# topel/audioset-convnext-inf

Hardware: NVIDIA B200
Metric: clips/sec (10s@32kHz, bf16) (higher is better)
Workload: dtype bf16

## Files before the change

### audioset-convnext-inf_b200/_native.py

```python
import ctypes
import os
import threading

_HERE = os.path.dirname(os.path.abspath(__file__))
_LIB_PATH = os.environ.get("ACX_LIBACX") or os.path.join(_HERE, "libacx.so")
_lock = threading.Lock()
_lib = None

ACX_BF16, ACX_F32 = 0, 1
EPI_BIAS, EPI_BIAS_GELU, EPI_BIAS_SCALE_RESID = 0, 1, 2

_vp, _i, _ll = ctypes.c_void_p, ctypes.c_int, ctypes.c_longlong

SIGNATURES = {
    "acx_version": [],
    "acx_last_error": [],
    "acx_device_ok": [],
    "acx_wave_prep": [_vp, _vp, _vp, _i, _i, _i, _i, _i, _vp],
    "acx_wave_prep_pcm16": [_vp, _vp, _vp, _i, _i, _i, _i, _i, _vp],
    "acx_power_mel_log": [_vp, _i, _i, _vp, _vp, _vp, _vp, _vp, _vp, _i, _i, _vp],
    "acx_frontend_fused": [_vp, _vp, _i, _vp, _vp, _vp, _vp, _i, _vp, _vp, _vp, _i, _i, _i, _i, _i, _vp],
    "acx_frame_fold": [_vp, _vp, _vp, _i, _i, _i, _i, _i, _vp],
    "acx_frame_fold_pcm16": [_vp, _vp, _vp, _i, _i, _i, _i, _i, _vp],
    "acx_frontend_folded": [_vp, _vp, _vp, _vp, _vp, _vp, _i, _vp, _vp, _vp, _i, _i, _i, _i, _vp],
    "acx_stem": [_vp, _vp, _vp, _vp, _vp, _vp, _i, _i, _i, _i, _vp],
    "acx_stem_gp": [_vp, _vp, _vp, _vp, _vp, _vp, _i, _i, _i, _vp],
    "acx_dwconv_ln": [_vp, _vp, _vp, _vp, _vp, _vp, _i, _i, _i, _i, _i, _vp],
    "acx_dwconv_tc": [_vp, _vp, _vp, _vp, _i, _i, _i, _i, _vp],
    "acx_layernorm_rows": [_vp, _vp, _vp, _vp, _ll, _i, _vp],
    "acx_dwconv_tc_gp": [_vp, _vp, _vp, _vp, _i, _i, _i, _i, _vp],
    "acx_gp_transpose": [_vp, _vp, _ll, _i, _i, _vp],
    "acx_gp_row_stats": [_vp, _vp, _ll, _i, _vp],
    "acx_ln_patchify_gp": [_vp, _vp, _vp, _vp, _i, _i, _i, _i, _vp],
    "acx_ln_patchify": [_vp, _vp, _vp, _vp, _i, _i, _i, _i, _i, _vp],
    "acx_downsample_fused_gp": [_vp, _vp, _vp, _vp, _vp, _vp, _i, _i, _i, _i, _i, _vp],
    "acx_gemm_bf16": [_vp, _vp, _vp, _i, _i, _i, _i, _vp, _vp, _vp, _vp],
    "acx_gemm_bf16_gp_out": [_vp, _vp, _vp, _i, _i, _i, _vp, _vp],
    "acx_gemm_bf16_pw1_gp": [_vp, _vp, _vp, _i, _i, _i, _vp, _vp, _vp, _vp],
    "acx_gemm_bf16_pw2_gp": [_vp, _vp, _vp, _i, _i, _i, _vp, _vp, _vp],
    "acx_gemm_f32": [_vp, _ll, _i, _i, _vp, _vp, _i, _i, _i, _i, _i, _vp, _vp, _vp, _vp],
    "acx_mlp_fused": [_vp, _vp, _vp, _vp, _vp, _vp, _vp, _i, _i, _vp],
    "acx_mlp_fused_ln": [_vp, _vp, _vp, _vp, _vp, _vp, _vp, _vp, _vp, _i, _i, _vp],
    "acx_mlp_fused_gp": [_vp, _vp, _vp, _vp, _vp, _vp, _vp, _vp, _vp, _vp, _i, _i, _vp],
    "acx_head": [_vp, _vp, _vp, _vp, _vp, _vp, _vp, _vp, _vp, _i, _i, _i, _i, _i, _i, _vp],
    "acx_nhwc_to_nchw_f32": [_vp, _vp, _i, _i, _i, _i, _i, _vp],
    "acx_resample_fit": [_vp, _i, _vp, _vp, _i, _i, _i, _i, _i, _i, _i, _vp],
    "acx_wave_prep_ragged": [_vp, _vp, _vp, _i, _i, _i, _i, _i, _i, _vp, _vp],
    "acx_frame_fold_ragged": [_vp, _vp, _vp, _i, _i, _i, _i, _i, _i, _vp, _vp],
    "acx_stem_ragged": [_vp, _vp, _vp, _vp, _vp, _vp, _i, _i, _i, _i, _vp, _vp],
    "acx_stem_gp_ragged": [_vp, _vp, _vp, _vp, _vp, _vp, _i, _i, _i, _vp, _vp],
    "acx_dwconv_tc_ragged": [_vp, _vp, _vp, _vp, _i, _i, _i, _i, _vp, _vp],
    "acx_dwconv_tc_gp_ragged": [_vp, _vp, _vp, _vp, _i, _i, _i, _i, _vp, _vp],
    "acx_dwconv_ln_ragged": [_vp, _vp, _vp, _vp, _vp, _vp, _i, _i, _i, _i, _i, _vp, _vp],
    "acx_head_ragged": [_vp, _vp, _vp, _vp, _vp, _vp, _vp, _vp, _vp, _i, _i, _i, _i, _i, _i, _vp, _vp],
    "acx_nhwc_to_nchw_f32_ragged": [_vp, _vp, _i, _i, _i, _i, _i, _vp, _vp],
    "acx_wave_prep_windows": [_vp, _ll, _vp, _vp, _vp, _vp, _i, _i, _i, _i, _i, _vp],
    "acx_wave_prep_pcm16_windows": [_vp, _ll, _vp, _vp, _vp, _vp, _i, _i, _i, _i, _i, _vp],
    "acx_frame_fold_windows": [_vp, _ll, _vp, _vp, _vp, _vp, _i, _i, _i, _i, _i, _vp],
    "acx_frame_fold_pcm16_windows": [_vp, _ll, _vp, _vp, _vp, _vp, _i, _i, _i, _i, _i, _vp],
}


class NativeError(RuntimeError):
    pass


def lib_path():
    return _LIB_PATH


def load():
    global _lib
    if _lib is not None:
        return _lib
    with _lock:
        if _lib is not None:
            return _lib
        if not os.path.isfile(_LIB_PATH):
            try:
                from . import build as _build
                _build.build()
            except Exception as e:
                raise NativeError(
                    f"libacx.so is missing at {_LIB_PATH} and could not be built ({e}). "
                    "The B200 path has no CPU or PyTorch fallback.") from e
        try:
            lib = ctypes.CDLL(_LIB_PATH)
        except OSError as e:
            raise NativeError(f"cannot load {_LIB_PATH}: {e}") from e
        for name, argtypes in SIGNATURES.items():
            try:
                fn = getattr(lib, name)
            except AttributeError as e:
                raise NativeError(f"{_LIB_PATH} does not export {name}; rebuild it") from e
            fn.argtypes = argtypes
            fn.restype = ctypes.c_char_p if name == "acx_last_error" else ctypes.c_int
        _lib = lib
    return _lib


def last_error():
    msg = load().acx_last_error()
    return msg.decode("utf-8", "replace") if msg else ""


def check(rc, what):
    if rc != 0:
        raise NativeError(f"{what} failed (code {rc}): {last_error()}")


def call(name, *args):
    check(getattr(load(), name)(*args), name)
```

### audioset-convnext-inf_b200/csrc/common.cuh

```cuda
#pragma once
#include <cuda.h>
#include <cuda_bf16.h>
#include <cuda_fp16.h>
#include <cuda_runtime.h>
#include <stdint.h>
#include <stdio.h>
#include <stdlib.h>

#include <atomic>

#include "../../include/acx.h"

namespace acx {

void set_error(const char* fmt, ...);
const char* last_error();

#define ACX_CHECK(cond, code, ...)                  \
  do {                                              \
    if (!(cond)) {                                  \
      ::acx::set_error(__VA_ARGS__);                \
      return (code);                                \
    }                                               \
  } while (0)

#define ACX_CUDA(expr)                                                              \
  do {                                                                              \
    cudaError_t _e = (expr);                                                        \
    if (_e != cudaSuccess) {                                                        \
      ::acx::set_error("%s failed: %s (%s:%d)", #expr, cudaGetErrorString(_e),      \
                       __FILE__, __LINE__);                                         \
      return ACX_ERR_CUDA;                                                          \
    }                                                                               \
  } while (0)

#define ACX_SET_MAX_SMEM(kern, bytes)                                                               \
  do {                                                                                              \
    static std::atomic<unsigned long long> acx_done_{0};       \
    int acx_dev_ = 0;                                                                               \
    ACX_CUDA(cudaGetDevice(&acx_dev_));                                                             \
    if (acx_dev_ >= 64 || !((acx_done_.load(std::memory_order_acquire) >> acx_dev_) & 1ull)) {      \
      ACX_CUDA(cudaFuncSetAttribute(kern, cudaFuncAttributeMaxDynamicSharedMemorySize, (bytes)));   \
      if (acx_dev_ < 64) acx_done_.fetch_or(1ull << acx_dev_, std::memory_order_release);           \
    }                                                                                               \
  } while (0)

static inline int sm_count() {
  static std::atomic<int> cached[64];
  int dev = 0;
  if (cudaGetDevice(&dev) != cudaSuccess) return 148;
  if (dev < 64) {
    const int c = cached[dev].load(std::memory_order_relaxed);
    if (c > 0) return c;
  }
  int sms = 0;
  if (cudaDeviceGetAttribute(&sms, cudaDevAttrMultiProcessorCount, dev) != cudaSuccess || sms <= 0) return 148;
  if (dev < 64) cached[dev].store(sms, std::memory_order_relaxed);
  return sms;
}

#ifndef ACX_PDL_DEFAULT
#define ACX_PDL_DEFAULT 7
#endif
__device__ __forceinline__ void pdl_trigger() { asm volatile("griddepcontrol.launch_dependents;" ::: "memory"); }
__device__ __forceinline__ void pdl_wait() { asm volatile("griddepcontrol.wait;" ::: "memory"); }

enum PdlKind { PDL_GEMM = 1, PDL_MLP = 2, PDL_DWTC = 4, PDL_STATS = 8, PDL_SMALL = 16 };
static inline bool pdl_enabled(int kind) {
  const char* e = getenv("ACX_PDL");
  return ((e ? atoi(e) : ACX_PDL_DEFAULT) & kind) != 0;
}

template <typename... KArgs, typename... Args>
static inline cudaError_t launch_pdl(void (*kern)(KArgs...), dim3 grid, dim3 block, size_t smem, cudaStream_t st, int cluster_x,
                                     int kind, Args&&... args) {
  cudaLaunchConfig_t cfg = {};
  cfg.gridDim = grid;
  cfg.blockDim = block;
  cfg.dynamicSmemBytes = smem;
  cfg.stream = st;
  cudaLaunchAttribute attr[2];
  unsigned na = 0;
  if (cluster_x > 1) {
    attr[na].id = cudaLaunchAttributeClusterDimension;
    attr[na].val.clusterDim.x = cluster_x;
    attr[na].val.clusterDim.y = 1;
    attr[na].val.clusterDim.z = 1;
    ++na;
  }
  if (pdl_enabled(kind)) {
    attr[na].id = cudaLaunchAttributeProgrammaticStreamSerialization;
    attr[na].val.programmaticStreamSerializationAllowed = 1;
    ++na;
  }
  cfg.attrs = attr;
  cfg.numAttrs = na;
  return cudaLaunchKernelEx(&cfg, kern, static_cast<KArgs>(args)...);
}

static inline int ceil_div(int a, int b) { return (a + b - 1) / b; }
static inline size_t align_up(size_t x, size_t a) { return (x + a - 1) / a * a; }

using bf16 = __nv_bfloat16;

template <typename T> struct Pair;
template <> struct Pair<float> {
  using type = float2;
  __device__ static __forceinline__ float2 unpack(float2 v) { return v; }
  __device__ static __forceinline__ float2 pack(float a, float b) { return make_float2(a, b); }
};
template <> struct Pair<bf16> {
  using type = uint32_t;
  __device__ static __forceinline__ float2 unpack(uint32_t v) {
    return make_float2(__uint_as_float(v << 16), __uint_as_float(v & 0xffff0000u));
  }
  __device__ static __forceinline__ uint32_t pack(float a, float b) {
    __nv_bfloat162 h = __floats2bfloat162_rn(a, b);
    return *reinterpret_cast<uint32_t*>(&h);
  }
};

__device__ __forceinline__ float to_float(float v) { return v; }
__device__ __forceinline__ float to_float(bf16 v) { return __bfloat162float(v); }
template <typename T> __device__ __forceinline__ T from_float(float v);
template <> __device__ __forceinline__ float from_float<float>(float v) { return v; }
template <> __device__ __forceinline__ bf16 from_float<bf16>(float v) { return __float2bfloat16_rn(v); }

__device__ __forceinline__ float warp_sum(float v) {
#pragma unroll
  for (int o = 16; o > 0; o >>= 1) v += __shfl_xor_sync(0xffffffffu, v, o);
  return v;
}

__device__ __forceinline__ float gelu_erf(float x) {
  return 0.5f * x * (1.0f + erff(x * 0.70710678118654752440f));
}

struct GeluPair {
  unsigned long long x, u;
};
__device__ __forceinline__ unsigned long long f2_pack(float lo, float hi) {
  unsigned long long r;
  asm("mov.b64 %0, {%1, %2};" : "=l"(r) : "f"(lo), "f"(hi));
  return r;
}
__device__ __forceinline__ void gelu_op_tanh(GeluPair& g) {
  asm volatile(
      "{\n\t.reg .f32 lo, hi;\n\tmov.b64 {lo, hi}, %0;\n\ttanh.approx.f32 lo, lo;\n\ttanh.approx.f32 hi, hi;\n\t"
      "mov.b64 %0, {lo, hi};\n\t}"
      : "+l"(g.u));
}
struct LnFold {
  unsigned long long rstd2, nmr2;
  uint32_t sb1_base, sbs_base;
};
template <bool kT, bool kA, bool kFold = false>
__device__ __forceinline__ void gelu_stage_ta4(GeluPair* t, GeluPair* a, const uint32_t* acc, uint32_t sbias_addr,
                                               const LnFold fold = LnFold{}) {
  const unsigned long long k50 = f2_pack(50.0f, 50.0f);
  const unsigned long long kc = f2_pack(-3.51516788e-04f, -3.51516788e-04f);
  const unsigned long long kb = f2_pack(3.70056460e-02f, 3.70056460e-02f);
  const unsigned long long ka = f2_pack(7.97507884e-01f, 7.97507884e-01f);
  unsigned long long q[4], p[4];
  if (kT) gelu_op_tanh(t[0]);
  if (kA) {
#pragma unroll
    for (int i = 0; i < 4; ++i) {
      float2 b;
#ifdef ACX_AB_NO_FOLD_EPI
      if (false) {
#else
      if (kFold) {
#endif
        float2 sj;
        asm("ld.shared.v4.f32 {%0, %1, %2, %3}, [%4];"
            : "=f"(b.x), "=f"(b.y), "=f"(sj.x), "=f"(sj.y)
            : "r"(fold.sbs_base + 2 * (sbias_addr - fold.sb1_base) + 16 * i));
        unsigned long long tt;
        asm volatile("fma.rn.f32x2 %0, %1, %2, %3;" : "=l"(tt) : "l"(fold.nmr2), "l"(f2_pack(sj.x, sj.y)), "l"(f2_pack(b.x, b.y)));
        asm volatile("fma.rn.f32x2 %0, %1, %2, %3;"
                     : "=l"(a[i].x)
                     : "l"(fold.rstd2), "l"(f2_pack(__uint_as_float(acc[2 * i]), __uint_as_float(acc[2 * i + 1]))), "l"(tt));
      } else {
        asm("ld.shared.v2.f32 {%0, %1}, [%2];" : "=f"(b.x), "=f"(b.y) : "r"(sbias_addr + 8 * i));
        asm volatile("add.rn.f32x2 %0, %1, %2;"
                     : "=l"(a[i].x)
                     : "l"(f2_pack(__uint_as_float(acc[2 * i]), __uint_as_float(acc[2 * i + 1]))), "l"(f2_pack(b.x, b.y)));
      }
    }
  }
  if (kT) gelu_op_tanh(t[1]);
  if (kA) {
#pragma unroll
    for (int i = 0; i < 4; ++i) asm volatile("mul.rn.f32x2 %0, %1, %1;" : "=l"(q[i]) : "l"(a[i].x));
#pragma unroll
    for (int i = 0; i < 4; ++i)
      asm volatile(
          "{\n\t.reg .f32 lo, hi, c;\n\tmov.b64 {lo, hi}, %0;\n\tmov.b64 {c, _}, %1;\n\t"
          "min.f32 lo, lo, c;\n\tmin.f32 hi, hi, c;\n\tmov.b64 %0, {lo, hi};\n\t}"
          : "+l"(q[i])
          : "l"(k50));
  }
  if (kT) gelu_op_tanh(t[2]);
  if (kA) {
#pragma unroll
    for (int i = 0; i < 4; ++i) asm volatile("fma.rn.f32x2 %0, %1, %2, %3;" : "=l"(p[i]) : "l"(q[i]), "l"(kc), "l"(kb));
  }
  if (kT) gelu_op_tanh(t[3]);
  if (kA) {
#pragma unroll
    for (int i = 0; i < 4; ++i) asm volatile("fma.rn.f32x2 %0, %1, %2, %3;" : "=l"(q[i]) : "l"(q[i]), "l"(p[i]), "l"(ka));
#pragma unroll
    for (int i = 0; i < 4; ++i) asm volatile("mul.rn.f32x2 %0, %1, %2;" : "=l"(a[i].u) : "l"(a[i].x), "l"(q[i]));
  }
}
__device__ __forceinline__ void gelu_stage_c8_twice_bf16(const GeluPair* g, uint32_t* pk) {
  unsigned long long o[8];
#pragma unroll
  for (int i = 0; i < 8; ++i) asm volatile("fma.rn.f32x2 %0, %1, %2, %1;" : "=l"(o[i]) : "l"(g[i].x), "l"(g[i].u));
#pragma unroll
  for (int i = 0; i < 8; ++i)
    asm volatile("{\n\t.reg .f32 lo, hi;\n\tmov.b64 {lo, hi}, %1;\n\tcvt.rn.bf16x2.f32 %0, hi, lo;\n\t}"
                 : "=r"(pk[i])
                 : "l"(o[i]));
}

template <bool kTwice, bool kFold = false>
__device__ __forceinline__ void bias_gelu_tile16_sp(const uint32_t* __restrict__ acc ,
                                                    const float* __restrict__ sbias , float2 (&out)[16],
                                                    const LnFold fold = LnFold{}) {
  GeluPair g[16];
  const uint32_t sb = static_cast<uint32_t>(__cvta_generic_to_shared(sbias));
  gelu_stage_ta4<false, true, kFold>(nullptr, g, acc, sb, fold);
  gelu_stage_ta4<true, true, kFold>(g, g + 4, acc + 8, sb + 32, fold);
  gelu_stage_ta4<true, true, kFold>(g + 4, g + 8, acc + 16, sb + 64, fold);
  gelu_stage_ta4<true, true, kFold>(g + 8, g + 12, acc + 24, sb + 96, fold);
  gelu_stage_ta4<true, false>(g + 12, nullptr, nullptr, 0);
  const unsigned long long khalf = f2_pack(0.5f, 0.5f);
#pragma unroll
  for (int i = 0; i < 16; ++i) {
    unsigned long long o, x = g[i].x;
    if (!kTwice) asm volatile("mul.rn.f32x2 %0, %1, %2;" : "=l"(x) : "l"(g[i].x), "l"(khalf));
    asm volatile("fma.rn.f32x2 %0, %1, %2, %1;" : "=l"(o) : "l"(x), "l"(g[i].u));
    asm("mov.b64 {%0, %1}, %2;" : "=f"(out[i].x), "=f"(out[i].y) : "l"(o));
  }
}

}
```

### audioset-convnext-inf_b200/csrc/dwconv_tc.cu

```cuda
#include <stdlib.h>

#include "common.cuh"
#include "ptx.cuh"

namespace acx {
namespace dwtc {

constexpr int TR = 63;
constexpr int AR = TR + 6;
constexpr int A_STRIDE = 73 * 128;
constexpr int CG = 8;
constexpr int BAND_TILE = 32 * 64;
constexpr int BAND = 7 * BAND_TILE;
constexpr int NSLOT = 2;
constexpr int THREADS = 256;
constexpr int OFF_A = 0;
constexpr int OFF_BAND = CG * A_STRIDE;
constexpr int OFF_TAPS = OFF_BAND + NSLOT * BAND;
constexpr int OFF_DUMMY = OFF_TAPS + 1024;
constexpr int OFF_BAR = OFF_DUMMY + 512;
constexpr int SMEM_BYTES = OFF_BAR + 128 + 1024;
static_assert(OFF_BAND % 1024 == 0 && BAND % 1024 == 0, "swizzle atoms");
static_assert(2 * (SMEM_BYTES + 1024) <= 227 * 1024, "two CTAs per SM");
static_assert(TR * 28 * 16 <= NSLOT * BAND, "the write-out staging of the planar layout lives in the band slots");
// ... 595 lines not shown
    float sum = 0.f;
#pragma unroll
    for (int j = 0; j < CH; ++j) sum += val[q][j];
#pragma unroll
    for (int o = LPP / 2; o > 0; o >>= 1) sum += __shfl_xor_sync(0xffffffffu, sum, o);
    const float mean = sum * (1.0f / C);
    float sq = 0.f;
#pragma unroll
    for (int j = 0; j < CH; ++j) {
      val[q][j] -= mean;
      sq = fmaf(val[q][j], val[q][j], sq);
    }
#pragma unroll
    for (int o = LPP / 2; o > 0; o >>= 1) sq += __shfl_xor_sync(0xffffffffu, sq, o);
    const float rstd = rsqrtf(sq * (1.0f / C) + 1e-6f);
    if (ok[q]) {
      bf16* dst = out + (grp * NPIX + q) * C + lig * CH;
#pragma unroll
      for (int j = 0; j < 3; ++j) {
        const int k = 8 * j;
        const float4 g0 = __ldg(reinterpret_cast<const float4*>(gp + k)), g1 = __ldg(reinterpret_cast<const float4*>(gp + k + 4));
        const float4 b0 = __ldg(reinterpret_cast<const float4*>(bp + k)), b1 = __ldg(reinterpret_cast<const float4*>(bp + k + 4));
        uint4 o4;
        o4.x = Pair<bf16>::pack(val[q][k + 0] * rstd * g0.x + b0.x, val[q][k + 1] * rstd * g0.y + b0.y);
        o4.y = Pair<bf16>::pack(val[q][k + 2] * rstd * g0.z + b0.z, val[q][k + 3] * rstd * g0.w + b0.w);
        o4.z = Pair<bf16>::pack(val[q][k + 4] * rstd * g1.x + b1.x, val[q][k + 5] * rstd * g1.y + b1.y);
        o4.w = Pair<bf16>::pack(val[q][k + 6] * rstd * g1.z + b1.z, val[q][k + 7] * rstd * g1.w + b1.w);
        reinterpret_cast<uint4*>(dst)[j] = o4;
      }
    }
  }
}

template <int C>
static int launch_ln(const void* in, const float* ln_w, const float* ln_b, void* out, long long M, cudaStream_t st) {
  constexpr int LPP = C / 24, NPIX = 2;
  const long long lanes = (M + NPIX - 1) / NPIX * LPP;
  const long long blocks = (lanes + 255) / 256;
  layernorm_rows_kernel<C><<<(unsigned)blocks, 256, 0, st>>>(reinterpret_cast<const bf16*>(in), ln_w, ln_b,
                                                             reinterpret_cast<bf16*>(out), M);
  ACX_CUDA(cudaGetLastError());
  return ACX_OK;
}

}
}

using namespace acx;

template <bool RAG>
static int dwconv_tc_impl(const void* x, const void* w, const float* bias, void* v, int B, int H, int W, int C,
                          const int32_t* valid, void* stream) {
  ACX_CHECK(x && w && bias && v, ACX_ERR_ARG, "dwconv_tc: null pointer");
  ACX_CHECK(B > 0 && H > 0, ACX_ERR_ARG, "dwconv_tc: B and H must be positive");
  ACX_CHECK(C % 8 == 0 && C > 0, ACX_ERR_ARG, "dwconv_tc: C must be a positive multiple of 8 (got %d)", C);
  ACX_CHECK(x != v, ACX_ERR_ARG, "dwconv_tc: out of place only (neighbouring units read the input halo)");
  ACX_CHECK(((reinterpret_cast<uintptr_t>(x) | reinterpret_cast<uintptr_t>(v)) & 15) == 0, ACX_ERR_ARG,
            "dwconv_tc: x and v must be 16-byte aligned");
  cudaStream_t st = reinterpret_cast<cudaStream_t>(stream);
  switch (W) {
    case 56: return dwtc::launch<56, false, RAG>(x, w, bias, v, B, H, C, valid, st);
    case 28: return dwtc::launch<28, false, RAG>(x, w, bias, v, B, H, C, valid, st);
    case 14: return dwtc::launch<14, false, RAG>(x, w, bias, v, B, H, C, valid, st);
    case 7: return dwtc::launch<7, false, RAG>(x, w, bias, v, B, H, C, valid, st);
    default:
      set_error("dwconv_tc: W=%d not supported (the ConvNeXt stages are 56 / 28 / 14 / 7 wide)", W);
      return ACX_ERR_UNSUPPORTED;
  }
}

extern "C" int acx_dwconv_tc(const void* x, const void* w, const float* bias, void* v, int B, int H, int W, int C,
                             void* stream) {
  return dwconv_tc_impl<false>(x, w, bias, v, B, H, W, C, nullptr, stream);
}

extern "C" int acx_dwconv_tc_ragged(const void* x, const void* w, const float* bias, void* v, int B, int H, int W, int C,
                                    const int32_t* valid, void* stream) {
  ACX_CHECK(valid, ACX_ERR_ARG, "dwconv_tc_ragged: null valid-length array");
  return dwconv_tc_impl<true>(x, w, bias, v, B, H, W, C, valid, stream);
}

template <bool RAG>
static int dwconv_tc_gp_impl(const void* x, const void* w, const float* bias, void* v, int B, int H, int W, int C,
                             const int32_t* valid, void* stream) {
  ACX_CHECK(x && w && bias && v, ACX_ERR_ARG, "dwconv_tc_gp: null pointer");
  ACX_CHECK(B > 0 && H > 0, ACX_ERR_ARG, "dwconv_tc_gp: B and H must be positive");
  ACX_CHECK(C % 8 == 0 && C > 0, ACX_ERR_ARG, "dwconv_tc_gp: C must be a positive multiple of 8 (got %d)", C);
  ACX_CHECK(x != v, ACX_ERR_ARG, "dwconv_tc_gp: out of place only (neighbouring units read the input halo)");
  ACX_CHECK(((reinterpret_cast<uintptr_t>(x) | reinterpret_cast<uintptr_t>(v) | reinterpret_cast<uintptr_t>(w)) & 15) == 0,
            ACX_ERR_ARG, "dwconv_tc_gp: x, v and w must be 16-byte aligned");
  cudaStream_t st = reinterpret_cast<cudaStream_t>(stream);
  static const bool use_v1 = getenv("ACX_DWTC_V1") != nullptr;
  switch (W) {
    case 56:
      return use_v1 ? dwtc::launch<56, true, RAG>(x, w, bias, v, B, H, C, valid, st)
                    : dwtc::v3::launch<56, RAG>(x, w, bias, v, B, H, C, valid, st);
    case 28:
      return use_v1 ? dwtc::launch<28, true, RAG>(x, w, bias, v, B, H, C, valid, st)
                    : dwtc::v3::launch<28, RAG>(x, w, bias, v, B, H, C, valid, st);
    case 14: return dwtc::v3::launch<14, RAG>(x, w, bias, v, B, H, C, valid, st);
    default:
      set_error("dwconv_tc_gp: W=%d not supported (stages 0 - 2: 56 / 28 / 14)", W);
      return ACX_ERR_UNSUPPORTED;
  }
}

extern "C" int acx_dwconv_tc_gp(const void* x, const void* w, const float* bias, void* v, int B, int H, int W, int C,
                                void* stream) {
  return dwconv_tc_gp_impl<false>(x, w, bias, v, B, H, W, C, nullptr, stream);
}

extern "C" int acx_dwconv_tc_gp_ragged(const void* x, const void* w, const float* bias, void* v, int B, int H, int W, int C,
                                       const int32_t* valid, void* stream) {
  ACX_CHECK(valid, ACX_ERR_ARG, "dwconv_tc_gp_ragged: null valid-length array");
  return dwconv_tc_gp_impl<true>(x, w, bias, v, B, H, W, C, valid, stream);
}

namespace acx {
namespace dwtc {
__global__ void __launch_bounds__(256) gp_transpose_kernel(const uint4* __restrict__ in, uint4* __restrict__ out, long long M,
                                                           int G, int to_gp) {
  extern __shared__ uint4 tile[];
  const long long r0 = (long long)blockIdx.x * 64;
  const int rows = (int)min((long long)64, M - r0);
  const int pitch = G + 1;
  const long long Mp = (M + 127) / 128 * 128;
  if (to_gp) {
    for (int i = threadIdx.x; i < rows * G; i += 256) {
      const int r = i / G, gq = i - r * G;
      tile[r * pitch + gq] = in[(r0 + r) * G + gq];
    }
    __syncthreads();
    for (int i = threadIdx.x; i < rows * G; i += 256) {
      const int gq = i / rows, r = i - gq * rows;
      out[(long long)gq * Mp + r0 + r] = tile[r * pitch + gq];
    }
  } else {
    for (int i = threadIdx.x; i < rows * G; i += 256) {
      const int gq = i / rows, r = i - gq * rows;
      tile[r * pitch + gq] = in[(long long)gq * Mp + r0 + r];
    }
    __syncthreads();
    for (int i = threadIdx.x; i < rows * G; i += 256) {
      const int r = i / G, gq = i - r * G;
      out[(r0 + r) * G + gq] = tile[r * pitch + gq];
    }
  }
}
}
}

namespace acx {
namespace dwtc {
__global__ void __launch_bounds__(128) gp_row_stats_kernel(const uint4* __restrict__ v, float2* __restrict__ stats,
                                                           long long M, int G) {
  pdl_trigger();
  pdl_wait();
  const long long row = (long long)blockIdx.x * blockDim.x + threadIdx.x;
  if (row >= M) return;
  const long long Mp = (M + 127) / 128 * 128;
  const float inv_c = 1.0f / (8.0f * G);
  const uint4 first = __ldg(v + row);
  const float shift = __uint_as_float(first.x << 16);
  const float2 sh2 = make_float2(-shift, -shift);
  float2 s = make_float2(0.f, 0.f), q = make_float2(0.f, 0.f);
  for (int g0 = 0; g0 < G; g0 += 12) {
    uint4 u[12];
#pragma unroll
    for (int j = 0; j < 12; ++j) u[j] = g0 + j < G ? __ldg(v + (long long)(g0 + j) * Mp + row) : make_uint4(0, 0, 0, 0);
#pragma unroll
    for (int j = 0; j < 12; ++j) {
      if (g0 + j < G) {
        const uint32_t w[4] = {u[j].x, u[j].y, u[j].z, u[j].w};
#pragma unroll
        for (int k = 0; k < 4; ++k) {
          const float2 d = __fadd2_rn(Pair<bf16>::unpack(w[k]), sh2);
          s = __fadd2_rn(s, d);
          q = __ffma2_rn(d, d, q);
        }
      }
    }
  }
  const float md = (s.x + s.y) * inv_c;
  const float var = fmaxf((q.x + q.y) * inv_c - md * md, 0.f);
  const float rstd = rsqrtf(var + 1e-6f);
  stats[row] = make_float2(rstd, -(md + shift) * rstd);
}
}
}

extern "C" int acx_gp_row_stats(const void* v, float* stats, long long M, int C, void* stream) {
  ACX_CHECK(v && stats, ACX_ERR_ARG, "gp_row_stats: null pointer");
  ACX_CHECK(M > 0 && C > 0 && C % 8 == 0, ACX_ERR_ARG, "gp_row_stats: bad shape M=%lld C=%d", M, C);
  ACX_CUDA(launch_pdl(dwtc::gp_row_stats_kernel, dim3((unsigned)((M + 127) / 128)), dim3(128), 0, reinterpret_cast<cudaStream_t>(stream),
                      1, PDL_STATS, reinterpret_cast<const uint4*>(v), reinterpret_cast<float2*>(stats), M, C / 8));
  return ACX_OK;
}

extern "C" int acx_gp_transpose(const void* in, void* out, long long M, int C, int to_gp, void* stream) {
  ACX_CHECK(in && out && in != out, ACX_ERR_ARG, "gp_transpose: null or aliased pointers");
  ACX_CHECK(M > 0 && C > 0 && C % 8 == 0 && C <= 768, ACX_ERR_ARG, "gp_transpose: bad shape M=%lld C=%d", M, C);
  ACX_CHECK(((reinterpret_cast<uintptr_t>(in) | reinterpret_cast<uintptr_t>(out)) & 15) == 0, ACX_ERR_ARG,
            "gp_transpose: 16-byte alignment");
  const int G = C / 8;
  const size_t smem = (size_t)64 * (G + 1) * 16;
  auto kern = dwtc::gp_transpose_kernel;
  ACX_SET_MAX_SMEM(kern, 64 * (768 / 8 + 1) * 16);
  kern<<<(unsigned)((M + 63) / 64), 256, smem, reinterpret_cast<cudaStream_t>(stream)>>>(
      reinterpret_cast<const uint4*>(in), reinterpret_cast<uint4*>(out), M, G, to_gp);
  ACX_CUDA(cudaGetLastError());
  return ACX_OK;
}

extern "C" int acx_layernorm_rows(const void* in, const float* ln_w, const float* ln_b, void* out, long long M, int C,
                                  void* stream) {
  ACX_CHECK(in && ln_w && ln_b && out, ACX_ERR_ARG, "layernorm_rows: null pointer");
  ACX_CHECK(M > 0, ACX_ERR_ARG, "layernorm_rows: M must be positive");
  ACX_CHECK(((reinterpret_cast<uintptr_t>(in) | reinterpret_cast<uintptr_t>(out)) & 15) == 0, ACX_ERR_ARG,
            "layernorm_rows: in and out must be 16-byte aligned");
  cudaStream_t st = reinterpret_cast<cudaStream_t>(stream);
  switch (C) {
    case 96: return dwtc::launch_ln<96>(in, ln_w, ln_b, out, M, st);
    case 192: return dwtc::launch_ln<192>(in, ln_w, ln_b, out, M, st);
    case 384: return dwtc::launch_ln<384>(in, ln_w, ln_b, out, M, st);
    case 768: return dwtc::launch_ln<768>(in, ln_w, ln_b, out, M, st);
    default:
      set_error("layernorm_rows: C=%d not supported (96 / 192 / 384 / 768)", C);
      return ACX_ERR_UNSUPPORTED;
  }
}
```

### audioset-convnext-inf_b200/csrc/gemm_umma.cu

```cuda
#include <stdlib.h>

#include "common.cuh"
#include "ptx.cuh"
#include "tmap.cuh"

namespace acx {

struct GemmArgs {
  bf16* out;
  const float* bias;
  const float* gamma;
  const bf16* resid;
  int M, N, K;
  int out_gp;
  int a_gp;
  const float2* stats;
  const float* ln_s;
  int reverse;
};
constexpr int ACX_EPI_BIAS_GELU_FOLD = 3;

template <int BN_, int NEPI_, int CG_ = 1>
struct GemmCfg {
  static constexpr int BM = 128, BN = BN_, BK = 64, NEPI = NEPI_, CG = CG_;
  static constexpr int A_BYTES = BM * BK * 2;
  static constexpr int B_BYTES = (BN / CG) * BK * 2;
  static constexpr int STAGE_BYTES = A_BYTES + B_BYTES;
  static constexpr int STAGES_RAW = (160 * 1024) / STAGE_BYTES;
  static constexpr int STAGES = STAGES_RAW > 6 ? 6 : STAGES_RAW;
  static_assert(CG == 1 || BN % 32 == 0, "B halves");
  static constexpr int ACC_STRIDE = BN <= 32 ? 32 : BN <= 64 ? 64 : BN <= 128 ? 128 : 256;
  static constexpr int TMEM_COLS = 2 * ACC_STRIDE;
  static constexpr int CHUNK = 32;
  static constexpr int NCHUNKS = BN / CHUNK;
  static constexpr int CH_G0 = (NCHUNKS + 1) / 2;
  static constexpr int THREADS = 128 + 32 * NEPI;
  static constexpr int STG_TILE = 32 * CHUNK * 2;
  static constexpr int STG_PER_WARP = 3 * STG_TILE;
  static constexpr int OFF_STG = STAGES * STAGE_BYTES;
  static constexpr int OFF_BAR = OFF_STG + NEPI * STG_PER_WARP;
  static constexpr int OFF_VEC = OFF_BAR + 256;
  static constexpr int VEC_BYTES = 16 * 1024;
  static constexpr int SMEM_BYTES = OFF_VEC + VEC_BYTES + 1024 ;
  static_assert(NEPI == 8, "epilogue layout assumes 8 warps");
  static_assert(BN % 32 == 0 && BN >= 32 && BN <= 256, "UMMA N constraint for M=128 / 32-column epilogue chunks");
  static_assert(B_BYTES % 1024 == 0, "stage buffers must stay 1024B aligned for SWIZZLE_128B");
  static_assert(SMEM_BYTES <= 227 * 1024, "smem budget");
};

template <int BN, int EPI, int NEPI, int CG>
__global__ void __launch_bounds__(GemmCfg<BN, NEPI, CG>::THREADS, 1)
    umma_gemm_kernel(const __grid_constant__ CUtensorMap tmA, const __grid_constant__ CUtensorMap tmB,
                     const __grid_constant__ CUtensorMap tmOut, GemmArgs g) {
  using Cfg = GemmCfg<BN, NEPI, CG>;
  const uint32_t cta_rank = CG == 2 ? ptx::cluster_ctarank() : 0u;
  const int unit = CG == 2 ? blockIdx.x >> 1 : blockIdx.x;
  const int num_units = CG == 2 ? gridDim.x >> 1 : gridDim.x;
  extern __shared__ uint8_t smem_raw[];
  uint8_t* smem = reinterpret_cast<uint8_t*>((reinterpret_cast<uintptr_t>(smem_raw) + 1023) & ~uintptr_t(1023));
  uint64_t* full_bar = reinterpret_cast<uint64_t*>(smem + Cfg::OFF_BAR);
  uint64_t* empty_bar = full_bar + Cfg::STAGES;
  uint64_t* tfull_bar = empty_bar + Cfg::STAGES;
  uint64_t* tempty_bar = tfull_bar + 2;
  uint32_t* tmem_slot = reinterpret_cast<uint32_t*>(tempty_bar + 2);

  const int warp = threadIdx.x >> 5;
  const int lane = threadIdx.x & 31;
  float* sbias = reinterpret_cast<float*>(smem + Cfg::OFF_VEC);
  float* sgamma = sbias + g.N;
  if (EPI == ACX_EPI_BIAS_GELU_FOLD) {
    for (int i = threadIdx.x; i < g.N; i += blockDim.x) {
      sbias[4 * (i >> 1) + (i & 1)] = g.bias[i];
      sbias[4 * (i >> 1) + 2 + (i & 1)] = g.ln_s[i];
    }
  } else {
    for (int i = threadIdx.x; i < g.N; i += blockDim.x) {
      sbias[i] = g.bias[i];
      if (EPI == ACX_EPI_BIAS_SCALE_RESID) sgamma[i] = g.gamma[i];
    }
  }

  if (warp == 0 && ptx::elect_one()) {
    ptx::prefetch_tensormap(&tmA);
    ptx::prefetch_tensormap(&tmB);
    ptx::prefetch_tensormap(&tmOut);
  }
  if (warp == 1 && ptx::elect_one()) {
    for (int s = 0; s < Cfg::STAGES; ++s) {
      ptx::mbar_init(&full_bar[s], 1);
      ptx::mbar_init(&empty_bar[s], 1);
    }
    for (int a = 0; a < 2; ++a) {
      ptx::mbar_init(&tfull_bar[a], 1);
      ptx::mbar_init(&tempty_bar[a], NEPI * CG);
    }
    ptx::fence_barrier_init();
  }
  if (warp == 2) {
    if (CG == 2) {
      ptx::tmem_alloc_cg2(tmem_slot, Cfg::TMEM_COLS);
      ptx::tmem_relinquish_cg2();
    } else {
      ptx::tmem_alloc(tmem_slot, Cfg::TMEM_COLS);
      ptx::tmem_relinquish();
    }
  }
  ptx::tc_fence_before();
  __syncthreads();
  if (CG == 2) ptx::cluster_sync_all();
  ptx::tc_fence_after();
  const uint32_t tmem_base = *tmem_slot;
  pdl_trigger();
  pdl_wait();

  const int num_m_tiles = (g.M + Cfg::BM * CG - 1) / (Cfg::BM * CG);
  const int num_n_tiles = g.N / BN;
  const int num_tiles = num_m_tiles * num_n_tiles;
  const int num_kb = (g.K + Cfg::BK - 1) / Cfg::BK;

  if (warp == 0) {
    if (ptx::elect_one()) {
      int stage = 0;
      uint32_t phase = 0;
      for (int tile = unit; tile < num_tiles; tile += num_units) {
        const int tt = g.reverse ? num_tiles - 1 - tile : tile;
        const int m0 = (tt / num_n_tiles) * Cfg::BM * CG + cta_rank * Cfg::BM;
        const int n0 = (tt % num_n_tiles) * BN + cta_rank * (BN / CG);
        for (int kb = 0; kb < num_kb; ++kb) {
          ptx::mbar_wait(&empty_bar[stage], phase ^ 1);
          uint8_t* sa = smem + stage * Cfg::STAGE_BYTES;
          uint8_t* sb = sa + Cfg::A_BYTES;
          if (CG == 2) {
            if (cta_rank == 0) ptx::mbar_arrive_expect_tx(&full_bar[stage], 2 * Cfg::STAGE_BYTES);
            if (g.a_gp) ptx::tma_load_3d_cg2(sa, &tmA, &full_bar[stage], 0, m0 >> 5, kb * (Cfg::BK / 8));
            else ptx::tma_load_2d_cg2(sa, &tmA, &full_bar[stage], kb * Cfg::BK, m0);
            ptx::tma_load_2d_cg2(sb, &tmB, &full_bar[stage], kb * Cfg::BK, n0);
          } else {
            ptx::mbar_arrive_expect_tx(&full_bar[stage], Cfg::STAGE_BYTES);
            if (g.a_gp) ptx::tma_load_3d(sa, &tmA, &full_bar[stage], 0, m0 >> 5, kb * (Cfg::BK / 8));
            else ptx::tma_load_2d(sa, &tmA, &full_bar[stage], kb * Cfg::BK, m0);
            ptx::tma_load_2d(sb, &tmB, &full_bar[stage], kb * Cfg::BK, n0);
          }
          if (++stage == Cfg::STAGES) {
            stage = 0;
            phase ^= 1;
          }
        }
      }
    }
  } else if (warp == 1) {
    if (cta_rank == 0 && ptx::elect_one()) {
      constexpr uint32_t idesc = ptx::umma_idesc_bf16(Cfg::BM * CG, BN);
      int stage = 0;
      uint32_t phase = 0;
      int it = 0;
      for (int tile = unit; tile < num_tiles; tile += num_units, ++it) {
        const int acc = it & 1;
        const uint32_t acc_phase = (it >> 1) & 1;
        ptx::mbar_wait(&tempty_bar[acc], acc_phase ^ 1);
        ptx::tc_fence_after();
        const uint32_t d_tmem = tmem_base + acc * Cfg::ACC_STRIDE;
        for (int kb = 0; kb < num_kb; ++kb) {
          ptx::mbar_wait(&full_bar[stage], phase);
          ptx::tc_fence_after();
          const uint32_t sa = ptx::smem_u32(smem + stage * Cfg::STAGE_BYTES);
          const uint64_t da = g.a_gp ? ptx::umma_desc_nosw_kmajor(sa, Cfg::BM * 16, 128) : ptx::umma_desc_sw128_kmajor(sa);
          const uint32_t ka = g.a_gp ? (2 * Cfg::BM * 16) >> 4 : 2;
          const uint64_t db = ptx::umma_desc_sw128_kmajor(sa + Cfg::A_BYTES);
#pragma unroll
          for (int k = 0; k < Cfg::BK / 16; ++k) {
            if (kb * Cfg::BK + k * 16 < g.K) {
              if (CG == 2) ptx::umma_bf16_cg2(d_tmem, da + ka * k, db + 2 * k, idesc, (kb | k) != 0 ? 1u : 0u);
              else ptx::umma_bf16(d_tmem, da + ka * k, db + 2 * k, idesc, (kb | k) != 0 ? 1u : 0u);
            }
          }
          if (CG == 2) ptx::umma_commit_cg2(&empty_bar[stage]);
          else ptx::umma_commit(&empty_bar[stage]);
          if (++stage == Cfg::STAGES) {
            stage = 0;
            phase ^= 1;
          }
        }
        if (CG == 2) ptx::umma_commit_cg2(&tfull_bar[acc]);
        else ptx::umma_commit(&tfull_bar[acc]);
      }
    }
  } else if (warp >= 4) {
    const int ew = warp - 4;
    const int quad = warp & 3;
    const int group = ew >> 2;
    const int ch_begin = group == 0 ? 0 : Cfg::CH_G0;
    const int ch_count = group == 0 ? Cfg::CH_G0 : Cfg::NCHUNKS - Cfg::CH_G0;
    uint8_t* stg = smem + Cfg::OFF_STG + ew * Cfg::STG_PER_WARP;
    uint8_t* rbuf = stg + 2 * Cfg::STG_TILE;
    const int sw = (lane >> 1) & 3;
    const int ld_piece = lane & 3, ld_row = lane >> 2;
    int it = 0;
    uint32_t store_parity = 0;
    for (int tile = unit; tile < num_tiles; tile += num_units, ++it) {
      const int acc = it & 1;
      const uint32_t acc_phase = (it >> 1) & 1;
      const int tt = g.reverse ? num_tiles - 1 - tile : tile;
      const int m0 = (tt / num_n_tiles) * Cfg::BM * CG + cta_rank * Cfg::BM;
      const int n0 = (tt % num_n_tiles) * BN;
      const int row0 = m0 + quad * 32;
      uint4 rq[4];
      auto fetch_resid = [&](int ci) {
        if (EPI != ACX_EPI_BIAS_SCALE_RESID) return;
        const int n = n0 + (ch_begin + ci) * Cfg::CHUNK;
#pragma unroll
        for (int q = 0; q < 4; ++q) {
          const int r = row0 + ld_row + 8 * q;
          rq[q] = make_uint4(0u, 0u, 0u, 0u);
          if (r < g.M)
            rq[q] = g.out_gp ? *reinterpret_cast<const uint4*>(g.resid + ((size_t)((n >> 3) + ld_piece) * (((size_t)g.M + 127) / 128 * 128) + r) * 8)
                             : *reinterpret_cast<const uint4*>(g.resid + (size_t)r * g.N + n + ld_piece * 8);
        }
      };
      fetch_resid(0);
      LnFold fold{0ull, 0ull, ptx::smem_u32(sbias), ptx::smem_u32(sbias)};
      if (EPI == ACX_EPI_BIAS_GELU_FOLD) {
        const int r = row0 + lane;
        const float2 stt = r < g.M ? __ldg(g.stats + r) : make_float2(0.f, 0.f);
        fold.rstd2 = f2_pack(stt.x, stt.x);
        fold.nmr2 = f2_pack(stt.y, stt.y);
      }
      ptx::mbar_wait(&tfull_bar[acc], acc_phase);
      ptx::tc_fence_after();
      const uint32_t t_base = tmem_base + (static_cast<uint32_t>(quad * 32) << 16) + acc * Cfg::ACC_STRIDE +
                              ch_begin * Cfg::CHUNK;
      uint32_t ra[32], rb[32];
      ptx::tmem_ld_32x32b_x32(t_base, ra);
#pragma unroll
      for (int ci = 0; ci < Cfg::CH_G0; ++ci) {
        if (ci < ch_count) {
          uint32_t(&r)[32] = (ci & 1) ? rb : ra;
          ptx::tmem_ld_wait();
          if (ci + 1 < ch_count) {
            ptx::tmem_ld_32x32b_x32(t_base + (ci + 1) * Cfg::CHUNK, (ci & 1) ? ra : rb);
          } else {
            ptx::tc_fence_before();
            __syncwarp();
            if (lane == 0) {
              if (CG == 2) ptx::mbar_arrive_leader(&tempty_bar[acc]);
              else ptx::mbar_arrive(&tempty_bar[acc]);
            }
          }
          const int n = n0 + (ch_begin + ci) * Cfg::CHUNK;
          float v[32];
          if (EPI == ACX_EPI_BIAS_GELU_FOLD) {
            float2 o[16];
            bias_gelu_tile16_sp<false, true>(r, sbias + n, o, fold);
#pragma unroll
            for (int j = 0; j < 16; ++j) {
              v[2 * j] = o[j].x;
              v[2 * j + 1] = o[j].y;
            }
          } else if (EPI == ACX_EPI_BIAS_GELU) {
            float2 o[16];
            bias_gelu_tile16_sp<false>(r, sbias + n, o);
#pragma unroll
            for (int j = 0; j < 16; ++j) {
              v[2 * j] = o[j].x;
              v[2 * j + 1] = o[j].y;
            }
          } else {
#pragma unroll
            for (int j = 0; j < 32; j += 4) {
              const float4 b4 = *reinterpret_cast<const float4*>(sbias + n + j);
              v[j + 0] = __uint_as_float(r[j + 0]) + b4.x;
              v[j + 1] = __uint_as_float(r[j + 1]) + b4.y;
              v[j + 2] = __uint_as_float(r[j + 2]) + b4.z;
              v[j + 3] = __uint_as_float(r[j + 3]) + b4.w;
            }
          }
          if (EPI == ACX_EPI_BIAS_SCALE_RESID) {
            __syncwarp();
#pragma unroll
            for (int q = 0; q < 4; ++q) {
              const int rr = ld_row + 8 * q;
              *reinterpret_cast<uint4*>(rbuf + rr * 64 + ((ld_piece ^ ((rr >> 1) & 3)) << 4)) = rq[q];
            }
            __syncwarp();
            if (ci + 1 < ch_count) fetch_resid(ci + 1);
#pragma unroll
            for (int j4 = 0; j4 < 4; ++j4) {
              const uint4 q = *reinterpret_cast<const uint4*>(rbuf + lane * 64 + ((j4 ^ sw) << 4));
              const float4 g0 = *reinterpret_cast<const float4*>(sgamma + n + j4 * 8);
              const float4 g1 = *reinterpret_cast<const float4*>(sgamma + n + j4 * 8 + 4);
              const int j = j4 * 8;
              float2 f;
              f = Pair<bf16>::unpack(q.x); v[j + 0] = fmaf(g0.x, v[j + 0], f.x); v[j + 1] = fmaf(g0.y, v[j + 1], f.y);
              f = Pair<bf16>::unpack(q.y); v[j + 2] = fmaf(g0.z, v[j + 2], f.x); v[j + 3] = fmaf(g0.w, v[j + 3], f.y);
              f = Pair<bf16>::unpack(q.z); v[j + 4] = fmaf(g1.x, v[j + 4], f.x); v[j + 5] = fmaf(g1.y, v[j + 5], f.y);
              f = Pair<bf16>::unpack(q.w); v[j + 6] = fmaf(g1.z, v[j + 6], f.x); v[j + 7] = fmaf(g1.w, v[j + 7], f.y);
            }
          }
          if (lane == 0) ptx::tma_store_wait_read<1>();
          __syncwarp();
          uint8_t* tile_smem = stg + store_parity * Cfg::STG_TILE;
#pragma unroll
          for (int j4 = 0; j4 < 4; ++j4) {
            const int j = j4 * 8;
            uint4 q;
            q.x = Pair<bf16>::pack(v[j + 0], v[j + 1]);
            q.y = Pair<bf16>::pack(v[j + 2], v[j + 3]);
            q.z = Pair<bf16>::pack(v[j + 4], v[j + 5]);
            q.w = Pair<bf16>::pack(v[j + 6], v[j + 7]);
            *reinterpret_cast<uint4*>(g.out_gp ? tile_smem + j4 * 512 + lane * 16 : tile_smem + lane * 64 + ((j4 ^ sw) << 4)) = q;
          }
          ptx::fence_proxy_async_smem();
          __syncwarp();
          if (lane == 0) {
            if (g.out_gp) ptx::tma_store_3d(&tmOut, tile_smem, 0, row0 >> 5, n >> 3);
            else ptx::tma_store_2d(&tmOut, tile_smem, n, row0);
            ptx::tma_store_commit();
          }
          store_parity ^= 1;
        }
      }
    }
    if (lane == 0) ptx::tma_store_wait_read<0>();
  }

  ptx::tc_fence_before();
  __syncthreads();
  if (CG == 2) ptx::cluster_sync_all();
  if (warp == 2) {
    ptx::tc_fence_after();
    if (CG == 2) ptx::tmem_dealloc_cg2(tmem_base, Cfg::TMEM_COLS);
    else ptx::tmem_dealloc(tmem_base, Cfg::TMEM_COLS);
  }
}

template <int BN, int EPI, int NEPI, int CG>
static int launch_umma_gemm(const CUtensorMap& tmA, const CUtensorMap& tmB, const CUtensorMap& tmOut, const GemmArgs& g,
                            cudaStream_t st) {
  using Cfg = GemmCfg<BN, NEPI, CG>;
  auto kern = umma_gemm_kernel<BN, EPI, NEPI, CG>;
  ACX_SET_MAX_SMEM(kern, Cfg::SMEM_BYTES);
  ACX_CHECK(g.N * (EPI == ACX_EPI_BIAS_SCALE_RESID || EPI == ACX_EPI_BIAS_GELU_FOLD ? 8 : 4) <= Cfg::VEC_BYTES, ACX_ERR_UNSUPPORTED,
            "gemm_bf16: N=%d exceeds the per-column vectors staged in shared memory", g.N);
  int dev = 0, sms = 0;
  ACX_CUDA(cudaGetDevice(&dev));
  ACX_CUDA(cudaDeviceGetAttribute(&sms, cudaDevAttrMultiProcessorCount, dev));
  const int tiles = ceil_div(g.M, Cfg::BM * CG) * (g.N / BN);
  const int units = sms / CG;
  ACX_CUDA(launch_pdl(kern, dim3((tiles < units ? tiles : units) * CG), dim3(Cfg::THREADS), Cfg::SMEM_BYTES, st, CG, PDL_GEMM, tmA, tmB,
                      tmOut, g));
  return ACX_OK;
}

template <int EPI>
static int dispatch_bn(const CUtensorMap& tmA, const void* W, const GemmArgs& g, cudaStream_t st) {
  int bn = 0;
  for (int cand : {256, 192, 128, 96}) {
    if (g.N % cand == 0) {
      bn = cand;
      break;
    }
  }
  ACX_CHECK(bn != 0, ACX_ERR_UNSUPPORTED, "gemm_bf16: N=%d is not a multiple of 96/128/192/256", g.N);
  static const bool pair_ok = getenv("ACX_GEMM_PAIR") == nullptr || atoi(getenv("ACX_GEMM_PAIR")) != 0;
  const long long pairs = sm_count() / 2;
  if (pair_ok && bn == 256 && g.N % 192 == 0) {
    const long long mt = ceil_div(g.M, 256);
    const long long r256 = (mt * (g.N / 256) + pairs - 1) / pairs * 256, r192 = (mt * (g.N / 192) + pairs - 1) / pairs * 192;
    if (mt * (g.N / 192) >= pairs && r192 < r256) bn = 192;
  }
  const bool pair = pair_ok && (bn == 256 || bn == 192) && (long long)ceil_div(g.M, 256) * (g.N / bn) >= pairs;
  CUtensorMap tmB;
  int rc = make_tmap_2d_bf16(&tmB, W, (uint64_t)g.K, (uint64_t)g.N, (uint64_t)g.K * 2, 64,
                             (uint32_t)(pair ? bn / 2 : bn));
  if (rc != ACX_OK) return rc;
  CUtensorMap tmOut;
  rc = g.out_gp ? make_tmap_gp_bf16(&tmOut, g.out, (uint64_t)g.M, (uint64_t)g.N / 8, 32, 4)
                : make_tmap_2d_bf16(&tmOut, g.out, (uint64_t)g.N, (uint64_t)g.M, (uint64_t)g.N * 2, 32, 32,
                                    CU_TENSOR_MAP_SWIZZLE_64B);
  if (rc != ACX_OK) return rc;
  if (pair) {
    if (bn == 256) return launch_umma_gemm<256, EPI, 8, 2>(tmA, tmB, tmOut, g, st);
    return launch_umma_gemm<192, EPI, 8, 2>(tmA, tmB, tmOut, g, st);
  }
  switch (bn) {
    case 256: return launch_umma_gemm<256, EPI, 8, 1>(tmA, tmB, tmOut, g, st);
    case 192: return launch_umma_gemm<192, EPI, 8, 1>(tmA, tmB, tmOut, g, st);
    case 128: return launch_umma_gemm<128, EPI, 8, 1>(tmA, tmB, tmOut, g, st);
    default:  return launch_umma_gemm<96, EPI, 8, 1>(tmA, tmB, tmOut, g, st);
  }
}

}

using namespace acx;

static int gemm_bf16_impl(const void* A, const void* W, void* out, int M, int N, int K, int epilogue, const float* bias,
                          const float* gamma, const void* resid, int out_gp, int a_gp, const float* stats,
                          const float* ln_s, void* stream) {
  ACX_CHECK(A && W && out && bias, ACX_ERR_ARG, "gemm_bf16: null pointer (A, W, out and bias are required)");
  ACX_CHECK(M > 0 && N > 0 && K > 0 && K % 8 == 0, ACX_ERR_ARG, "gemm_bf16: K=%d must be a positive multiple of 8", K);
  ACX_CHECK((reinterpret_cast<uintptr_t>(A) & 15) == 0 && (reinterpret_cast<uintptr_t>(W) & 15) == 0 &&
                (reinterpret_cast<uintptr_t>(out) & 15) == 0,
            ACX_ERR_ARG, "gemm_bf16: A, W and out must be 16-byte aligned");
  if (epilogue == ACX_EPI_BIAS_SCALE_RESID)
    ACX_CHECK(gamma && resid, ACX_ERR_ARG, "gemm_bf16: scale+residual epilogue needs gamma and resid");
  ACX_CHECK(!out_gp || epilogue != ACX_EPI_BIAS_GELU, ACX_ERR_UNSUPPORTED, "gemm_bf16: the hidden activation stays row-major");
  ACX_CHECK(!a_gp || K % 64 == 0, ACX_ERR_UNSUPPORTED, "gemm_bf16: a planar A operand needs K %% 64 == 0 (got %d)", K);
  ACX_CHECK((stats == nullptr) == (ln_s == nullptr), ACX_ERR_ARG, "gemm_bf16: stats and ln_s go together");
  ACX_CHECK(!stats || epilogue == ACX_EPI_BIAS_GELU, ACX_ERR_UNSUPPORTED, "gemm_bf16: the LayerNorm fold belongs to the GELU epilogue");
  GemmArgs g;
  g.out = reinterpret_cast<bf16*>(out);
  g.bias = bias;
  g.gamma = gamma;
  g.resid = reinterpret_cast<const bf16*>(resid);
  g.M = M;
  g.N = N;
  g.K = K;
  g.out_gp = out_gp;
  g.a_gp = a_gp;
  g.stats = reinterpret_cast<const float2*>(stats);
  g.ln_s = ln_s;
  static const bool rev_ok = getenv("ACX_GEMM_REVERSE") == nullptr || atoi(getenv("ACX_GEMM_REVERSE")) != 0;
  g.reverse = rev_ok && epilogue == ACX_EPI_BIAS_SCALE_RESID && (size_t)M * K * 2 > (size_t)96 << 20;
  CUtensorMap tmA;
  int rc = a_gp ? make_tmap_gp_bf16(&tmA, A, (uint64_t)M, (uint64_t)K / 8, 128, 8)
                : make_tmap_2d_bf16(&tmA, A, (uint64_t)K, (uint64_t)M, (uint64_t)K * 2, 64, 128);
  if (rc != ACX_OK) return rc;
  cudaStream_t st = reinterpret_cast<cudaStream_t>(stream);
  switch (epilogue) {
    case ACX_EPI_BIAS: return dispatch_bn<ACX_EPI_BIAS>(tmA, W, g, st);
    case ACX_EPI_BIAS_GELU:
      return stats ? dispatch_bn<ACX_EPI_BIAS_GELU_FOLD>(tmA, W, g, st) : dispatch_bn<ACX_EPI_BIAS_GELU>(tmA, W, g, st);
    case ACX_EPI_BIAS_SCALE_RESID: return dispatch_bn<ACX_EPI_BIAS_SCALE_RESID>(tmA, W, g, st);
    default:
      set_error("gemm_bf16: unknown epilogue %d", epilogue);
      return ACX_ERR_ARG;
  }
}

extern "C" int acx_gemm_bf16(const void* A, const void* W, void* out, int M, int N, int K, int epilogue,
                             const float* bias, const float* gamma, const void* resid, void* stream) {
  return gemm_bf16_impl(A, W, out, M, N, K, epilogue, bias, gamma, resid, 0, 0, nullptr, nullptr, stream);
}

extern "C" int acx_gemm_bf16_gp_out(const void* A, const void* W, void* out, int M, int N, int K, const float* bias,
                                    void* stream) {
  return gemm_bf16_impl(A, W, out, M, N, K, ACX_EPI_BIAS, bias, nullptr, nullptr, 1, 0, nullptr, nullptr, stream);
}

extern "C" int acx_gemm_bf16_pw1_gp(const void* v_gp, const void* w1f, void* hid, int M, int N, int K, const float* b1f,
                                    const float* stats, const float* ln_s, void* stream) {
  ACX_CHECK(stats && ln_s, ACX_ERR_ARG, "gemm_bf16_pw1_gp: stats and ln_s are required");
  return gemm_bf16_impl(v_gp, w1f, hid, M, N, K, ACX_EPI_BIAS_GELU, b1f, nullptr, nullptr, 0, 1, stats, ln_s, stream);
}
extern "C" int acx_gemm_bf16_pw2_gp(const void* hid, const void* w2, void* x_gp, int M, int N, int K, const float* b2,
                                    const float* gamma, void* stream) {
  return gemm_bf16_impl(hid, w2, x_gp, M, N, K, ACX_EPI_BIAS_SCALE_RESID, b2, gamma, x_gp, 1, 0, nullptr, nullptr, stream);
}
```

### audioset-convnext-inf_b200/csrc/mlp_fused.cu

```cuda
#include <stdlib.h>

#include "common.cuh"
#include "ptx.cuh"
#include "tmap.cuh"

namespace acx {

struct MlpArgs {
  bf16* x;
  const float* b1;
  const float* b2;
  const float* gamma;
  int M;
  const float* ln_w;
  const float* ln_b;
  const float* ln_s;
  unsigned long long* trace;
};

template <int C, typename ChunkFn>
__device__ __forceinline__ void ln_row_in_smem(ChunkFn chunk, const float* __restrict__ sw, const float* __restrict__ sb) {
  constexpr int NCH = C / 8;
  float shift;
  {
    const uint32_t w0 = *reinterpret_cast<const uint32_t*>(chunk(0));
    shift = __uint_as_float(w0 << 16);
  }
  const float2 sh2 = make_float2(-shift, -shift);
  float2 s = make_float2(0.f, 0.f), q = make_float2(0.f, 0.f);
#pragma unroll 4
  for (int j = 0; j < NCH; ++j) {
    const uint4 v = *reinterpret_cast<const uint4*>(chunk(j));
    const uint32_t w[4] = {v.x, v.y, v.z, v.w};
#pragma unroll
    for (int k = 0; k < 4; ++k) {
      const float2 d = __fadd2_rn(Pair<bf16>::unpack(w[k]), sh2);
      s = __fadd2_rn(s, d);
      q = __ffma2_rn(d, d, q);
    }
  }
  const float md = (s.x + s.y) * (1.0f / C);
  const float var = fmaxf((q.x + q.y) * (1.0f / C) - md * md, 0.f);
  const float rstd = rsqrtf(var + 1e-6f);
  const float nmr = -(md + shift) * rstd;
  const float2 r2 = make_float2(rstd, rstd), n2 = make_float2(nmr, nmr);
#pragma unroll 2
  for (int j = 0; j < NCH; ++j) {
    uint8_t* pc = chunk(j);
    const uint4 v = *reinterpret_cast<const uint4*>(pc);
    const uint32_t w[4] = {v.x, v.y, v.z, v.w};
    uint32_t o[4];
#pragma unroll
    for (int k = 0; k < 4; ++k) {
      const float2 g = *reinterpret_cast<const float2*>(sw + 8 * j + 2 * k);
      const float2 b = *reinterpret_cast<const float2*>(sb + 8 * j + 2 * k);
      const float2 t = __fmul2_rn(r2, g);
      const float2 u = __ffma2_rn(n2, g, b);
      const float2 y = __ffma2_rn(Pair<bf16>::unpack(w[k]), t, u);
      o[k] = Pair<bf16>::pack(y.x, y.y);
    }
    *reinterpret_cast<uint4*>(pc) = make_uint4(o[0], o[1], o[2], o[3]);
  }
}

template <int C, typename ChunkFn>
__device__ __forceinline__ float2 ln_row_stats_smem(ChunkFn chunk) {
  constexpr int NCH = C / 8;
  const float shift = __uint_as_float(*reinterpret_cast<const uint32_t*>(chunk(0)) << 16);
  const float2 sh2 = make_float2(-shift, -shift);
  float2 s = make_float2(0.f, 0.f), q = make_float2(0.f, 0.f);
#pragma unroll 4
  for (int j = 0; j < NCH; ++j) {
    const uint4 v = *reinterpret_cast<const uint4*>(chunk(j));
    const uint32_t w[4] = {v.x, v.y, v.z, v.w};
#pragma unroll
    for (int k = 0; k < 4; ++k) {
      const float2 d = __fadd2_rn(Pair<bf16>::unpack(w[k]), sh2);
      s = __fadd2_rn(s, d);
      q = __ffma2_rn(d, d, q);
    }
  }
  const float md = (s.x + s.y) * (1.0f / C);
  const float var = fmaxf((q.x + q.y) * (1.0f / C) - md * md, 0.f);
  const float rstd = rsqrtf(var + 1e-6f);
  return make_float2(rstd, -(md + shift) * rstd);
}

template <int C_>
struct MlpCfg {
  static constexpr int C = C_, HD = 4 * C, BM = 128, NH = 128, BK = 64;
  static constexpr int NC = HD / NH;
  static constexpr int KB1 = (C + BK - 1) / BK;
  static constexpr int KB2 = NH / BK;
  static constexpr int A_TILE = BM * BK * 2;
  static constexpr int A_BUFS = C <= 96 ? 2 : 1;
  static constexpr int W1_TILE = NH * BK * 2;
  static constexpr int W2_TILE = C * BK * 2;
  static constexpr int SLOT = W1_TILE > W2_TILE ? W1_TILE : W2_TILE;
  static constexpr int SLOTS = C <= 96 ? 4 : 3;
  static constexpr int H_TILE = BM * BK * 2;
  static constexpr int OFF_A = 0;
  static constexpr int OFF_RING = OFF_A + A_BUFS * KB1 * A_TILE;
  static constexpr int OFF_H = OFF_RING + SLOTS * SLOT;
  static constexpr int OFF_STG = OFF_H + 2 * KB2 * H_TILE;
  static constexpr int STG_TILE = 32 * 64;
  static constexpr int STG_PER_WARP = STG_TILE;
  static constexpr int OFF_BAR = OFF_STG + 8 * STG_PER_WARP;
  static constexpr int OFF_VEC = OFF_BAR + 512;
  static constexpr int SMEM_BYTES = OFF_VEC + (3 * HD + 4 * C) * 4 + 2 * BM * 8 + 1024;
  static constexpr int D2_COL = 0, D1_COL = 256, TMEM_COLS = 512;
  static constexpr int OUT_CHUNKS = C / 32;
  static constexpr int OUT_G0 = (OUT_CHUNKS + 1) / 2;
  static constexpr int THREADS = 512;
  static_assert(C % 32 == 0 && C <= 192, "D2 must fit 256 TMEM columns");
  static_assert(SLOT % 1024 == 0 && W2_TILE % 1024 == 0, "swizzle alignment");
  static_assert(SMEM_BYTES <= 227 * 1024, "smem budget");
};

template <int C, bool GP, bool FOLD>
__global__ void __launch_bounds__(512, 1)
    mlp_fused_kernel(const __grid_constant__ CUtensorMap tmY, const __grid_constant__ CUtensorMap tmW1,
                     const __grid_constant__ CUtensorMap tmW2, const __grid_constant__ CUtensorMap tmOut, MlpArgs a) {
  using Cfg = MlpCfg<C>;
  extern __shared__ uint8_t smem_raw[];
  uint8_t* smem = reinterpret_cast<uint8_t*>((reinterpret_cast<uintptr_t>(smem_raw) + 1023) & ~uintptr_t(1023));
  uint64_t* bars = reinterpret_cast<uint64_t*>(smem + Cfg::OFF_BAR);
  uint64_t* ring_full = bars;
  uint64_t* ring_empty = ring_full + Cfg::SLOTS;
  uint64_t* a_full = ring_empty + Cfg::SLOTS;
  uint64_t* a_empty = a_full + Cfg::A_BUFS;
  uint64_t* d1_full = a_empty + Cfg::A_BUFS;
  uint64_t* d1_empty = d1_full + 2;
  uint64_t* h_full = d1_empty + 2;
  uint64_t* h_empty = h_full + 2;
  uint64_t* d2_full = h_empty + 2;
  uint64_t* d2_empty = d2_full + 1;
  uint64_t* a_ready = d2_empty + 1;
  uint32_t* tmem_slot = reinterpret_cast<uint32_t*>(a_ready + Cfg::A_BUFS);

  const int warp = threadIdx.x >> 5;
  const int lane = threadIdx.x & 31;
  float* sb1 = reinterpret_cast<float*>(smem + Cfg::OFF_VEC);
  float* sb2 = sb1 + Cfg::HD;
  float* sgamma = sb2 + C;
  float* slnw = sgamma + C;
  float* slnb = slnw + C;
  float* ss1 = slnb + C;
  float2* sstat = reinterpret_cast<float2*>(ss1 + 2 * Cfg::HD);
  const bool ln = a.ln_w != nullptr;
  for (int i = threadIdx.x; i < Cfg::HD; i += blockDim.x) sb1[i] = a.b1[i];
  if (FOLD)
    for (int i = threadIdx.x; i < Cfg::HD; i += blockDim.x) {
      ss1[4 * (i >> 1) + (i & 1)] = a.b1[i];
      ss1[4 * (i >> 1) + 2 + (i & 1)] = a.ln_s[i];
    }
  if (ln)
    for (int i = threadIdx.x; i < C; i += blockDim.x) {
      slnw[i] = a.ln_w[i];
      slnb[i] = a.ln_b[i];
    }
  for (int i = threadIdx.x; i < C; i += blockDim.x) {
    sgamma[i] = 0.5f * a.gamma[i];
    sb2[i] = a.gamma[i] * a.b2[i];
  }

  if (warp == 0 && ptx::elect_one()) {
    ptx::prefetch_tensormap(&tmY);
    ptx::prefetch_tensormap(&tmW1);
    ptx::prefetch_tensormap(&tmW2);
    ptx::prefetch_tensormap(&tmOut);
  }
  if (warp == 1 && ptx::elect_one()) {
    for (int s = 0; s < Cfg::SLOTS; ++s) {
      ptx::mbar_init(&ring_full[s], 1);
      ptx::mbar_init(&ring_empty[s], 1);
    }
    for (int s = 0; s < Cfg::A_BUFS; ++s) {
      ptx::mbar_init(&a_full[s], 1);
      ptx::mbar_init(&a_empty[s], FOLD ? 5 : 1);
      ptx::mbar_init(&a_ready[s], 4);
    }
    for (int s = 0; s < 2; ++s) {
      ptx::mbar_init(&d1_full[s], 1);
      ptx::mbar_init(&d1_empty[s], 8);
      ptx::mbar_init(&h_full[s], 8);
      ptx::mbar_init(&h_empty[s], 1);
    }
    ptx::mbar_init(d2_full, 1);
    ptx::mbar_init(d2_empty, 4);
    ptx::fence_barrier_init();
  }
  if (warp == 2) {
    ptx::tmem_alloc(tmem_slot, Cfg::TMEM_COLS);
    ptx::tmem_relinquish();
  }
  ptx::tc_fence_before();
  __syncthreads();
  ptx::tc_fence_after();
  const uint32_t tmem_base = *tmem_slot;
  const int num_tiles = (a.M + Cfg::BM - 1) / Cfg::BM;
  pdl_trigger();
  if (warp != 0) pdl_wait();

  if (warp == 3) {
    if (ptx::elect_one()) {
      int it = 0;
      for (int tile = blockIdx.x; tile < num_tiles; tile += gridDim.x, ++it) {
        const int buf = it % Cfg::A_BUFS;
        const uint32_t use = it / Cfg::A_BUFS;
        ptx::mbar_wait(&a_empty[buf], (use & 1) ^ 1);
        uint8_t* sa = smem + Cfg::OFF_A + buf * Cfg::KB1 * Cfg::A_TILE;
        ptx::mbar_arrive_expect_tx(&a_full[buf], Cfg::KB1 * Cfg::A_TILE);
        if (GP) {
          ptx::tma_load_3d(sa, &tmY, &a_full[buf], 0, tile * (Cfg::BM / 32), 0);
        } else {
          for (int kb = 0; kb < Cfg::KB1; ++kb)
            ptx::tma_load_2d(sa + kb * Cfg::A_TILE, &tmY, &a_full[buf], kb * Cfg::BK, tile * Cfg::BM);
        }
      }
    }
  } else if (warp == 0) {
    if (ptx::elect_one()) {
      int slot = 0;
      uint32_t phase = 0;
      auto next_slot = [&]() -> uint8_t* {
        ptx::mbar_wait(&ring_empty[slot], phase ^ 1);
        return smem + Cfg::OFF_RING + slot * Cfg::SLOT;
      };
      auto advance = [&]() {
        if (++slot == Cfg::SLOTS) {
          slot = 0;
          phase ^= 1;
        }
      };
      auto load_w2 = [&](int hh) {
        for (int kb = 0; kb < Cfg::KB2; ++kb) {
          uint8_t* dst = next_slot();
          ptx::mbar_arrive_expect_tx(&ring_full[slot], Cfg::W2_TILE);
          ptx::tma_load_2d(dst, &tmW2, &ring_full[slot], hh * Cfg::NH + kb * Cfg::BK, 0);
          advance();
        }
      };
      for (int tile = blockIdx.x; tile < num_tiles; tile += gridDim.x) {
        for (int h = 0; h < Cfg::NC; ++h) {
          for (int kb = 0; kb < Cfg::KB1; ++kb) {
            uint8_t* dst = next_slot();
            ptx::mbar_arrive_expect_tx(&ring_full[slot], Cfg::W1_TILE);
            ptx::tma_load_2d(dst, &tmW1, &ring_full[slot], kb * Cfg::BK, h * Cfg::NH);
            advance();
          }
          if (h >= 1) load_w2(h - 1);
        }
        load_w2(Cfg::NC - 1);
      }
    }
  } else if (warp == 1) {
    if (ptx::elect_one()) {
      constexpr uint32_t idesc1 = ptx::umma_idesc_bf16(Cfg::BM, Cfg::NH);
      constexpr uint32_t idesc2 = ptx::umma_idesc_bf16(Cfg::BM, C);
      const uint32_t d2 = tmem_base + Cfg::D2_COL;
      int slot = 0;
      uint32_t phase = 0;
      auto advance = [&]() {
        if (++slot == Cfg::SLOTS) {
          slot = 0;
          phase ^= 1;
        }
      };
      int it = 0;
      uint32_t gc = 0;
      for (int tile = blockIdx.x; tile < num_tiles; tile += gridDim.x, ++it) {
        const int abuf = it % Cfg::A_BUFS;
        const uint32_t ause = it / Cfg::A_BUFS;
        const uint32_t sa = ptx::smem_u32(smem + Cfg::OFF_A + abuf * Cfg::KB1 * Cfg::A_TILE);
        auto gemm2 = [&](int hh, uint32_t gch) {
          const int hb = gch & 1;
          ptx::mbar_wait(&h_full[hb], (gch >> 1) & 1);
          if (hh == 0) ptx::mbar_wait(d2_empty, (it & 1) ^ 1);
          ptx::tc_fence_after();
          const uint32_t sh = ptx::smem_u32(smem + Cfg::OFF_H + hb * Cfg::KB2 * Cfg::H_TILE);
          for (int kb = 0; kb < Cfg::KB2; ++kb) {
            ptx::mbar_wait(&ring_full[slot], phase);
            ptx::tc_fence_after();
            const uint64_t da = ptx::umma_desc_sw128_kmajor(sh + kb * Cfg::H_TILE);
            const uint64_t db = ptx::umma_desc_sw128_kmajor(ptx::smem_u32(smem + Cfg::OFF_RING + slot * Cfg::SLOT));
#pragma unroll
            for (int k = 0; k < Cfg::BK / 16; ++k)
              ptx::umma_bf16(d2, da + 2 * k, db + 2 * k, idesc2, (hh | kb | k) != 0 ? 1u : 0u);
            ptx::umma_commit(&ring_empty[slot]);
            advance();
          }
          ptx::umma_commit(&h_empty[hb]);
        };
        ptx::mbar_wait((ln && !FOLD) ? &a_ready[abuf] : &a_full[abuf], ause & 1);
        ptx::tc_fence_after();
        for (int h = 0; h < Cfg::NC; ++h, ++gc) {
          const int db1 = gc & 1;
          ptx::mbar_wait(&d1_empty[db1], ((gc >> 1) & 1) ^ 1);
          ptx::tc_fence_after();
          const uint32_t d1 = tmem_base + Cfg::D1_COL + db1 * Cfg::NH;
          for (int kb = 0; kb < Cfg::KB1; ++kb) {
            ptx::mbar_wait(&ring_full[slot], phase);
            ptx::tc_fence_after();
            const uint64_t da = GP ? ptx::umma_desc_nosw_kmajor(sa + kb * Cfg::A_TILE, Cfg::BM * 16, 128)
                                   : ptx::umma_desc_sw128_kmajor(sa + kb * Cfg::A_TILE);
            const uint64_t db = ptx::umma_desc_sw128_kmajor(ptx::smem_u32(smem + Cfg::OFF_RING + slot * Cfg::SLOT));
#pragma unroll
            for (int k = 0; k < Cfg::BK / 16; ++k)
              if (kb * Cfg::BK + k * 16 < C)
                ptx::umma_bf16(d1, da + (GP ? k * (4096 >> 4) : 2 * k), db + 2 * k, idesc1, (kb | k) != 0 ? 1u : 0u);
            ptx::umma_commit(&ring_empty[slot]);
            advance();
          }
          ptx::umma_commit(&d1_full[db1]);
          if (h == Cfg::NC - 1) ptx::umma_commit(&a_empty[abuf]);
          if (h >= 1) gemm2(h - 1, gc - 1);
        }
        gemm2(Cfg::NC - 1, gc - 1);
        ptx::umma_commit(d2_full);
      }
    }
  } else if (warp >= 4 && warp < 12) {
    const int ew = warp - 4;
    const int quad = warp & 3;
    const int group = ew >> 2;
    const int row_in_tile = quad * 32 + lane;
    const uint32_t lane_base = tmem_base + (static_cast<uint32_t>(quad * 32) << 16);
    uint32_t gc = 0;
    LnFold fold{0ull, 0ull, ptx::smem_u32(sb1), ptx::smem_u32(ss1)};
    int it1 = 0;
    for (int tile = blockIdx.x; tile < num_tiles; tile += gridDim.x, ++it1) {
      for (int h = 0; h < Cfg::NC; ++h, ++gc) {
        const int buf = gc & 1;
        const uint32_t par = (gc >> 1) & 1;
        ptx::mbar_wait(&d1_full[buf], par);
        ptx::tc_fence_after();
        const uint32_t t0 = lane_base + Cfg::D1_COL + buf * Cfg::NH + group * 64;
        const float* bias = sb1 + h * Cfg::NH + group * 64;
        if (FOLD && h == 0) {
          const int abuf = it1 % Cfg::A_BUFS;
          ptx::mbar_wait(&a_ready[abuf], (it1 / Cfg::A_BUFS) & 1);
          const float2 stt = sstat[(it1 & 1) * Cfg::BM + row_in_tile];
          fold.rstd2 = f2_pack(stt.x, stt.x);
          fold.nmr2 = f2_pack(stt.y, stt.y);
        }
        uint8_t* hrow = smem + Cfg::OFF_H + (buf * Cfg::KB2 + group) * Cfg::H_TILE + row_in_tile * 128;
        uint32_t ra[32];
        ptx::tmem_ld_32x32b_x32(t0, ra);
        ptx::tmem_ld_wait();
#pragma unroll
        for (int half = 0; half < 2; ++half) {
          uint32_t packed[16];
          {
            float2 o[16];
            bias_gelu_tile16_sp<true, FOLD>(ra, bias + 32 * half, o, fold);
#pragma unroll
            for (int j = 0; j < 16; ++j) packed[j] = Pair<bf16>::pack(o[j].x, o[j].y);
          }
          if (half == 0) {
            ptx::tmem_ld_32x32b_x32(t0 + 32, ra);
            ptx::mbar_wait(&h_empty[buf], par ^ 1);
          }
#pragma unroll
          for (int q = 0; q < 4; ++q)
            *reinterpret_cast<uint4*>(hrow + (((4 * half + q) ^ (row_in_tile & 7)) << 4)) =
                make_uint4(packed[4 * q], packed[4 * q + 1], packed[4 * q + 2], packed[4 * q + 3]);
          if (half == 0) {
            ptx::tmem_ld_wait();
            ptx::tc_fence_before();
            __syncwarp();
            if (lane == 0) ptx::mbar_arrive(&d1_empty[buf]);
          }
        }
        ptx::fence_proxy_async_smem();
        __syncwarp();
        if (lane == 0) ptx::mbar_arrive(&h_full[buf]);
      }
    }
  } else if (warp >= 12) {
    constexpr int NCH = C / 32;
    const int quad = warp & 3;
    const uint32_t lane_base = tmem_base + (static_cast<uint32_t>(quad * 32) << 16);
    uint8_t* stg = smem + Cfg::OFF_STG + quad * 4096;
    const int sw64 = (lane >> 1) & 3;
    const int ld_piece = lane & 3, ld_row = lane >> 2;
    auto ln_tile = [&](int j) {
      const int buf = j % Cfg::A_BUFS;
      ptx::mbar_wait(&a_full[buf], (j / Cfg::A_BUFS) & 1);
      const int r = quad * 32 + lane;
      uint8_t* base = smem + Cfg::OFF_A + buf * Cfg::KB1 * Cfg::A_TILE + r * 128;
      if (GP)
        ln_row_in_smem<C>([&](int ch) { return base - r * 128 + ch * (Cfg::BM * 16) + r * 16; }, slnw, slnb);
      else
        ln_row_in_smem<C>([&](int ch) { return base + (ch >> 3) * Cfg::A_TILE + (((ch & 7) ^ (r & 7)) << 4); }, slnw, slnb);
      ptx::fence_proxy_async_smem();
      __syncwarp();
      if (lane == 0) ptx::mbar_arrive(&a_ready[buf]);
    };
    auto stats_tile = [&](int j) {
      const int buf = j % Cfg::A_BUFS;
      ptx::mbar_wait(&a_full[buf], (j / Cfg::A_BUFS) & 1);
      const int r = quad * 32 + lane;
      uint8_t* base = smem + Cfg::OFF_A + buf * Cfg::KB1 * Cfg::A_TILE;
      sstat[(j & 1) * Cfg::BM + r] =
          GP ? ln_row_stats_smem<C>([&](int ch) { return base + ch * (Cfg::BM * 16) + r * 16; })
             : ln_row_stats_smem<C>([&](int ch) { return base + r * 128 + (ch >> 3) * Cfg::A_TILE + (((ch & 7) ^ (r & 7)) << 4); });
      __syncwarp();
      if (lane == 0) {
        ptx::mbar_arrive(&a_ready[buf]);
        ptx::mbar_arrive(&a_empty[buf]);
      }
    };
    if (FOLD && (int)blockIdx.x < num_tiles) stats_tile(0);
    if (!FOLD && ln && (int)blockIdx.x < num_tiles) ln_tile(0);
    int it = 0;
    for (int tile = blockIdx.x; tile < num_tiles; tile += gridDim.x, ++it) {
      const int row0 = tile * Cfg::BM + quad * 32;
      if (FOLD && tile + (int)gridDim.x < num_tiles) stats_tile(it + 1);
      if (!FOLD && ln && tile + (int)gridDim.x < num_tiles) ln_tile(it + 1);
      auto fetch_resid = [&](int c) {
        uint8_t* dst = stg + (c & 1) * 2048;
#pragma unroll
        for (int q = 0; q < 4; ++q) {
          const int rr = ld_row + 8 * q;
          const int r = row0 + rr;
          const bf16* src = GP ? a.x + ((size_t)(c * 4 + ld_piece) * (((size_t)a.M + 127) / 128 * 128) + (r < a.M ? r : 0)) * 8
                               : a.x + (size_t)(r < a.M ? r : 0) * C + c * 32 + ld_piece * 8;
          const uint32_t d = GP ? ptx::smem_u32(dst + ld_piece * 512 + rr * 16)
                                : ptx::smem_u32(dst + rr * 64 + ((ld_piece ^ ((rr >> 1) & 3)) << 4));
          const int nbytes = r < a.M ? 16 : 0;
          asm volatile("cp.async.ca.shared.global [%0], [%1], 16, %2;" ::"r"(d), "l"(src), "r"(nbytes) : "memory");
        }
        asm volatile("cp.async.commit_group;" ::: "memory");
      };
      if (lane == 0) ptx::tma_store_wait_read<0>();
      __syncwarp();
      fetch_resid(0);
      ptx::mbar_wait(d2_full, it & 1);
      ptx::tc_fence_after();
#pragma unroll
      for (int c = 0; c < NCH; ++c) {
        uint8_t* tbuf = stg + (c & 1) * 2048;
        uint32_t r[32];
        ptx::tmem_ld_32x32b_x32(lane_base + Cfg::D2_COL + c * 32, r);
        if (c + 1 < NCH) {
          if (c >= 1) {
            if (lane == 0) ptx::tma_store_wait_read<0>();
            __syncwarp();
          }
          fetch_resid(c + 1);
          asm volatile("cp.async.wait_group 1;" ::: "memory");
        } else {
          asm volatile("cp.async.wait_group 0;" ::: "memory");
        }
        ptx::tmem_ld_wait();
        if (c == NCH - 1) {
          ptx::tc_fence_before();
          __syncwarp();
          if (lane == 0) ptx::mbar_arrive(d2_empty);
        }
        __syncwarp();
        uint4 res[4];
#pragma unroll
        for (int j4 = 0; j4 < 4; ++j4)
          res[j4] = *reinterpret_cast<const uint4*>(GP ? tbuf + j4 * 512 + lane * 16 : tbuf + lane * 64 + ((j4 ^ sw64) << 4));
        __syncwarp();
        const int n = c * 32;
#pragma unroll
        for (int j4 = 0; j4 < 4; ++j4) {
          const int j = j4 * 8;
          const float4 bA = *reinterpret_cast<const float4*>(sb2 + n + j);
          const float4 bB = *reinterpret_cast<const float4*>(sb2 + n + j + 4);
          const float4 gA = *reinterpret_cast<const float4*>(sgamma + n + j);
          const float4 gB = *reinterpret_cast<const float4*>(sgamma + n + j + 4);
          float2 f;
          uint4 o;
          f = Pair<bf16>::unpack(res[j4].x);
          o.x = Pair<bf16>::pack(fmaf(gA.x, __uint_as_float(r[j + 0]), bA.x + f.x), fmaf(gA.y, __uint_as_float(r[j + 1]), bA.y + f.y));
          f = Pair<bf16>::unpack(res[j4].y);
          o.y = Pair<bf16>::pack(fmaf(gA.z, __uint_as_float(r[j + 2]), bA.z + f.x), fmaf(gA.w, __uint_as_float(r[j + 3]), bA.w + f.y));
          f = Pair<bf16>::unpack(res[j4].z);
          o.z = Pair<bf16>::pack(fmaf(gB.x, __uint_as_float(r[j + 4]), bB.x + f.x), fmaf(gB.y, __uint_as_float(r[j + 5]), bB.y + f.y));
          f = Pair<bf16>::unpack(res[j4].w);
          o.w = Pair<bf16>::pack(fmaf(gB.z, __uint_as_float(r[j + 6]), bB.z + f.x), fmaf(gB.w, __uint_as_float(r[j + 7]), bB.w + f.y));
          *reinterpret_cast<uint4*>(GP ? tbuf + j4 * 512 + lane * 16 : tbuf + lane * 64 + ((j4 ^ sw64) << 4)) = o;
        }
        ptx::fence_proxy_async_smem();
        __syncwarp();
        if (lane == 0) {
          if (GP) ptx::tma_store_3d(&tmOut, tbuf, 0, row0 >> 5, c * 4);
          else ptx::tma_store_2d(&tmOut, tbuf, n, row0);
          ptx::tma_store_commit();
        }
      }
    }
    if (lane == 0) ptx::tma_store_wait_read<0>();
  }

  ptx::tc_fence_before();
  __syncthreads();
  if (warp == 2) {
    ptx::tc_fence_after();
    ptx::tmem_dealloc(tmem_base, Cfg::TMEM_COLS);
  }
}

#define ACX_TRACE(role, ev)                                                                    \
  do {                                                                                         \
    if (a.trace && blockIdx.x == 0 && it < 16) a.trace[(it * 2 + (role)) * 32 + (ev)] = clock64(); \
  } while (0)

struct Mlp96 {
  static constexpr int C = 96, HD = 384, BM = 128, NH = 64, NC = 6;
  static constexpr int OFF_W1M = 0;
  static constexpr int OFF_W1T = OFF_W1M + 3 * 16384;
  static constexpr int OFF_W2 = OFF_W1T + 3 * 8192;
  static constexpr int OFF_AM = OFF_W2 + 6 * 12288;
  static constexpr int OFF_AT = OFF_AM + 16384;
  static constexpr int OFF_H = OFF_AT + 8192;
  static constexpr int OFF_STG = OFF_H + 32768;
  static constexpr int OFF_BAR = OFF_STG + 8 * 2048;
  static constexpr int OFF_VEC = OFF_BAR + 256;
  static constexpr int SMEM_BYTES = OFF_VEC + (3 * HD + 4 * C) * 4 + 2 * BM * 8 + 1024;
  static constexpr int D2_COL = 0, D2_STRIDE = 128, D1_COL = 256, TMEM_COLS = 512;
  static constexpr int W_BYTES = 3 * 16384 + 3 * 8192 + 6 * 12288;
  static_assert(SMEM_BYTES <= 227 * 1024, "smem budget");
};

template <bool GP, bool FOLD>
__global__ void __launch_bounds__(512, 1)
    mlp_fused96_kernel(const __grid_constant__ CUtensorMap tmYm, const __grid_constant__ CUtensorMap tmYt,
                       const __grid_constant__ CUtensorMap tmW1m, const __grid_constant__ CUtensorMap tmW1t,
                       const __grid_constant__ CUtensorMap tmW2, const __grid_constant__ CUtensorMap tmOut, MlpArgs a) {
  using Cfg = Mlp96;
  constexpr int C = 96;
  extern __shared__ uint8_t smem_raw[];
  uint8_t* smem = reinterpret_cast<uint8_t*>((reinterpret_cast<uintptr_t>(smem_raw) + 1023) & ~uintptr_t(1023));
  uint64_t* bars = reinterpret_cast<uint64_t*>(smem + Cfg::OFF_BAR);
  uint64_t* w_full = bars;
  uint64_t* a_full = bars + 1;
  uint64_t* a_empty = bars + 2;
  uint64_t* d1_full = bars + 3;
  uint64_t* d1_empty = bars + 7;
  uint64_t* h_full = bars + 11;
  uint64_t* h_empty = bars + 13;
  uint64_t* d2_full = bars + 15;
  uint64_t* d2_empty = bars + 17;
  uint64_t* a_ready = bars + 19;
  uint32_t* tmem_slot = reinterpret_cast<uint32_t*>(bars + 20);

  const int warp = threadIdx.x >> 5;
  const int lane = threadIdx.x & 31;
  float* sb1 = reinterpret_cast<float*>(smem + Cfg::OFF_VEC);
  float* sb2 = sb1 + Cfg::HD;
  float* sgamma = sb2 + C;
  float* slnw = sgamma + C;
  float* slnb = slnw + C;
  float* ss1 = slnb + C;
  float2* sstat = reinterpret_cast<float2*>(ss1 + 2 * Cfg::HD);
  const bool ln = a.ln_w != nullptr;
  for (int i = threadIdx.x; i < Cfg::HD; i += blockDim.x) sb1[i] = a.b1[i];
  if (FOLD)
    for (int i = threadIdx.x; i < Cfg::HD; i += blockDim.x) {
      ss1[4 * (i >> 1) + (i & 1)] = a.b1[i];
      ss1[4 * (i >> 1) + 2 + (i & 1)] = a.ln_s[i];
    }
  if (ln)
    for (int i = threadIdx.x; i < C; i += blockDim.x) {
      slnw[i] = a.ln_w[i];
      slnb[i] = a.ln_b[i];
    }
  for (int i = threadIdx.x; i < C; i += blockDim.x) {
    sgamma[i] = 0.5f * a.gamma[i];
    sb2[i] = a.gamma[i] * a.b2[i];
  }
  if (warp == 0 && ptx::elect_one()) {
    ptx::prefetch_tensormap(&tmYm);
    ptx::prefetch_tensormap(&tmYt);
    ptx::prefetch_tensormap(&tmW1m);
    ptx::prefetch_tensormap(&tmW1t);
    ptx::prefetch_tensormap(&tmW2);
    ptx::prefetch_tensormap(&tmOut);
  }
  if (warp == 1 && ptx::elect_one()) {
    ptx::mbar_init(w_full, 1);
    ptx::mbar_init(a_full, 1);
    ptx::mbar_init(a_empty, FOLD ? 5 : 1);
    ptx::mbar_init(a_ready, 4);
    for (int s = 0; s < 4; ++s) {
      ptx::mbar_init(&d1_full[s], 1);
      ptx::mbar_init(&d1_empty[s], 4);
    }
    for (int s = 0; s < 2; ++s) {
      ptx::mbar_init(&h_full[s], 4);
      ptx::mbar_init(&h_empty[s], 1);
      ptx::mbar_init(&d2_full[s], 1);
      ptx::mbar_init(&d2_empty[s], 4);
    }
    ptx::fence_barrier_init();
  }
  if (warp == 2) {
    ptx::tmem_alloc(tmem_slot, Cfg::TMEM_COLS);
    ptx::tmem_relinquish();
  }
  ptx::tc_fence_before();
  __syncthreads();
  ptx::tc_fence_after();
  const uint32_t tmem_base = *tmem_slot;
  const int num_tiles = (a.M + Cfg::BM - 1) / Cfg::BM;
  pdl_trigger();
  if (warp != 0) pdl_wait();

  if (warp == 0) {
    if (ptx::elect_one()) {
      ptx::mbar_arrive_expect_tx(w_full, Cfg::W_BYTES);
      for (int h = 0; h < 3; ++h) {
        ptx::tma_load_2d(smem + Cfg::OFF_W1M + h * 16384, &tmW1m, w_full, 0, h * 128);
        ptx::tma_load_2d(smem + Cfg::OFF_W1T + h * 8192, &tmW1t, w_full, 64, h * 128);
      }
      for (int kb = 0; kb < 6; ++kb) ptx::tma_load_2d(smem + Cfg::OFF_W2 + kb * 12288, &tmW2, w_full, kb * 64, 0);
      pdl_wait();
      int it = 0;
      for (int tile = blockIdx.x; tile < num_tiles; tile += gridDim.x, ++it) {
        ptx::mbar_wait(a_empty, (it & 1) ^ 1);
        ptx::mbar_arrive_expect_tx(a_full, 16384 + 8192);
        const int next = tile + gridDim.x;
        if (GP) {
          ptx::tma_load_3d(smem + Cfg::OFF_AM, &tmYm, a_full, 0, tile * (Cfg::BM / 32), 0);
          if (next < num_tiles) ptx::tma_prefetch_3d(&tmYm, 0, next * (Cfg::BM / 32), 0);
        } else {
          ptx::tma_load_2d(smem + Cfg::OFF_AM, &tmYm, a_full, 0, tile * Cfg::BM);
          ptx::tma_load_2d(smem + Cfg::OFF_AT, &tmYt, a_full, 64, tile * Cfg::BM);
          if (next < num_tiles) {
            ptx::tma_prefetch_2d(&tmYm, 0, next * Cfg::BM);
            ptx::tma_prefetch_2d(&tmYt, 64, next * Cfg::BM);
          }
        }
      }
    }
  } else if (warp == 1) {
    if (ptx::elect_one()) {
      constexpr uint32_t idesc1 = ptx::umma_idesc_bf16(Cfg::BM, Cfg::NH);
      constexpr uint32_t idesc2 = ptx::umma_idesc_bf16(Cfg::BM, C);
      const uint32_t sbase = ptx::smem_u32(smem);
      const uint64_t dAm = ptx::umma_desc_sw128_kmajor(sbase + Cfg::OFF_AM);
      const uint64_t dAt = ptx::umma_desc_sw64_kmajor(sbase + Cfg::OFF_AT);
      const uint64_t dAg = ptx::umma_desc_nosw_kmajor(sbase + Cfg::OFF_AM, 128 * 16, 128);
      ptx::mbar_wait(w_full, 0);
      ptx::tc_fence_after();
      const int my_tiles = (int)blockIdx.x < num_tiles ? (num_tiles - 1 - (int)blockIdx.x) / (int)gridDim.x + 1 : 0;
      const uint32_t total = (uint32_t)Cfg::NC * my_tiles;
      auto gemm1 = [&](uint32_t g, int h, int it) {
        if (h == 0) {
          ptx::mbar_wait((ln && !FOLD) ? a_ready : a_full, it & 1);
          ptx::tc_fence_after();
        }
        const int db1 = g & 3;
        ptx::mbar_wait(&d1_empty[db1], ((g >> 2) & 1) ^ 1);
        ptx::tc_fence_after();
        const uint32_t d1 = tmem_base + Cfg::D1_COL + db1 * Cfg::NH;
        const uint64_t dBm = ptx::umma_desc_sw128_kmajor(sbase + Cfg::OFF_W1M + (h >> 1) * 16384 + (h & 1) * 8192);
        const uint64_t dBt = ptx::umma_desc_sw64_kmajor(sbase + Cfg::OFF_W1T + (h >> 1) * 8192 + (h & 1) * 4096);
        if (GP) {
#pragma unroll
          for (int k = 0; k < 4; ++k) ptx::umma_bf16(d1, dAg + k * (4096 >> 4), dBm + 2 * k, idesc1, k != 0 ? 1u : 0u);
#pragma unroll
          for (int k = 0; k < 2; ++k) ptx::umma_bf16(d1, dAg + (4 + k) * (4096 >> 4), dBt + 2 * k, idesc1, 1u);
        } else {
#pragma unroll
          for (int k = 0; k < 4; ++k) ptx::umma_bf16(d1, dAm + 2 * k, dBm + 2 * k, idesc1, k != 0 ? 1u : 0u);
#pragma unroll
          for (int k = 0; k < 2; ++k) ptx::umma_bf16(d1, dAt + 2 * k, dBt + 2 * k, idesc1, 1u);
        }
        ptx::umma_commit(&d1_full[db1]);
        if (h == Cfg::NC - 1) ptx::umma_commit(a_empty);
      };
      auto gemm2 = [&](uint32_t g, int h, int it) {
        const int hb = g & 1;
        ptx::mbar_wait(&h_full[hb], (g >> 1) & 1);
        ACX_TRACE(0, 2 * h);
        if (h == 0) ptx::mbar_wait(&d2_empty[it & 1], ((it >> 1) & 1) ^ 1);
        ptx::tc_fence_after();
        const uint32_t d2 = tmem_base + Cfg::D2_COL + (it & 1) * Cfg::D2_STRIDE;
        const uint64_t da = ptx::umma_desc_sw128_kmajor(sbase + Cfg::OFF_H + hb * 16384);
        const uint64_t db = ptx::umma_desc_sw128_kmajor(sbase + Cfg::OFF_W2 + h * 12288);
#pragma unroll
        for (int k = 0; k < 4; ++k) ptx::umma_bf16(d2, da + 2 * k, db + 2 * k, idesc2, (h | k) != 0 ? 1u : 0u);
        ptx::umma_commit(&h_empty[hb]);
        if (h == Cfg::NC - 1) ptx::umma_commit(&d2_full[it & 1]);
        ACX_TRACE(0, 2 * h + 1);
      };
      constexpr int LA = 4;
      int h1 = 0, it1 = 0;
      uint32_t g1 = 0;
      auto issue_gemm1 = [&]() {
        if (g1 < total) {
          gemm1(g1, h1, it1);
          ++g1;
          if (++h1 == Cfg::NC) {
            h1 = 0;
            ++it1;
          }
        }
      };
      for (int i = 0; i < LA; ++i) issue_gemm1();
      int h = 0, it = 0;
      for (uint32_t g = 0; g < total; ++g) {
        gemm2(g, h, it);
        issue_gemm1();
        if (++h == Cfg::NC) {
          h = 0;
          ++it;
        }
      }
    }
  } else if (warp >= 4 && warp < 12) {
    const int ew = warp - 4;
    const int quad = warp & 3;
    const int group = ew >> 2;
    const int row_in_tile = quad * 32 + lane;
    const uint32_t lane_base = tmem_base + (static_cast<uint32_t>(quad * 32) << 16);
    const bool tr = (warp == 4 && lane == 0);
    LnFold fold{0ull, 0ull, ptx::smem_u32(sb1), ptx::smem_u32(ss1)};
    int it = 0;
    for (int tile = blockIdx.x; tile < num_tiles; tile += gridDim.x, ++it) {
      if (FOLD) {
        ptx::mbar_wait(a_ready, it & 1);
        const float2 stt = sstat[(it & 1) * Cfg::BM + row_in_tile];
        fold.rstd2 = f2_pack(stt.x, stt.x);
        fold.nmr2 = f2_pack(stt.y, stt.y);
      }
      for (int hc = 0; hc < Cfg::NC / 2; ++hc) {
        const int h = 2 * hc + group;
        const uint32_t gc = (uint32_t)Cfg::NC * it + h;
        const int buf = gc & 3;
        if (tr) ACX_TRACE(1, 4 * hc);
        ptx::mbar_wait(&d1_full[buf], (gc >> 2) & 1);
        ptx::tc_fence_after();
        if (tr) ACX_TRACE(1, 4 * hc + 1);
        const uint32_t t0 = lane_base + Cfg::D1_COL + buf * Cfg::NH;
        const uint32_t bias = ptx::smem_u32(sb1 + h * Cfg::NH);
        const uint32_t hrow = ptx::smem_u32(smem + Cfg::OFF_H + group * 16384 + row_in_tile * 128);
        uint32_t raA[16], raB[16];
        GeluPair gA[8], gB[8];
        uint32_t pk[8] = {};
        auto store_quarter = [&](int qi) {
          asm volatile("st.shared.v4.b32 [%0], {%1, %2, %3, %4};" ::"r"(hrow + (((2 * qi) ^ (row_in_tile & 7)) << 4)),
                       "r"(pk[0]), "r"(pk[1]), "r"(pk[2]), "r"(pk[3])
                       : "memory");
          asm volatile("st.shared.v4.b32 [%0], {%1, %2, %3, %4};" ::"r"(hrow + (((2 * qi + 1) ^ (row_in_tile & 7)) << 4)),
                       "r"(pk[4]), "r"(pk[5]), "r"(pk[6]), "r"(pk[7])
                       : "memory");
        };
        ptx::tmem_ld_32x32b_x16(t0, raA);
        ptx::tmem_ld_32x32b_x16(t0 + 16, raB);
        ptx::tmem_ld_wait_dep(raA, raB);
        gelu_stage_ta4<false, true, FOLD>(nullptr, gA, raA, bias, fold);
        gelu_stage_ta4<false, true, FOLD>(nullptr, gA + 4, raA + 8, bias + 32, fold);
        ptx::tmem_ld_32x32b_x16(t0 + 32, raA);
        gelu_stage_ta4<true, true, FOLD>(gA, gB, raB, bias + 64, fold);
        gelu_stage_ta4<true, true, FOLD>(gA + 4, gB + 4, raB + 8, bias + 96, fold);
        ptx::tmem_ld_32x32b_x16(t0 + 48, raB);
        gelu_stage_c8_twice_bf16(gA, pk);
        ptx::mbar_wait(&h_empty[group], ((gc >> 1) & 1) ^ 1);
        store_quarter(0);
        ptx::tmem_ld_wait_dep(raA, raB);
        ptx::tc_fence_before();
        __syncwarp();
        if (lane == 0) ptx::mbar_arrive(&d1_empty[buf]);
        if (tr) ACX_TRACE(1, 4 * hc + 2);
        gelu_stage_ta4<true, true, FOLD>(gB, gA, raA, bias + 128, fold);
        gelu_stage_ta4<true, true, FOLD>(gB + 4, gA + 4, raA + 8, bias + 160, fold);
        gelu_stage_c8_twice_bf16(gB, pk);
        store_quarter(1);
        gelu_stage_ta4<true, true, FOLD>(gA, gB, raB, bias + 192, fold);
        gelu_stage_ta4<true, true, FOLD>(gA + 4, gB + 4, raB + 8, bias + 224, fold);
        gelu_stage_c8_twice_bf16(gA, pk);
        store_quarter(2);
        gelu_stage_ta4<true, false>(gB, nullptr, nullptr, 0);
        gelu_stage_ta4<true, false>(gB + 4, nullptr, nullptr, 0);
        gelu_stage_c8_twice_bf16(gB, pk);
        store_quarter(3);
        ptx::fence_proxy_async_smem();
        __syncwarp();
        if (lane == 0) ptx::mbar_arrive(&h_full[group]);
        if (tr) ACX_TRACE(1, 4 * hc + 3);
      }
    }
  } else if (warp >= 12) {
    const int quad = warp & 3;
    const uint32_t lane_base = tmem_base + (static_cast<uint32_t>(quad * 32) << 16);
    uint8_t* stg = smem + Cfg::OFF_STG + quad * 4096;
    const bool tr = (warp == 12 && lane == 0);
    const int sw64 = (lane >> 1) & 3;
    const int ld_piece = lane & 3, ld_row = lane >> 2;
    auto ln_tile = [&](int j) {
      ptx::mbar_wait(a_full, j & 1);
      const int r = quad * 32 + lane;
      uint8_t* am = smem + Cfg::OFF_AM + r * 128;
      uint8_t* at = smem + Cfg::OFF_AT + r * 64;
      if (GP)
        ln_row_in_smem<C>([&](int ch) { return smem + Cfg::OFF_AM + ch * 2048 + r * 16; }, slnw, slnb);
      else
        ln_row_in_smem<C>([&](int ch) { return ch < 8 ? am + ((ch ^ (r & 7)) << 4) : at + (((ch - 8) ^ ((r >> 1) & 3)) << 4); },
                          slnw, slnb);
      ptx::fence_proxy_async_smem();
      __syncwarp();
      if (lane == 0) ptx::mbar_arrive(a_ready);
    };
    auto stats_tile = [&](int j) {
      ptx::mbar_wait(a_full, j & 1);
      const int r = quad * 32 + lane;
      uint8_t* am = smem + Cfg::OFF_AM + r * 128;
      uint8_t* at = smem + Cfg::OFF_AT + r * 64;
#ifdef ACX_AB_NO_STATS
      sstat[(j & 1) * Cfg::BM + r] = make_float2(1.f, 0.f);
      (void)am;
      (void)at;
#else
      sstat[(j & 1) * Cfg::BM + r] =
          GP ? ln_row_stats_smem<C>([&](int ch) { return smem + Cfg::OFF_AM + ch * 2048 + r * 16; })
             : ln_row_stats_smem<C>([&](int ch) { return ch < 8 ? am + ((ch ^ (r & 7)) << 4) : at + (((ch - 8) ^ ((r >> 1) & 3)) << 4); });
#endif
      __syncwarp();
      if (lane == 0) {
        ptx::mbar_arrive(a_ready);
        ptx::mbar_arrive(a_empty);
      }
    };
    if (FOLD && (int)blockIdx.x < num_tiles) stats_tile(0);
    if (!FOLD && ln && (int)blockIdx.x < num_tiles) ln_tile(0);
    int it = 0;
    for (int tile = blockIdx.x; tile < num_tiles; tile += gridDim.x, ++it) {
      const int row0 = tile * Cfg::BM + quad * 32;
      if (FOLD && tile + (int)gridDim.x < num_tiles) stats_tile(it + 1);
      if (!FOLD && ln && tile + (int)gridDim.x < num_tiles) ln_tile(it + 1);
      auto fetch_resid = [&](int c) {
        uint8_t* dst = stg + (c & 1) * 2048;
#pragma unroll
        for (int q = 0; q < 4; ++q) {
          const int rr = ld_row + 8 * q;
          const int r = row0 + rr;
          const bf16* src = GP ? a.x + ((size_t)(c * 4 + ld_piece) * (((size_t)a.M + 127) / 128 * 128) + (r < a.M ? r : 0)) * 8
                               : a.x + (size_t)(r < a.M ? r : 0) * C + c * 32 + ld_piece * 8;
          const uint32_t d = GP ? ptx::smem_u32(dst + ld_piece * 512 + rr * 16)
                                : ptx::smem_u32(dst + rr * 64 + ((ld_piece ^ ((rr >> 1) & 3)) << 4));
          const int nbytes = r < a.M ? 16 : 0;
          asm volatile("cp.async.ca.shared.global [%0], [%1], 16, %2;" ::"r"(d), "l"(src), "r"(nbytes) : "memory");
        }
        asm volatile("cp.async.commit_group;" ::: "memory");
      };
      if (lane == 0) ptx::tma_store_wait_read<0>();
      __syncwarp();
      fetch_resid(0);
      if (tr) ACX_TRACE(1, 12);
      ptx::mbar_wait(&d2_full[it & 1], (it >> 1) & 1);
      ptx::tc_fence_after();
#pragma unroll
      for (int c = 0; c < 3; ++c) {
        uint8_t* tbuf = stg + (c & 1) * 2048;
        uint32_t r[32];
        ptx::tmem_ld_32x32b_x32(lane_base + Cfg::D2_COL + (it & 1) * Cfg::D2_STRIDE + c * 32, r);
        if (c + 1 < 3) {
          if (c >= 1) {
            if (lane == 0) ptx::tma_store_wait_read<0>();
            __syncwarp();
          }
          fetch_resid(c + 1);
          asm volatile("cp.async.wait_group 1;" ::: "memory");
        } else {
          asm volatile("cp.async.wait_group 0;" ::: "memory");
        }
        ptx::tmem_ld_wait();
        if (c == 2) {
          ptx::tc_fence_before();
          __syncwarp();
          if (lane == 0) ptx::mbar_arrive(&d2_empty[it & 1]);
          if (tr) ACX_TRACE(1, 13);
        }
        __syncwarp();
        uint4 res[4];
#pragma unroll
        for (int j4 = 0; j4 < 4; ++j4)
          res[j4] = *reinterpret_cast<const uint4*>(GP ? tbuf + j4 * 512 + lane * 16 : tbuf + lane * 64 + ((j4 ^ sw64) << 4));
        __syncwarp();
        const int n = c * 32;
#pragma unroll
        for (int j4 = 0; j4 < 4; ++j4) {
          const int j = j4 * 8;
          const float4 bA = *reinterpret_cast<const float4*>(sb2 + n + j);
          const float4 bB = *reinterpret_cast<const float4*>(sb2 + n + j + 4);
          const float4 gA = *reinterpret_cast<const float4*>(sgamma + n + j);
          const float4 gB = *reinterpret_cast<const float4*>(sgamma + n + j + 4);
          float2 f;
          uint4 o;
          f = Pair<bf16>::unpack(res[j4].x);
          o.x = Pair<bf16>::pack(fmaf(gA.x, __uint_as_float(r[j + 0]), bA.x + f.x), fmaf(gA.y, __uint_as_float(r[j + 1]), bA.y + f.y));
          f = Pair<bf16>::unpack(res[j4].y);
          o.y = Pair<bf16>::pack(fmaf(gA.z, __uint_as_float(r[j + 2]), bA.z + f.x), fmaf(gA.w, __uint_as_float(r[j + 3]), bA.w + f.y));
          f = Pair<bf16>::unpack(res[j4].z);
          o.z = Pair<bf16>::pack(fmaf(gB.x, __uint_as_float(r[j + 4]), bB.x + f.x), fmaf(gB.y, __uint_as_float(r[j + 5]), bB.y + f.y));
          f = Pair<bf16>::unpack(res[j4].w);
          o.w = Pair<bf16>::pack(fmaf(gB.z, __uint_as_float(r[j + 6]), bB.z + f.x), fmaf(gB.w, __uint_as_float(r[j + 7]), bB.w + f.y));
          *reinterpret_cast<uint4*>(GP ? tbuf + j4 * 512 + lane * 16 : tbuf + lane * 64 + ((j4 ^ sw64) << 4)) = o;
        }
        ptx::fence_proxy_async_smem();
        __syncwarp();
        if (lane == 0) {
          if (GP) ptx::tma_store_3d(&tmOut, tbuf, 0, row0 >> 5, c * 4);
          else ptx::tma_store_2d(&tmOut, tbuf, n, row0);
          ptx::tma_store_commit();
        }
      }
      if (tr) ACX_TRACE(1, 15);
    }
    if (lane == 0) ptx::tma_store_wait_read<0>();
  }

  ptx::tc_fence_before();
  __syncthreads();
  if (warp == 2) {
    ptx::tc_fence_after();
    ptx::tmem_dealloc(tmem_base, Cfg::TMEM_COLS);
  }
}

static int launch_mlp96_resident(const void* y, void* x, const void* w1, const float* b1, const void* w2,
                                 const float* b2, const float* gamma, int M, const float* ln_w, const float* ln_b,
                                 const float* ln_s, bool gp, cudaStream_t st) {
  using Cfg = Mlp96;
  CUtensorMap tmYm, tmYt, tmW1m, tmW1t, tmW2, tmOut;
  int rc;
  if (gp) {
    rc = make_tmap_gp_bf16(&tmYm, y, (uint64_t)M, 12, 128, 12);
    tmYt = tmYm;
  } else {
    rc = make_tmap_2d_bf16(&tmYm, y, 96, (uint64_t)M, 192, 64, 128);
    if (rc != ACX_OK) return rc;
    rc = make_tmap_2d_bf16(&tmYt, y, 96, (uint64_t)M, 192, 32, 128, CU_TENSOR_MAP_SWIZZLE_64B);
  }
  if (rc != ACX_OK) return rc;
  rc = make_tmap_2d_bf16(&tmW1m, w1, 96, 384, 192, 64, 128);
  if (rc != ACX_OK) return rc;
  rc = make_tmap_2d_bf16(&tmW1t, w1, 96, 384, 192, 32, 128, CU_TENSOR_MAP_SWIZZLE_64B);
  if (rc != ACX_OK) return rc;
  rc = make_tmap_2d_bf16(&tmW2, w2, 384, 96, 768, 64, 96);
  if (rc != ACX_OK) return rc;
  rc = gp ? make_tmap_gp_bf16(&tmOut, x, (uint64_t)M, 12, 32, 4)
          : make_tmap_2d_bf16(&tmOut, x, 96, (uint64_t)M, 192, 32, 32, CU_TENSOR_MAP_SWIZZLE_64B);
  if (rc != ACX_OK) return rc;
  ACX_SET_MAX_SMEM((mlp_fused96_kernel<false, false>), Cfg::SMEM_BYTES);
  ACX_SET_MAX_SMEM((mlp_fused96_kernel<true, false>), Cfg::SMEM_BYTES);
  ACX_SET_MAX_SMEM((mlp_fused96_kernel<true, true>), Cfg::SMEM_BYTES);
  int dev = 0, sms = 0;
  ACX_CUDA(cudaGetDevice(&dev));
  ACX_CUDA(cudaDeviceGetAttribute(&sms, cudaDevAttrMultiProcessorCount, dev));
  const int tiles = ceil_div(M, Cfg::BM);
  MlpArgs a;
  a.x = reinterpret_cast<bf16*>(x);
  a.b1 = b1;
  a.b2 = b2;
  a.gamma = gamma;
  a.M = M;
  a.ln_w = ln_w;
  a.ln_b = ln_b;
  a.ln_s = ln_s;
#ifdef ACX_ENABLE_TRACE
  a.trace = getenv("ACX_TRACE_PTR") ? reinterpret_cast<unsigned long long*>(strtoull(getenv("ACX_TRACE_PTR"), nullptr, 0)) : nullptr;
#else
  a.trace = nullptr;
#endif
  const int grid = tiles < sms ? tiles : sms;
  auto kern = gp && ln_s ? mlp_fused96_kernel<true, true> : gp ? mlp_fused96_kernel<true, false> : mlp_fused96_kernel<false, false>;
  ACX_CUDA(launch_pdl(kern, dim3(grid), dim3(512), Cfg::SMEM_BYTES, st, 1, PDL_MLP, tmYm, tmYt, tmW1m, tmW1t, tmW2, tmOut, a));
  return ACX_OK;
}
// ... 87 lines not shown
```

### audioset-convnext-inf_b200/csrc/ptx.cuh

```cuda
#pragma once
#include <cuda.h>
#include <stdint.h>

namespace acx {
namespace ptx {

__device__ __forceinline__ uint32_t smem_u32(const void* p) {
  return static_cast<uint32_t>(__cvta_generic_to_shared(p));
}

__device__ __forceinline__ bool elect_one() {
  uint32_t pred = 0;
  asm volatile(
      "{\n\t.reg .pred p;\n\t"
      "elect.sync _|p, 0xffffffff;\n\t"
      "selp.u32 %0, 1, 0, p;\n\t}\n"
      : "=r"(pred));
  return pred != 0;
}

__device__ __forceinline__ void mbar_init(uint64_t* bar, uint32_t count) {
  asm volatile("mbarrier.init.shared::cta.b64 [%0], %1;" ::"r"(smem_u32(bar)), "r"(count) : "memory");
}
__device__ __forceinline__ void fence_barrier_init() {
  asm volatile("fence.mbarrier_init.release.cluster;" ::: "memory");
}
__device__ __forceinline__ void mbar_arrive(uint64_t* bar) {
  asm volatile("mbarrier.arrive.shared::cta.b64 _, [%0];" ::"r"(smem_u32(bar)) : "memory");
}
__device__ __forceinline__ void mbar_arrive_expect_tx(uint64_t* bar, uint32_t bytes) {
  asm volatile("mbarrier.arrive.expect_tx.shared::cta.b64 _, [%0], %1;" ::"r"(smem_u32(bar)), "r"(bytes)
               : "memory");
}
#ifndef ACX_MBAR_TIMEOUT_NS
#define ACX_MBAR_TIMEOUT_NS 20000000000ull
#endif
__device__ __forceinline__ bool mbar_try_wait_hint(uint64_t* bar, uint32_t parity, uint32_t ticks) {
  uint32_t ok;
  asm volatile(
      "{\n\t.reg .pred p;\n\t"
      "mbarrier.try_wait.parity.shared::cta.b64 p, [%1], %2, %3;\n\t"
      "selp.u32 %0, 1, 0, p;\n\t}\n"
      : "=r"(ok)
      : "r"(smem_u32(bar)), "r"(parity), "r"(ticks)
      : "memory");
  return ok != 0;
}
__device__ __forceinline__ uint64_t globaltimer_ns() {
  uint64_t t;
  asm volatile("mov.u64 %0, %%globaltimer;" : "=l"(t));
  return t;
}
__device__ __forceinline__ void mbar_wait(uint64_t* bar, uint32_t parity) {
  uint32_t spins = 0;
  uint64_t t0 = 0;
  while (!mbar_try_wait_hint(bar, parity, 0x989680u)) {
    if ((++spins & 63u) == 0) {
      const uint64_t t = globaltimer_ns();
      if (t0 == 0) t0 = t;
      else if (t - t0 > ACX_MBAR_TIMEOUT_NS) {
        printf("acx: mbarrier watchdog block=%d thread=%d bar=%u parity=%u\n", (int)blockIdx.x, (int)threadIdx.x,
               smem_u32(bar), parity);
        __trap();
      }
    }
  }
}

__device__ __forceinline__ void fence_proxy_async_smem() {
  asm volatile("fence.proxy.async.shared::cta;" ::: "memory");
}

__device__ __forceinline__ void prefetch_tensormap(const CUtensorMap* tm) {
  asm volatile("prefetch.tensormap [%0];" ::"l"(reinterpret_cast<uint64_t>(tm)) : "memory");
}
__device__ __forceinline__ void tma_load_2d(void* smem_dst, const CUtensorMap* tm, uint64_t* bar, int c0,
                                            int c1) {
  asm volatile(
      "cp.async.bulk.tensor.2d.shared::cluster.global.mbarrier::complete_tx::bytes [%0], [%1, {%3, %4}], [%2];"
      ::"r"(smem_u32(smem_dst)), "l"(reinterpret_cast<uint64_t>(tm)), "r"(smem_u32(bar)), "r"(c0), "r"(c1)
      : "memory");
}
__device__ __forceinline__ void tma_load_3d(void* smem_dst, const CUtensorMap* tm, uint64_t* bar, int c0, int c1,
                                            int c2) {
  asm volatile(
      "cp.async.bulk.tensor.3d.shared::cluster.global.mbarrier::complete_tx::bytes [%0], [%1, {%3, %4, %5}], [%2];"
      ::"r"(smem_u32(smem_dst)), "l"(reinterpret_cast<uint64_t>(tm)), "r"(smem_u32(bar)), "r"(c0), "r"(c1), "r"(c2)
      : "memory");
}
__device__ __forceinline__ void tma_load_4d(void* smem_dst, const CUtensorMap* tm, uint64_t* bar, int c0,
                                            int c1, int c2, int c3) {
  asm volatile(
      "cp.async.bulk.tensor.4d.shared::cluster.global.mbarrier::complete_tx::bytes [%0], [%1, {%3, %4, %5, %6}], [%2];"
      ::"r"(smem_u32(smem_dst)), "l"(reinterpret_cast<uint64_t>(tm)), "r"(smem_u32(bar)), "r"(c0), "r"(c1),
      "r"(c2), "r"(c3)
      : "memory");
}

__device__ __forceinline__ void tma_prefetch_2d(const CUtensorMap* tm, int c0, int c1) {
  asm volatile("cp.async.bulk.prefetch.tensor.2d.L2.global [%0, {%1, %2}];" ::"l"(reinterpret_cast<uint64_t>(tm)),
               "r"(c0), "r"(c1)
               : "memory");
}
__device__ __forceinline__ void prefetch_l2(const void* p) {
  asm volatile("prefetch.global.L2 [%0];" ::"l"(p));
}

__device__ __forceinline__ void tma_prefetch_3d(const CUtensorMap* tm, int c0, int c1, int c2) {
  asm volatile("cp.async.bulk.prefetch.tensor.3d.L2.global [%0, {%1, %2, %3}];" ::"l"(reinterpret_cast<uint64_t>(tm)),
               "r"(c0), "r"(c1), "r"(c2)
               : "memory");
}
__device__ __forceinline__ void tma_store_3d(const CUtensorMap* tm, const void* smem_src, int c0, int c1, int c2) {
  asm volatile("cp.async.bulk.tensor.3d.global.shared::cta.bulk_group [%0, {%2, %3, %4}], [%1];" ::"l"(
                   reinterpret_cast<uint64_t>(tm)),
               "r"(smem_u32(smem_src)), "r"(c0), "r"(c1), "r"(c2)
               : "memory");
}

__device__ __forceinline__ void tma_store_2d(const CUtensorMap* tm, const void* smem_src, int c0, int c1) {
  asm volatile("cp.async.bulk.tensor.2d.global.shared::cta.bulk_group [%0, {%2, %3}], [%1];" ::"l"(
                   reinterpret_cast<uint64_t>(tm)),
               "r"(smem_u32(smem_src)), "r"(c0), "r"(c1)
               : "memory");
}
__device__ __forceinline__ void tma_store_commit() { asm volatile("cp.async.bulk.commit_group;" ::: "memory"); }
template <int N>
__device__ __forceinline__ void tma_store_wait_read() {
  asm volatile("cp.async.bulk.wait_group.read %0;" ::"n"(N) : "memory");
}

__device__ __forceinline__ void tmem_alloc(uint32_t* smem_out, uint32_t ncols) {
  asm volatile("tcgen05.alloc.cta_group::1.sync.aligned.shared::cta.b32 [%0], %1;" ::"r"(smem_u32(smem_out)),
               "r"(ncols)
               : "memory");
}
__device__ __forceinline__ void tmem_relinquish() {
  asm volatile("tcgen05.relinquish_alloc_permit.cta_group::1.sync.aligned;" ::: "memory");
}
__device__ __forceinline__ void tmem_dealloc(uint32_t taddr, uint32_t ncols) {
  asm volatile("tcgen05.dealloc.cta_group::1.sync.aligned.b32 %0, %1;" ::"r"(taddr), "r"(ncols) : "memory");
}
__device__ __forceinline__ void tc_fence_before() {
  asm volatile("tcgen05.fence::before_thread_sync;" ::: "memory");
}
__device__ __forceinline__ void tc_fence_after() {
  asm volatile("tcgen05.fence::after_thread_sync;" ::: "memory");
}
__device__ __forceinline__ void umma_bf16(uint32_t tmem_d, uint64_t desc_a, uint64_t desc_b, uint32_t idesc,
                                          uint32_t accumulate) {
  asm volatile(
      "{\n\t.reg .pred p;\n\t"
      "setp.ne.b32 p, %4, 0;\n\t"
      "tcgen05.mma.cta_group::1.kind::f16 [%0], %1, %2, %3, p;\n\t}\n"
      ::"r"(tmem_d), "l"(desc_a), "l"(desc_b), "r"(idesc), "r"(accumulate)
      : "memory");
}
__device__ __forceinline__ void umma_commit(uint64_t* bar) {
  asm volatile("tcgen05.commit.cta_group::1.mbarrier::arrive::one.shared::cluster.b64 [%0];" ::"r"(smem_u32(bar))
               : "memory");
}
__device__ __forceinline__ void tmem_ld_32x32b_x32(uint32_t taddr, uint32_t (&r)[32]) {
  asm volatile(
      "tcgen05.ld.sync.aligned.32x32b.x32.b32 "
      "{%0, %1, %2, %3, %4, %5, %6, %7, %8, %9, %10, %11, %12, %13, %14, %15, "
      "%16, %17, %18, %19, %20, %21, %22, %23, %24, %25, %26, %27, %28, %29, %30, %31}, [%32];"
      : "=r"(r[0]), "=r"(r[1]), "=r"(r[2]), "=r"(r[3]), "=r"(r[4]), "=r"(r[5]), "=r"(r[6]), "=r"(r[7]),
        "=r"(r[8]), "=r"(r[9]), "=r"(r[10]), "=r"(r[11]), "=r"(r[12]), "=r"(r[13]), "=r"(r[14]), "=r"(r[15]),
        "=r"(r[16]), "=r"(r[17]), "=r"(r[18]), "=r"(r[19]), "=r"(r[20]), "=r"(r[21]), "=r"(r[22]), "=r"(r[23]),
        "=r"(r[24]), "=r"(r[25]), "=r"(r[26]), "=r"(r[27]), "=r"(r[28]), "=r"(r[29]), "=r"(r[30]), "=r"(r[31])
      : "r"(taddr)
      : "memory");
}
__device__ __forceinline__ void tmem_ld_32x32b_x16(uint32_t taddr, uint32_t (&r)[16]) {
  asm volatile(
      "tcgen05.ld.sync.aligned.32x32b.x16.b32 "
      "{%0, %1, %2, %3, %4, %5, %6, %7, %8, %9, %10, %11, %12, %13, %14, %15}, [%16];"
      : "=r"(r[0]), "=r"(r[1]), "=r"(r[2]), "=r"(r[3]), "=r"(r[4]), "=r"(r[5]), "=r"(r[6]), "=r"(r[7]),
        "=r"(r[8]), "=r"(r[9]), "=r"(r[10]), "=r"(r[11]), "=r"(r[12]), "=r"(r[13]), "=r"(r[14]), "=r"(r[15])
      : "r"(taddr)
      : "memory");
}
__device__ __forceinline__ void tmem_ld_wait() {
  asm volatile("tcgen05.wait::ld.sync.aligned;" ::: "memory");
}
__device__ __forceinline__ void tmem_ld_wait_dep(uint32_t (&r)[16]) {
  asm volatile("tcgen05.wait::ld.sync.aligned;"
               : "+r"(r[0]), "+r"(r[1]), "+r"(r[2]), "+r"(r[3]), "+r"(r[4]), "+r"(r[5]), "+r"(r[6]), "+r"(r[7]),
                 "+r"(r[8]), "+r"(r[9]), "+r"(r[10]), "+r"(r[11]), "+r"(r[12]), "+r"(r[13]), "+r"(r[14]), "+r"(r[15])
               :
               : "memory");
}
__device__ __forceinline__ void tmem_ld_wait_dep(uint32_t (&a)[16], uint32_t (&b)[16]) {
  asm volatile("tcgen05.wait::ld.sync.aligned;"
               : "+r"(a[0]), "+r"(a[1]), "+r"(a[2]), "+r"(a[3]), "+r"(a[4]), "+r"(a[5]), "+r"(a[6]), "+r"(a[7]),
                 "+r"(a[8]), "+r"(a[9]), "+r"(a[10]), "+r"(a[11]), "+r"(a[12]), "+r"(a[13]), "+r"(a[14]), "+r"(a[15]),
                 "+r"(b[0]), "+r"(b[1]), "+r"(b[2]), "+r"(b[3]), "+r"(b[4]), "+r"(b[5]), "+r"(b[6]), "+r"(b[7]),
                 "+r"(b[8]), "+r"(b[9]), "+r"(b[10]), "+r"(b[11]), "+r"(b[12]), "+r"(b[13]), "+r"(b[14]), "+r"(b[15])
               :
               : "memory");
}

constexpr uint32_t kPeerBitMask = 0xFEFFFFFFu;
__device__ __forceinline__ uint32_t cluster_ctarank() {
  uint32_t r;
  asm volatile("mov.u32 %0, %%cluster_ctarank;" : "=r"(r));
  return r;
}
__device__ __forceinline__ void cluster_sync_all() {
  asm volatile("barrier.cluster.arrive.release.aligned;\n\tbarrier.cluster.wait.acquire.aligned;" ::: "memory");
}
__device__ __forceinline__ void tma_load_2d_cg2(void* smem_dst, const CUtensorMap* tm, uint64_t* bar, int c0, int c1) {
  asm volatile(
      "cp.async.bulk.tensor.2d.cta_group::2.shared::cluster.global.mbarrier::complete_tx::bytes [%0], [%1, {%3, %4}], [%2];"
      ::"r"(smem_u32(smem_dst)), "l"(reinterpret_cast<uint64_t>(tm)), "r"(smem_u32(bar) & kPeerBitMask), "r"(c0),
      "r"(c1)
      : "memory");
}
__device__ __forceinline__ void tma_load_3d_cg2(void* smem_dst, const CUtensorMap* tm, uint64_t* bar, int c0, int c1,
                                                int c2) {
  asm volatile(
      "cp.async.bulk.tensor.3d.cta_group::2.shared::cluster.global.mbarrier::complete_tx::bytes [%0], [%1, {%3, %4, %5}], [%2];"
      ::"r"(smem_u32(smem_dst)), "l"(reinterpret_cast<uint64_t>(tm)), "r"(smem_u32(bar) & kPeerBitMask), "r"(c0),
      "r"(c1), "r"(c2)
      : "memory");
}
__device__ __forceinline__ void mbar_arrive_leader(uint64_t* bar) {
  asm volatile("mbarrier.arrive.shared::cluster.b64 _, [%0];" ::"r"(smem_u32(bar) & kPeerBitMask) : "memory");
}
__device__ __forceinline__ void tmem_alloc_cg2(uint32_t* smem_out, uint32_t ncols) {
  asm volatile("tcgen05.alloc.cta_group::2.sync.aligned.shared::cta.b32 [%0], %1;" ::"r"(smem_u32(smem_out)),
               "r"(ncols)
               : "memory");
}
__device__ __forceinline__ void tmem_relinquish_cg2() {
  asm volatile("tcgen05.relinquish_alloc_permit.cta_group::2.sync.aligned;" ::: "memory");
}
__device__ __forceinline__ void tmem_dealloc_cg2(uint32_t taddr, uint32_t ncols) {
  asm volatile("tcgen05.dealloc.cta_group::2.sync.aligned.b32 %0, %1;" ::"r"(taddr), "r"(ncols) : "memory");
}
__device__ __forceinline__ void umma_bf16_cg2(uint32_t tmem_d, uint64_t desc_a, uint64_t desc_b, uint32_t idesc,
                                              uint32_t accumulate) {
  asm volatile(
      "{\n\t.reg .pred p;\n\t"
      "setp.ne.b32 p, %4, 0;\n\t"
      "tcgen05.mma.cta_group::2.kind::f16 [%0], %1, %2, %3, p;\n\t}\n"
      ::"r"(tmem_d), "l"(desc_a), "l"(desc_b), "r"(idesc), "r"(accumulate)
      : "memory");
}
__device__ __forceinline__ void umma_commit_cg2(uint64_t* bar) {
  asm volatile(
      "{\n\t.reg .b16 m;\n\tmov.b16 m, 3;\n\t"
      "tcgen05.commit.cta_group::2.mbarrier::arrive::one.shared::cluster.multicast::cluster.b64 [%0], m;\n\t}\n"
      ::"r"(smem_u32(bar))
      : "memory");
}

__device__ __forceinline__ uint64_t umma_desc_sw128_kmajor(uint32_t smem_addr) {
  uint64_t d = 0;
  d |= static_cast<uint64_t>((smem_addr & 0x3FFFFu) >> 4);
  d |= static_cast<uint64_t>(1) << 16;
  d |= static_cast<uint64_t>(1024 >> 4) << 32;
  d |= static_cast<uint64_t>(1) << 46;
  d |= static_cast<uint64_t>(2) << 61;
  return d;
}
__device__ __forceinline__ uint64_t umma_desc_sw64_kmajor(uint32_t smem_addr) {
  uint64_t d = 0;
  d |= static_cast<uint64_t>((smem_addr & 0x3FFFFu) >> 4);
  d |= static_cast<uint64_t>(1) << 16;
  d |= static_cast<uint64_t>(512 >> 4) << 32;
  d |= static_cast<uint64_t>(1) << 46;
  d |= static_cast<uint64_t>(4) << 61;
  return d;
}
__device__ __forceinline__ uint64_t umma_desc_nosw_kmajor(uint32_t smem_addr, uint32_t k_stride, uint32_t mn_stride) {
  uint64_t d = 0;
  d |= static_cast<uint64_t>((smem_addr & 0x3FFFFu) >> 4);
  d |= static_cast<uint64_t>((k_stride >> 4) & 0x3FFFu) << 16;
  d |= static_cast<uint64_t>((mn_stride >> 4) & 0x3FFFu) << 32;
  d |= static_cast<uint64_t>(1) << 46;
  return d;
}
__host__ __device__ constexpr uint32_t umma_idesc_f16(int m, int n) {
  return (1u << 4) | (static_cast<uint32_t>(n >> 3) << 17) | (static_cast<uint32_t>(m >> 4) << 24);
}
__host__ __device__ constexpr uint32_t umma_idesc_bf16(int m, int n) {
  return (1u << 4) | (1u << 7) | (1u << 10) | (static_cast<uint32_t>(n >> 3) << 17) |
         (static_cast<uint32_t>(m >> 4) << 24);
}

}
}
```

### audioset-convnext-inf_b200/engine.py

```python
import collections
import os

import torch

from . import _native as N

DEPTHS = (3, 3, 9, 3)
DIMS = (96, 192, 384, 768)
N_FFT, HOP, N_MELS, N_BINS, N_CLASSES = 1024, 320, 224, 513, 527
BN0_EPS = 1e-5
FE_SCALE_LOG2 = 8


def _p(t):
    return 0 if t is None else t.data_ptr()


class PackedWeights:

    def __init__(self, sd, device, precision):
        assert precision in ("bf16", "fp32")
        self.precision = precision
        self.device = device
        adt = torch.bfloat16 if precision == "bf16" else torch.float32
        self.act_dtype = adt
        f32 = dict(device=device, dtype=torch.float32)

        def g(key):
            return sd[key].detach().to(**f32)

        conv_real = g("spectrogram_extractor.stft.conv_real.weight")[:, 0, :]
        conv_imag = g("spectrogram_extractor.stft.conv_imag.weight")[:, 0, :]
        melW = g("logmel_extractor.melW")
        assert conv_real.shape == (N_BINS, N_FFT) and melW.shape == (N_BINS, N_MELS), \
            "only the n_fft=1024 / 224-mel front end of convnext_tiny is supported"
        scale = g("bn0.weight") / torch.sqrt(g("bn0.running_var") + BN0_EPS)
        self.bn_scale = scale.contiguous()
        self.bn_shift = (g("bn0.bias") - g("bn0.running_mean") * scale).contiguous()
        self.dft_f32 = torch.cat([conv_real, conv_imag], 0).contiguous()
        self.melT = melW.t().contiguous()
        nz = melW != 0
        idx = torch.arange(N_BINS, device=device)[:, None].expand(N_BINS, N_MELS)
        big = torch.full_like(idx, N_BINS)
        lo = torch.where(nz, idx, big).min(0).values
        hi = torch.where(nz, idx + 1, torch.zeros_like(idx)).max(0).values
        lo = torch.minimum(lo, hi)
        self.mel_lo = lo.to(torch.int32).contiguous()
        self.mel_hi = hi.to(torch.int32).contiguous()
        used = nz.any(1).nonzero().flatten()
        k_end = int(used.max().item()) + 1 if used.numel() else 1
        self.n_chunks = (k_end + 63) // 64
        if precision == "bf16":
            nb = self.n_chunks * 64
            re = torch.zeros(nb, N_FFT, **f32)
            im = torch.zeros(nb, N_FFT, **f32)
            m = min(nb, N_BINS)
            re[:m], im[:m] = conv_real[:m], conv_imag[:m]
            dft = torch.stack([re.view(self.n_chunks, 64, N_FFT), im.view(self.n_chunks, 64, N_FFT)], 1)
            dft = dft.reshape(self.n_chunks * 128, N_FFT)
            self.dft_hi, self.dft_lo = _split_f16(dft * float(1 << FE_SCALE_LOG2))
            self.dftf = fold_dft_weights(conv_real, conv_imag, self.n_chunks)
            if self.dftf is not None:
                self.dftf_hi, self.dftf_lo = _split_f16(self.dftf * float(1 << FE_SCALE_LOG2))
            mw = torch.zeros(nb, 256, **f32)
            mw[:m, :N_MELS] = melW[:m]
            mel = mw.view(self.n_chunks, 64, 256).transpose(1, 2).reshape(self.n_chunks * 256, 64)
            self.melc_hi, self.melc_lo = _split_bf16(mel)

        self.stem_w = g("downsample_layers.0.0.weight").reshape(DIMS[0], 16).t().contiguous()
        self.stem_b = g("downsample_layers.0.0.bias").contiguous()
        self.stem_ln_w = g("downsample_layers.0.1.weight").contiguous()
        self.stem_ln_b = g("downsample_layers.0.1.bias").contiguous()

        self.ds = []
        for i in range(1, 4):
            w = g(f"downsample_layers.{i}.1.weight")
            cout, cin = w.shape[0], w.shape[1]
            self.ds.append(dict(
                ln_w=g(f"downsample_layers.{i}.0.weight").contiguous(),
                ln_b=g(f"downsample_layers.{i}.0.bias").contiguous(),
                w=w.permute(0, 2, 3, 1).reshape(cout, 4 * cin).to(adt).contiguous(),
                b=g(f"downsample_layers.{i}.1.bias").contiguous()))
            if precision == "bf16":
                self.ds[-1]["w_fused"] = pack_downsample_weight(w).to(adt).contiguous()

        self.blocks = []
        for s in range(4):
            C = DIMS[s]
            stage = []
            for j in range(DEPTHS[s]):
                p = f"stages.{s}.{j}."
                stage.append(dict(
                    dw_w=g(p + "dwconv.weight").reshape(C, 49).t().to(adt).contiguous(),
                    dw_b=g(p + "dwconv.bias").contiguous(),
                    ln_w=g(p + "norm.weight").contiguous(), ln_b=g(p + "norm.bias").contiguous(),
                    w1=g(p + "pwconv1.weight").to(adt).contiguous(), b1=g(p + "pwconv1.bias").contiguous(),
                    w2=g(p + "pwconv2.weight").to(adt).contiguous(), b2=g(p + "pwconv2.bias").contiguous(),
                    gamma=g(p + "gamma").contiguous()))
                if precision == "bf16" and s < 3:
                    stage[-1].update(fold_layernorm_into_pwconv1(g(p + "pwconv1.weight"), g(p + "pwconv1.bias"),
                                                                 g(p + "norm.weight"), g(p + "norm.bias")))
            self.blocks.append(stage)

        self.norm_w, self.norm_b = g("norm.weight").contiguous(), g("norm.bias").contiguous()
        self.fc_w, self.fc_b = g("head_audioset.weight").contiguous(), g("head_audioset.bias").contiguous()


def fold_layernorm_into_pwconv1(w1, b1, ln_w, ln_b):
    w1f = (w1.double() * ln_w.double()[None, :]).to(torch.float32).to(torch.bfloat16).contiguous()
    return dict(w1f=w1f, s1=w1f.double().sum(1).to(torch.float32).contiguous(),
                b1f=(b1.double() + w1.double() @ ln_b.double()).to(torch.float32).contiguous())


def fold_dft_weights(conv_real, conv_imag, n_chunks, tol=1e-6):
    n_bins, n_fft = conv_real.shape
    h = n_fft // 2
    scale = max(conv_real.abs().max().item(), conv_imag.abs().max().item(), 1e-30)
    mir = torch.arange(n_fft - 1, h, -1, device=conv_real.device)
    asym = max((conv_real[:, 1:h] - conv_real[:, mir]).abs().max().item(), (conv_imag[:, 1:h] + conv_imag[:, mir]).abs().max().item(),
               conv_real[:, 0].abs().max().item(), conv_imag[:, 0].abs().max().item(), conv_imag[:, h].abs().max().item())
    if asym > tol * scale:
        return None
    fre = torch.zeros(n_bins, h, device=conv_real.device, dtype=torch.float32)
    fim = torch.zeros_like(fre)
    fre[:, 0] = conv_real[:, h]
    fre[:, 1:] = 0.5 * (conv_real[:, 1:h] + conv_real[:, mir])
    fim[:, 1:] = 0.5 * (conv_imag[:, 1:h] - conv_imag[:, mir])
    n_pairs = (n_chunks + 1) // 2
    out = torch.zeros(n_pairs, 4, 64, h, device=conv_real.device, dtype=torch.float32)
    for c in range(n_chunks):
        lo, hi = 64 * c, min(64 * c + 64, n_bins)
        if hi > lo:
            out[c // 2, c % 2, : hi - lo] = fre[lo:hi]
            out[c // 2, 2 + c % 2, : hi - lo] = fim[lo:hi]
    return out.reshape(n_pairs * 256, h).contiguous()


def pack_downsample_weight(w):
    cout, cin = w.shape[0], w.shape[1]
    return w.reshape(cout, cin // 8, 8, 2, 2).permute(0, 3, 1, 4, 2).reshape(cout, 4 * cin)


def _split_f16(x):
    hi = x.to(torch.float16)
    lo = (x - hi.to(torch.float32)).to(torch.float16)
    return hi.contiguous(), lo.contiguous()


def _split_bf16(x):
    hi = x.to(torch.bfloat16)
    lo = (x - hi.to(torch.float32)).to(torch.bfloat16)
    return hi.contiguous(), lo.contiguous()


def out_time_dims(L):
    T = L // HOP + 1
    H0 = (T + 4) // 4 + 1
    hs = [H0, H0 // 2, (H0 // 2) // 2, ((H0 // 2) // 2) // 2]
    return T, hs


MIN_RAGGED_LEN = 7360


def check_lengths(lengths, B, L):
    if isinstance(lengths, torch.Tensor):
        if lengths.device.type != "cpu":
            raise ValueError("lengths must be a host sequence or a CPU tensor")
        lengths = lengths.tolist()
    try:
        ls = [int(n) for n in lengths]
    except (TypeError, ValueError) as e:
        raise ValueError(f"lengths must be a sequence of integers: {e}") from e
    if len(ls) != B:
        raise ValueError(f"lengths has {len(ls)} entries for a batch of {B} clips")
    bad = [n for n in ls if not MIN_RAGGED_LEN <= n <= L]
    if bad:
        raise ValueError(f"every length must lie in [{MIN_RAGGED_LEN}, {L}] (the canvas), got {bad[:4]}")
    return ls


def ragged_table(lengths):
    rows = []
    for n in lengths:
        T, hs = out_time_dims(n)
        rows.append([n, T] + hs)
    return torch.tensor(rows, dtype=torch.int32).t().contiguous()


class Engine:
    def __init__(self, state_dict, device, precision="bf16", chunk=None, frontend=None, mlp=None):
        self.lib = N.load()
        self.device = torch.device(device)
        if self.device.type != "cuda":
            raise N.NativeError("the B200 engine needs a CUDA device; there is no CPU path")
        with torch.cuda.device(self.device):
            if not self.lib.acx_device_ok():
                raise N.NativeError(N.last_error())
        self.precision = precision
        self.w = PackedWeights(state_dict, self.device, precision)
        self.adt = N.ACX_BF16 if precision == "bf16" else N.ACX_F32
        self.esize = 2 if precision == "bf16" else 4
        self.chunk = int(chunk or os.environ.get("ACX_CHUNK", 64 if precision == "bf16" else 4))
        self.frontend = frontend or os.environ.get("ACX_FRONTEND", "fused" if precision == "bf16" else "simt")
        if self.frontend == "folded" and getattr(self.w, "dftf", None) is None:
            self.frontend = "fused"
        self.mlp = mlp or os.environ.get("ACX_MLP", "fused")
        self.dwconv = os.environ.get("ACX_DWCONV", "tc" if precision == "bf16" else "simt")
        self.dwconv_tc_stages = tuple(int(c) for c in os.environ.get("ACX_DWCONV_TC_STAGES", "012"))
        self.gp = os.environ.get("ACX_GP", "1") == "1"
        self.ln_mode = os.environ.get("ACX_LN", "fused")
        self.ds_fused = os.environ.get("ACX_DS_FUSED", "1") == "1"
        self.ds_fused_widths = tuple(int(c) for c in os.environ.get("ACX_DS_FUSED_C", "96,192").split(",") if c)
        if precision == "fp32":
            self.frontend, self.mlp, self.dwconv = "simt", "gemm", "simt"
        self._ws = collections.OrderedDict()
        self.max_workspaces = int(os.environ.get("ACX_WORKSPACES", 4))
        self.graph_after = int(os.environ.get("ACX_GRAPH_AFTER", 2))
        self.use_graph = os.environ.get("ACX_GRAPH", "1") == "1" and precision == "bf16"
        self._prof = None
        self._prof_only = None
        self.launches = 0

    def _workspace(self, n, L):
        key = (n, L)
        ws = self._ws.get(key)
        if ws is not None:
            self._ws.move_to_end(key)
            return ws
        T, hs = out_time_dims(L)
        dev = self.device
        adt = self.w.act_dtype
        ld_pad = (max(L + N_FFT, HOP * (T + 3)) + 7) // 8 * 8
        ws = dict(T=T, hs=hs, ld_pad=ld_pad)
        if self.frontend == "folded":
            ws["f_hi"] = torch.empty(n, T, N_FFT, device=dev, dtype=torch.float16)
            ws["f_lo"] = torch.empty(n, T, N_FFT, device=dev, dtype=torch.float16)
        elif self.frontend == "fused":
            ws["wav_hi"] = torch.empty(n, ld_pad, device=dev, dtype=torch.float16)
            ws["wav_lo"] = torch.empty(n, ld_pad, device=dev, dtype=torch.float16)
        else:
            ws["wav_pad"] = torch.empty(n, ld_pad, device=dev, dtype=torch.float32)
            ws["spec"] = torch.empty(n * T, 2 * N_BINS, device=dev, dtype=torch.float32)
        ws["logmel"] = torch.empty(n, T, N_MELS, device=dev, dtype=torch.float32)
        m0 = n * hs[0] * 56
        pad = 128 * DIMS[1]
        ws["x"] = torch.empty(m0 * DIMS[0] + pad, device=dev, dtype=adt)
        ws["y"] = torch.empty(m0 * DIMS[0] + pad, device=dev, dtype=adt)
        ws["hid"] = torch.empty(m0 * 4 * DIMS[0], device=dev, dtype=adt)
        if self.precision == "bf16":
            ws["xg"] = torch.empty(m0 * DIMS[0] + pad, device=dev, dtype=adt)
            ws["stats"] = torch.empty(n * hs[2] * 14 + 128, 2, device=dev, dtype=torch.float32)
        ws["pooled"] = torch.empty(n, DIMS[3], device=dev, dtype=torch.float32)
        ws["scene"] = torch.empty(n, DIMS[3], device=dev, dtype=torch.float32)
        ws["logits"] = torch.empty(n, N_CLASSES, device=dev, dtype=torch.float32)
        ws["probs"] = torch.empty(n, N_CLASSES, device=dev, dtype=torch.float32)
        ws["frame"] = torch.empty(n, DIMS[3], hs[3], 7, device=dev, dtype=torch.float32)
        ws["valid"] = torch.empty(6 * n, device=dev, dtype=torch.int32)
        ws["offsets"] = torch.empty(n, device=dev, dtype=torch.int64)
        ws["graphs"] = {}
        ws["uses"] = {}
        while len(self._ws) >= max(1, self.max_workspaces):
            self._ws.popitem(last=False)
        self._ws[key] = ws
# ... 3 lines not shown
        self.launches += 1
        if self._prof is None or (self._prof_only is not None and not tag.startswith(self._prof_only)):
            N.call(name, *args)
            return
        e0, e1 = torch.cuda.Event(enable_timing=True), torch.cuda.Event(enable_timing=True)
        e0.record()
        N.call(name, *args)
        e1.record()
        self._prof.append((tag, e0, e1))

    def _call_v(self, tag, name, valid, *args):
        if valid:
            self._call(tag, name + "_ragged", *args[:-1], valid, args[-1])
        else:
            self._call(tag, name, *args)

    def profile(self, wave, want=("logits",)):
        self.start_timing(None)
        self.run(wave, want)
        return self.stop_timing()

    def start_timing(self, only=None):
        self._prof, self._prof_only = [], only

    def stop_timing(self):
        torch.cuda.synchronize(self.device)
        res = [(tag, e0.elapsed_time(e1)) for tag, e0, e1 in self._prof]
        self._prof, self._prof_only = None, None
        return res

    def algorithmic_work(self, tag, n, L):
        T, hs = out_time_dims(L)
        es = self.esize
        if tag.startswith("ds_fused_c"):
            C = int(tag[len("ds_fused_c"):])
            s = DIMS.index(C)
            return "hbm", 1.0 * n * es * (hs[s] * (56 >> s) * C + hs[s + 1] * (28 >> s) * 2 * C)
        if tag.startswith(("pw1_gelu", "pw2_resid", "ds_")):
            K, Nn = (int(t[1:]) for t in tag.split("_")[-2:])
            C = {"pw1_gelu": K, "pw2_resid": Nn, "ds": K // 4}[tag.rsplit("_", 2)[0]]
            s = DIMS.index(C)
            M = n * (hs[s + 1] * (28 >> s) if tag.startswith("ds_") else hs[s] * (56 >> s))
            return "tensor", 2.0 * M * Nn * K
        if tag.startswith("mlp_fused_c"):
            C = int(tag[len("mlp_fused_c"):])
            s = DIMS.index(C)
            return "tensor", 2.0 * (n * hs[s] * (56 >> s)) * C * 4 * C * 2
        if tag.startswith("row_stats_c"):
            C = int(tag.rsplit("_c", 1)[1])
            s = DIMS.index(C)
            return "hbm", 1.0 * n * hs[s] * (56 >> s) * C * es
        if tag.startswith(("dwconv_tc_c", "ln_rows_c", "to_gp_c")):
            C = int(tag.rsplit("_c", 1)[1])
            s = DIMS.index(C)
            return "hbm", 2.0 * n * hs[s] * (56 >> s) * C * es
        if tag.startswith("dwconv_ln_c"):
            C = int(tag[len("dwconv_ln_c"):])
            s = DIMS.index(C)
            return "hbm", 2.0 * n * hs[s] * (56 >> s) * C * es
        if tag.startswith("ln_patchify_c"):
            C = int(tag[len("ln_patchify_c"):])
            s = DIMS.index(C)
            return "hbm", 2.0 * n * hs[s] * (56 >> s) * C * es
        if tag in ("frontend_fused", "frontend_folded"):
            return "tensor", n * T * 2.0 * (N_FFT * 2 * N_BINS + N_BINS * N_MELS)
        if tag == "dft_simt":
            return "tensor", n * T * 2.0 * N_FFT * 2 * N_BINS
        if tag == "stem":
            return "hbm", n * (T * N_MELS * 4.0 + hs[0] * 56 * DIMS[0] * es)
        if tag == "frame_fold":
            return "hbm", n * L * 4.0 + n * T * N_FFT * 4.0
        if tag == "wave_prep":
            return "hbm", n * L * 4.0 + n * (L + N_FFT) * 4.0
        if tag == "head":
            return "hbm", n * hs[3] * 7 * DIMS[3] * es + N_CLASSES * DIMS[3] * 4.0
        return "hbm", 0.0

    def _wave_prep(self, wave, ws, n, L, st, rv=None, windows=False):
        ld_pad = ws["ld_pad"]
        fn = "acx_wave_prep_pcm16" if wave.dtype == torch.int16 else "acx_wave_prep"
        if self.frontend == "folded":
            fn = "acx_frame_fold_pcm16" if wave.dtype == torch.int16 else "acx_frame_fold"
            args = (ws["f_hi"].data_ptr(), ws["f_lo"].data_ptr(), n, L, ws["T"], N_FFT, HOP)
            tag = "frame_fold"
        elif self.frontend == "fused":
            args = (ws["wav_hi"].data_ptr(), ws["wav_lo"].data_ptr(), n, L, N_FFT, ld_pad, N.ACX_BF16)
            tag = "wave_prep"
        else:
            args = (ws["wav_pad"].data_ptr(), 0, n, L, N_FFT, ld_pad, N.ACX_F32)
            tag = "wave_prep"
        if windows:
            self._call(tag, fn + "_windows", wave.data_ptr(), wave.numel(), ws["offsets"].data_ptr(), rv[0] if rv else 0,
                       *args, st)
        elif rv:
            self._call(tag, fn + "_ragged", wave.data_ptr(), *args, L, rv[0], st)
        else:
            self._call(tag, fn, wave.data_ptr(), *args, st)

    def _frontend(self, ws, n, L, st):
        w = self.w
        T, ld_pad = ws["T"], ws["ld_pad"]
        if self.frontend == "folded":
            self._call("frontend_folded", "acx_frontend_folded", ws["f_hi"].data_ptr(), ws["f_lo"].data_ptr(), w.dftf_hi.data_ptr(),
                       w.dftf_lo.data_ptr(), w.melc_hi.data_ptr(), w.melc_lo.data_ptr(), w.n_chunks, w.bn_scale.data_ptr(),
                       w.bn_shift.data_ptr(), ws["logmel"].data_ptr(), n, T, N_FFT, N_MELS, st)
        elif self.frontend == "fused":
            self._call("frontend_fused", "acx_frontend_fused", ws["wav_hi"].data_ptr(), ws["wav_lo"].data_ptr(), ld_pad,
                   w.dft_hi.data_ptr(), w.dft_lo.data_ptr(), w.melc_hi.data_ptr(), w.melc_lo.data_ptr(), w.n_chunks,
                   w.bn_scale.data_ptr(), w.bn_shift.data_ptr(), ws["logmel"].data_ptr(), n, T, N_FFT, HOP, N_MELS, st)
        else:
            self._call("dft_simt", "acx_gemm_f32", ws["wav_pad"].data_ptr(), ld_pad, T, HOP, w.dft_f32.data_ptr(),
                   ws["spec"].data_ptr(), 2 * N_BINS, n * T, 2 * N_BINS, N_FFT, N.EPI_BIAS, 0, 0, 0, st)
            self._call("power_mel_log", "acx_power_mel_log", ws["spec"].data_ptr(), 2 * N_BINS, N_BINS, w.melT.data_ptr(),
                   w.mel_lo.data_ptr(), w.mel_hi.data_ptr(), w.bn_scale.data_ptr(), w.bn_shift.data_ptr(),
                   ws["logmel"].data_ptr(), n * T, N_MELS, st)

    def _gemm(self, a, wt, out, M, Nn, K, epi, bias, gamma, resid, st):
        tag = f"{('ds', 'pw1_gelu', 'pw2_resid')[epi]}_k{K}_n{Nn}"
        if self.precision == "bf16":
            self._call(tag, "acx_gemm_bf16", a, wt, out, M, Nn, K, epi, bias, gamma, resid, st)
        else:
            self._call(tag, "acx_gemm_f32", a, M * K, M, K, wt, out, Nn, M, Nn, K, epi, bias, gamma, resid, st)

    def _trunk(self, ws, n, st, rv=None):
        w = self.w
        x, y, hid = ws["x"].data_ptr(), ws["y"].data_ptr(), ws["hid"].data_ptr()
        xgp = ws["xg"].data_ptr() if "xg" in ws else 0
        fused0 = self.mlp == "fused" and self.dwconv == "tc" and 0 in self.dwconv_tc_stages and self.gp
        stem_gp = fused0 and os.environ.get("ACX_STEM", "") != "simt"
        rT = rv[1] if rv else 0
        if stem_gp:
            self._call_v("stem", "acx_stem_gp", rT, ws["logmel"].data_ptr(), w.stem_w.data_ptr(), w.stem_b.data_ptr(),
                         w.stem_ln_w.data_ptr(), w.stem_ln_b.data_ptr(), xgp, n, ws["T"], N_MELS, st)
        else:
            self._call_v("stem", "acx_stem", rT, ws["logmel"].data_ptr(), w.stem_w.data_ptr(), w.stem_b.data_ptr(),
                         w.stem_ln_w.data_ptr(), w.stem_ln_b.data_ptr(), x, n, ws["T"], N_MELS, self.adt, st)
        Wd = 56
        entered_gp = False
        for s in range(4):
            C, H = DIMS[s], ws["hs"][s]
            rh = rv[2 + s] if rv else 0
            M = n * H * Wd
            fused_mlp = self.mlp == "fused" and C in (96, 192)
            tc = self.dwconv == "tc" and s in self.dwconv_tc_stages
            gp = tc and fused_mlp and self.gp and Wd in (56, 28)
            gp2 = tc and not fused_mlp and self.gp and self.mlp == "fused" and Wd == 14 and C == 384
            if gp2:
                xg, vg = xgp, y
                if not entered_gp:
                    self._call(f"to_gp_c{C}", "acx_gp_transpose", x, xg, M, C, 1, st)
                stats = ws["stats"].data_ptr()
                for blk in w.blocks[s]:
                    self._call_v(f"dwconv_tc_c{C}", "acx_dwconv_tc_gp", rh, xg, blk["dw_w"].data_ptr(), blk["dw_b"].data_ptr(), vg, n, H, Wd, C, st)
                    self._call(f"row_stats_c{C}", "acx_gp_row_stats", vg, stats, M, C, st)
                    self._call(f"pw1_gelu_k{C}_n{4 * C}", "acx_gemm_bf16_pw1_gp", vg, blk["w1f"].data_ptr(), hid, M, 4 * C, C,
                               blk["b1f"].data_ptr(), stats, blk["s1"].data_ptr(), st)
                    self._call(f"pw2_resid_k{4 * C}_n{C}", "acx_gemm_bf16_pw2_gp", hid, blk["w2"].data_ptr(), xg, M, C, 4 * C,
                               blk["b2"].data_ptr(), blk["gamma"].data_ptr(), st)
            elif gp:
                xg, vg = xgp, x
                if not (s == 0 and stem_gp) and not entered_gp:
                    self._call(f"to_gp_c{C}", "acx_gp_transpose", x, xg, M, C, 1, st)
            for blk in (() if gp2 else w.blocks[s]):
                if gp:
                    self._call_v(f"dwconv_tc_c{C}", "acx_dwconv_tc_gp", rh, xg, blk["dw_w"].data_ptr(), blk["dw_b"].data_ptr(), vg, n, H, Wd, C, st)
                    if self.ln_mode == "smem":
                        self._call(f"mlp_fused_c{C}", "acx_mlp_fused_gp", vg, xg, blk["ln_w"].data_ptr(), blk["ln_b"].data_ptr(), 0,
                                   blk["w1"].data_ptr(), blk["b1"].data_ptr(), blk["w2"].data_ptr(), blk["b2"].data_ptr(),
                                   blk["gamma"].data_ptr(), M, C, st)
                    else:
                        self._call(f"mlp_fused_c{C}", "acx_mlp_fused_gp", vg, xg, 0, 0, blk["s1"].data_ptr(),
                                   blk["w1f"].data_ptr(), blk["b1f"].data_ptr(), blk["w2"].data_ptr(), blk["b2"].data_ptr(),
                                   blk["gamma"].data_ptr(), M, C, st)
                    continue
                ln_fused = False
                if tc:
                    self._call_v(f"dwconv_tc_c{C}", "acx_dwconv_tc", rh, x, blk["dw_w"].data_ptr(), blk["dw_b"].data_ptr(), y, n, H, Wd, C, st)
                    ln_fused = fused_mlp and self.ln_mode == "fused"
                    if not ln_fused:
                        self._call(f"ln_rows_c{C}", "acx_layernorm_rows", y, blk["ln_w"].data_ptr(), blk["ln_b"].data_ptr(), y, M, C, st)
                else:
                    self._call_v(f"dwconv_ln_c{C}", "acx_dwconv_ln", rh, x, blk["dw_w"].data_ptr(), blk["dw_b"].data_ptr(),
                                 blk["ln_w"].data_ptr(), blk["ln_b"].data_ptr(), y, n, H, Wd, C, self.adt, st)
                if ln_fused:
                    self._call(f"mlp_fused_c{C}", "acx_mlp_fused_ln", y, x, blk["ln_w"].data_ptr(), blk["ln_b"].data_ptr(),
                               blk["w1"].data_ptr(), blk["b1"].data_ptr(), blk["w2"].data_ptr(), blk["b2"].data_ptr(),
                               blk["gamma"].data_ptr(), M, C, st)
                elif fused_mlp:
                    self._call(f"mlp_fused_c{C}", "acx_mlp_fused", y, x, blk["w1"].data_ptr(), blk["b1"].data_ptr(), blk["w2"].data_ptr(),
                           blk["b2"].data_ptr(), blk["gamma"].data_ptr(), M, C, st)
                else:
                    self._gemm(y, blk["w1"].data_ptr(), hid, M, 4 * C, C, N.EPI_BIAS_GELU, blk["b1"].data_ptr(), 0, 0, st)
                    self._gemm(hid, blk["w2"].data_ptr(), x, M, C, 4 * C, N.EPI_BIAS_SCALE_RESID,
                               blk["b2"].data_ptr(), blk["gamma"].data_ptr(), x, st)
            if s < 3:
                d = w.ds[s]
                entered_gp = (self.precision == "bf16" and self.mlp == "fused" and 2 * C in (96, 192, 384) and self.dwconv == "tc"
                              and (s + 1) in self.dwconv_tc_stages and self.gp and Wd // 2 in (56, 28, 14)
                              and os.environ.get("ACX_DS_GP", "1") == "1")
                if (gp or gp2) and self.ds_fused and C in self.ds_fused_widths:
                    self._call(f"ds_fused_c{C}", "acx_downsample_fused_gp", xg, d["ln_w"].data_ptr(), d["ln_b"].data_ptr(),
                               d["w_fused"].data_ptr(), d["b"].data_ptr(), y if entered_gp else x, n, H, Wd, C, 1 if entered_gp else 0, st)
                    if entered_gp:
                        xgp, y = y, xgp
                    Wd //= 2
                    continue
                if gp or gp2:
                    self._call(f"ln_patchify_c{C}", "acx_ln_patchify_gp", xg, d["ln_w"].data_ptr(), d["ln_b"].data_ptr(), y, n, H, Wd, C, st)
                else:
                    self._call(f"ln_patchify_c{C}", "acx_ln_patchify", x, d["ln_w"].data_ptr(), d["ln_b"].data_ptr(), y, n, H, Wd, C, self.adt, st)
                Wd //= 2
                Mo = n * ws["hs"][s + 1] * Wd
                if entered_gp:
                    self._call(f"ds_k{4 * C}_n{2 * C}", "acx_gemm_bf16_gp_out", y, d["w"].data_ptr(), xgp, Mo, 2 * C, 4 * C,
                               d["b"].data_ptr(), st)
                else:
                    self._gemm(y, d["w"].data_ptr(), x, Mo, 2 * C, 4 * C, N.EPI_BIAS, d["b"].data_ptr(), 0, 0, st)

    @staticmethod
    def _ragged_ptrs(ws, n, ragged):
        if not ragged:
            return None
        base = ws["valid"].data_ptr()
        return [base + 4 * k * n for k in range(6)]

    def _body(self, ws, n, L, st, trunk, need_head, need_frame, ragged=False):
        rv = self._ragged_ptrs(ws, n, ragged)
        self._frontend(ws, n, L, st)
        if not trunk:
            return
        self._trunk(ws, n, st, rv)
        x = ws["x"].data_ptr()
        h3 = ws["hs"][3]
        rh3 = rv[5] if rv else 0
        if need_head:
            w = self.w
            self._call_v("head", "acx_head", rh3, x, w.norm_w.data_ptr(), w.norm_b.data_ptr(), w.fc_w.data_ptr(),
                         w.fc_b.data_ptr(), ws["pooled"].data_ptr(), ws["scene"].data_ptr(), ws["logits"].data_ptr(),
                         ws["probs"].data_ptr(), n, h3, 7, DIMS[3], N_CLASSES, self.adt, st)
        if need_frame:
            self._call_v("frame_nchw", "acx_nhwc_to_nchw_f32", rh3, x, ws["frame"].data_ptr(), n, h3, 7, DIMS[3], self.adt, st)

    def _capture(self, ws, n, L, trunk, need_head, need_frame, ragged=False):
        st = torch.cuda.current_stream(self.device).cuda_stream
        before = self.launches
        self._body(ws, n, L, st, trunk, need_head, need_frame, ragged)
        per_replay = self.launches - before
        torch.cuda.synchronize(self.device)
        g = torch.cuda.CUDAGraph()
        with torch.cuda.graph(g):
            cst = torch.cuda.current_stream(self.device).cuda_stream
            self._body(ws, n, L, cst, trunk, need_head, need_frame, ragged)
        self.launches = before
        return g, per_replay

    def run(self, wave, want=("logits",), lengths=None):
        assert wave.is_cuda and wave.dim() == 2 and wave.is_contiguous()
        assert wave.dtype in (torch.float32, torch.int16), "waveform must be float32 or int16 PCM"
        B, L = wave.shape
        T, hs = out_time_dims(L)
        if hs[3] < 1:
            raise ValueError(f"clip of {L} samples is too short for the 4-stage trunk")
        ragged = lengths is not None
        if ragged:
            lengths = check_lengths(lengths, B, L)
            if "logmel" in want:
                raise ValueError("a ragged batch has no log-mel output (its rows past each clip's end are not masked)")
            if wave.dtype != torch.float32:
                raise ValueError("a ragged batch takes a float32 waveform")
        dev = self.device
        out = {}
        need_head = "logits" in want or "scene" in want
        f32 = dict(device=dev, dtype=torch.float32)
        with torch.cuda.device(dev):
            st = torch.cuda.current_stream(dev).cuda_stream
            if need_head:
                out["scene"] = torch.empty(B, DIMS[3], **f32)
                out["logits"] = torch.empty(B, N_CLASSES, **f32)
                out["probs"] = torch.empty(B, N_CLASSES, **f32)
            if "frame" in want:
                out["frame"] = torch.empty(B, DIMS[3], hs[3], 7, **f32)
            if "logmel" in want:
                out["logmel"] = torch.empty(B, T, N_MELS, **f32)
            for b0 in range(0, B, self.chunk):
                n = min(self.chunk, B - b0)
                ws = self._workspace(min(self.chunk, B), L)
                self._run_chunk(ws, n, L, st, want, lengths[b0:b0 + n] if ragged else None,
                                lambda rv: self._wave_prep(wave[b0:b0 + n], ws, n, L, st, rv))
                for name in ("logmel", "scene", "logits", "probs", "frame"):
                    if name in out:
                        out[name][b0:b0 + n].copy_(ws[name][:n])
        return out

    def _run_chunk(self, ws, n, L, st, want, lengths, prep):
        ragged = lengths is not None
        rv = None
        if ragged:
            tab = ragged_table(lengths).pin_memory()
            ws["valid"][:6 * n].view(6, n).copy_(tab, non_blocking=True)
            rv = self._ragged_ptrs(ws, n, True)
        prep(rv)
        need_head = "logits" in want or "scene" in want
        trunk = need_head or "frame" in want
        key = (n, L, trunk, need_head, "frame" in want, ragged)
        g = ws["graphs"].get(key) if (self.use_graph and self._prof is None) else None
        if g is None and self.use_graph and self._prof is None:
            ws["uses"][key] = ws["uses"].get(key, 0) + 1
            if ws["uses"][key] >= self.graph_after:
                g = ws["graphs"][key] = self._capture(ws, n, L, *key[2:])
# ... 47 lines not shown
```

### include/acx.h

```cpp
#ifndef ACX_H_
#define ACX_H_

#include <stddef.h>
#include <stdint.h>

#ifdef __cplusplus
extern "C" {
#endif

#define ACX_VERSION 100
#define ACX_API __attribute__((visibility("default")))

enum { ACX_OK = 0, ACX_ERR_ARG = 1, ACX_ERR_CUDA = 2, ACX_ERR_UNSUPPORTED = 3, ACX_ERR_WORKSPACE = 4 };
enum { ACX_BF16 = 0, ACX_F32 = 1 };

enum {
  ACX_EPI_BIAS = 0,
  ACX_EPI_BIAS_GELU = 1,
  ACX_EPI_BIAS_SCALE_RESID = 2
};

ACX_API int acx_version(void);
ACX_API const char* acx_last_error(void);
ACX_API int acx_device_ok(void);


#define ACX_FE_SCALE_LOG2 8

ACX_API int acx_wave_prep(const float* wave, void* hi, void* lo, int B, int L, int n_fft, int ld_pad,
                  int act_dtype, void* stream);

ACX_API int acx_wave_prep_pcm16(const int16_t* pcm, void* hi, void* lo, int B, int L, int n_fft, int ld_pad,
                        int act_dtype, void* stream);

ACX_API int acx_power_mel_log(const float* spec, int ld_spec, int n_bins, const float* melT, const int32_t* mel_lo,
                      const int32_t* mel_hi, const float* bn_scale, const float* bn_shift, float* out,
                      int rows, int n_mels, void* stream);

ACX_API int acx_frame_fold(const float* wave, void* f_hi, void* f_lo, int B, int L, int T, int n_fft, int hop, void* stream);
ACX_API int acx_frame_fold_pcm16(const int16_t* pcm, void* f_hi, void* f_lo, int B, int L, int T, int n_fft, int hop, void* stream);
ACX_API int acx_frontend_folded(const void* f_hi, const void* f_lo, const void* w_hi, const void* w_lo, const void* mel_hi,
                        const void* mel_lo, int n_chunks, const float* bn_scale, const float* bn_shift, float* out,
                        int B, int T, int n_fft, int n_mels, void* stream);

ACX_API int acx_frontend_fused(const void* hi, const void* lo, int ld_pad, const void* dft_hi, const void* dft_lo,
                       const void* mel_hi, const void* mel_lo, int n_chunks, const float* bn_scale,
                       const float* bn_shift, float* out, int B, int T, int n_fft, int hop, int n_mels,
                       void* stream);

ACX_API int acx_stem(const float* logmel, const float* w, const float* bias, const float* ln_w, const float* ln_b,
             void* out, int B, int T, int n_mels, int act_dtype, void* stream);
ACX_API int acx_stem_gp(const float* logmel, const float* w, const float* bias, const float* ln_w, const float* ln_b,
                void* out, int B, int T, int n_mels, void* stream);

ACX_API int acx_dwconv_ln(const void* x, const void* w, const float* bias, const float* ln_w, const float* ln_b,
                  void* y, int B, int H, int W, int C, int act_dtype, void* stream);

ACX_API int acx_dwconv_tc(const void* x, const void* w, const float* bias, void* v, int B, int H, int W, int C,
                  void* stream);
ACX_API int acx_layernorm_rows(const void* in, const float* ln_w, const float* ln_b, void* out, long long M, int C,
                       void* stream);

ACX_API int acx_dwconv_tc_gp(const void* x, const void* w, const float* bias, void* v, int B, int H, int W, int C,
                     void* stream);
ACX_API int acx_gp_transpose(const void* in, void* out, long long M, int C, int to_gp, void* stream);
ACX_API int acx_gp_row_stats(const void* v, float* stats, long long M, int C, void* stream);

ACX_API int acx_ln_patchify(const void* x, const float* ln_w, const float* ln_b, void* a, int B, int H, int W, int C,
                    int act_dtype, void* stream);
ACX_API int acx_ln_patchify_gp(const void* x, const float* ln_w, const float* ln_b, void* a, int B, int H, int W, int C,
                       void* stream);

ACX_API int acx_downsample_fused_gp(const void* x, const float* ln_w, const float* ln_b, const void* w, const float* bias,
                            void* out, int B, int H, int W, int C, int out_gp, void* stream);

ACX_API int acx_gemm_bf16(const void* A, const void* W, void* out, int M, int N, int K, int epilogue,
                  const float* bias, const float* gamma, const void* resid, void* stream);
ACX_API int acx_gemm_bf16_gp_out(const void* A, const void* W, void* out, int M, int N, int K, const float* bias,
                         void* stream);
ACX_API int acx_gemm_bf16_pw1_gp(const void* v_gp, const void* w1f, void* hid, int M, int N, int K, const float* b1f,
                         const float* stats, const float* ln_s, void* stream);
ACX_API int acx_gemm_bf16_pw2_gp(const void* hid, const void* w2, void* x_gp, int M, int N, int K, const float* b2,
                         const float* gamma, void* stream);
ACX_API int acx_gemm_f32(const float* A, long long batch_stride, int rows_per_batch, int row_stride, const float* W,
                 float* out, int ldo, int M, int N, int K, int epilogue, const float* bias,
                 const float* gamma, const float* resid, void* stream);

ACX_API int acx_mlp_fused(const void* y, void* x, const void* w1, const float* b1, const void* w2, const float* b2,
                  const float* gamma, int M, int C, void* stream);
ACX_API int acx_mlp_fused_ln(const void* v, void* x, const float* ln_w, const float* ln_b, const void* w1,
                     const float* b1, const void* w2, const float* b2, const float* gamma, int M, int C,
                     void* stream);
ACX_API int acx_mlp_fused_gp(const void* v, void* x, const float* ln_w, const float* ln_b, const float* ln_s,
                     const void* w1, const float* b1, const void* w2, const float* b2, const float* gamma, int M, int C,
                     void* stream);

ACX_API int acx_head(const void* x, const float* ln_w, const float* ln_b, const float* fc_w, const float* fc_b,
             float* pooled, float* scene, float* logits, float* probs, int B, int H, int W, int C, int n_cls,
             int act_dtype, void* stream);

ACX_API int acx_nhwc_to_nchw_f32(const void* x, float* out, int B, int H, int W, int C, int act_dtype, void* stream);

ACX_API int acx_wave_prep_ragged(const float* wave, void* hi, void* lo, int B, int L, int n_fft, int ld_pad, int act_dtype,
                                 int ld_wave, const int32_t* valid, void* stream);
ACX_API int acx_frame_fold_ragged(const float* wave, void* f_hi, void* f_lo, int B, int L, int T, int n_fft, int hop,
                                  int ld_wave, const int32_t* valid, void* stream);
ACX_API int acx_stem_ragged(const float* logmel, const float* w, const float* bias, const float* ln_w, const float* ln_b,
                            void* out, int B, int T, int n_mels, int act_dtype, const int32_t* valid, void* stream);
ACX_API int acx_stem_gp_ragged(const float* logmel, const float* w, const float* bias, const float* ln_w, const float* ln_b,
                               void* out, int B, int T, int n_mels, const int32_t* valid, void* stream);
ACX_API int acx_dwconv_tc_ragged(const void* x, const void* w, const float* bias, void* v, int B, int H, int W, int C,
                                 const int32_t* valid, void* stream);
ACX_API int acx_dwconv_tc_gp_ragged(const void* x, const void* w, const float* bias, void* v, int B, int H, int W, int C,
                                    const int32_t* valid, void* stream);
ACX_API int acx_dwconv_ln_ragged(const void* x, const void* w, const float* bias, const float* ln_w, const float* ln_b,
                                 void* y, int B, int H, int W, int C, int act_dtype, const int32_t* valid, void* stream);
ACX_API int acx_head_ragged(const void* x, const float* ln_w, const float* ln_b, const float* fc_w, const float* fc_b,
                            float* pooled, float* scene, float* logits, float* probs, int B, int H, int W, int C, int n_cls,
                            int act_dtype, const int32_t* valid, void* stream);
ACX_API int acx_nhwc_to_nchw_f32_ragged(const void* x, float* out, int B, int H, int W, int C, int act_dtype,
                                        const int32_t* valid, void* stream);

ACX_API int acx_wave_prep_windows(const float* rec, long long rec_len, const long long* offsets, const int32_t* valid,
                                  void* hi, void* lo, int B, int L, int n_fft, int ld_pad, int act_dtype, void* stream);
ACX_API int acx_wave_prep_pcm16_windows(const int16_t* rec, long long rec_len, const long long* offsets,
                                        const int32_t* valid, void* hi, void* lo, int B, int L, int n_fft, int ld_pad,
                                        int act_dtype, void* stream);
ACX_API int acx_frame_fold_windows(const float* rec, long long rec_len, const long long* offsets, const int32_t* valid,
                                   void* f_hi, void* f_lo, int B, int L, int T, int n_fft, int hop, void* stream);
ACX_API int acx_frame_fold_pcm16_windows(const int16_t* rec, long long rec_len, const long long* offsets,
                                         const int32_t* valid, void* f_hi, void* f_lo, int B, int L, int T, int n_fft,
                                         int hop, void* stream);

ACX_API int acx_resample_fit(const float* x, int ld_in, const float* taps, float* out, int ld_out, int B, int L_in,
                     int orig, int newf, int width, int n_out, void* stream);

#ifdef __cplusplus
}
#endif
#endif
```

Before: 13760.

## Fold LayerNorm mean correction into pwconv1 GEMM as rank-1 MMA term

The LayerNorm mean-shift term (-mean * rowsum(W)) is now computed on the tensor cores. Each row's negative mean and each weight column's row-sum are split into three bf16 parts, and the product is added either as an extra K=8 slice in the GEMM or as an extra UMMA issue in the fused MLP. The GELU epilogue then only applies rstd with an FMA plus bias, which removes one FMA and one shared load per element. The cost is an extra MMA per tile, extra shared memory for the rank-1 planes, and a wider K with alignment checks (K % 64 == 8). It also risks precision loss, since the three-way bf16 split only approximates the float values.

```diff
diff --git a/audioset-convnext-inf_b200/_native.py b/audioset-convnext-inf_b200/_native.py
--- a/audioset-convnext-inf_b200/_native.py
+++ b/audioset-convnext-inf_b200/_native.py
@@ -31,12 +31,14 @@
     "acx_dwconv_tc_gp": [_vp, _vp, _vp, _vp, _i, _i, _i, _i, _vp],
     "acx_gp_transpose": [_vp, _vp, _ll, _i, _i, _vp],
     "acx_gp_row_stats": [_vp, _vp, _ll, _i, _vp],
+    "acx_gp_row_stats_rank1": [_vp, _vp, _ll, _i, _vp],
     "acx_ln_patchify_gp": [_vp, _vp, _vp, _vp, _i, _i, _i, _i, _vp],
     "acx_ln_patchify": [_vp, _vp, _vp, _vp, _i, _i, _i, _i, _i, _vp],
     "acx_downsample_fused_gp": [_vp, _vp, _vp, _vp, _vp, _vp, _i, _i, _i, _i, _i, _vp],
     "acx_gemm_bf16": [_vp, _vp, _vp, _i, _i, _i, _i, _vp, _vp, _vp, _vp],
     "acx_gemm_bf16_gp_out": [_vp, _vp, _vp, _i, _i, _i, _vp, _vp],
     "acx_gemm_bf16_pw1_gp": [_vp, _vp, _vp, _i, _i, _i, _vp, _vp, _vp, _vp],
+    "acx_gemm_bf16_pw1_gp_rank1": [_vp, _vp, _vp, _i, _i, _i, _vp, _vp, _vp],
     "acx_gemm_bf16_pw2_gp": [_vp, _vp, _vp, _i, _i, _i, _vp, _vp, _vp],
     "acx_gemm_f32": [_vp, _ll, _i, _i, _vp, _vp, _i, _i, _i, _i, _i, _vp, _vp, _vp, _vp],
     "acx_mlp_fused": [_vp, _vp, _vp, _vp, _vp, _vp, _vp, _i, _i, _vp],
diff --git a/audioset-convnext-inf_b200/csrc/common.cuh b/audioset-convnext-inf_b200/csrc/common.cuh
--- a/audioset-convnext-inf_b200/csrc/common.cuh
+++ b/audioset-convnext-inf_b200/csrc/common.cuh
@@ -154,7 +154,7 @@
   unsigned long long rstd2, nmr2;
   uint32_t sb1_base, sbs_base;
 };
-template <bool kT, bool kA, bool kFold = false>
+template <bool kT, bool kA, bool kFold = false, bool kRstd = false>
 __device__ __forceinline__ void gelu_stage_ta4(GeluPair* t, GeluPair* a, const uint32_t* acc, uint32_t sbias_addr,
                                                const LnFold fold = LnFold{}) {
   const unsigned long long k50 = f2_pack(50.0f, 50.0f);
@@ -167,11 +167,7 @@
 #pragma unroll
     for (int i = 0; i < 4; ++i) {
       float2 b;
-#ifdef ACX_AB_NO_FOLD_EPI
-      if (false) {
-#else
       if (kFold) {
-#endif
         float2 sj;
         asm("ld.shared.v4.f32 {%0, %1, %2, %3}, [%4];"
             : "=f"(b.x), "=f"(b.y), "=f"(sj.x), "=f"(sj.y)
@@ -183,9 +179,15 @@
                      : "l"(fold.rstd2), "l"(f2_pack(__uint_as_float(acc[2 * i]), __uint_as_float(acc[2 * i + 1]))), "l"(tt));
       } else {
         asm("ld.shared.v2.f32 {%0, %1}, [%2];" : "=f"(b.x), "=f"(b.y) : "r"(sbias_addr + 8 * i));
-        asm volatile("add.rn.f32x2 %0, %1, %2;"
-                     : "=l"(a[i].x)
-                     : "l"(f2_pack(__uint_as_float(acc[2 * i]), __uint_as_float(acc[2 * i + 1]))), "l"(f2_pack(b.x, b.y)));
+        if (kRstd)
+          asm volatile("fma.rn.f32x2 %0, %1, %2, %3;"
+                       : "=l"(a[i].x)
+                       : "l"(fold.rstd2), "l"(f2_pack(__uint_as_float(acc[2 * i]), __uint_as_float(acc[2 * i + 1]))),
+                         "l"(f2_pack(b.x, b.y)));
+        else
+          asm volatile("add.rn.f32x2 %0, %1, %2;"
+                       : "=l"(a[i].x)
+                       : "l"(f2_pack(__uint_as_float(acc[2 * i]), __uint_as_float(acc[2 * i + 1]))), "l"(f2_pack(b.x, b.y)));
       }
     }
   }
@@ -225,16 +227,16 @@
                  : "l"(o[i]));
 }
 
-template <bool kTwice, bool kFold = false>
+template <bool kTwice, bool kFold = false, bool kRstd = false>
 __device__ __forceinline__ void bias_gelu_tile16_sp(const uint32_t* __restrict__ acc ,
                                                     const float* __restrict__ sbias , float2 (&out)[16],
                                                     const LnFold fold = LnFold{}) {
   GeluPair g[16];
   const uint32_t sb = static_cast<uint32_t>(__cvta_generic_to_shared(sbias));
-  gelu_stage_ta4<false, true, kFold>(nullptr, g, acc, sb, fold);
-  gelu_stage_ta4<true, true, kFold>(g, g + 4, acc + 8, sb + 32, fold);
-  gelu_stage_ta4<true, true, kFold>(g + 4, g + 8, acc + 16, sb + 64, fold);
-  gelu_stage_ta4<true, true, kFold>(g + 8, g + 12, acc + 24, sb + 96, fold);
+  gelu_stage_ta4<false, true, kFold, kRstd>(nullptr, g, acc, sb, fold);
+  gelu_stage_ta4<true, true, kFold, kRstd>(g, g + 4, acc + 8, sb + 32, fold);
+  gelu_stage_ta4<true, true, kFold, kRstd>(g + 4, g + 8, acc + 16, sb + 64, fold);
+  gelu_stage_ta4<true, true, kFold, kRstd>(g + 8, g + 12, acc + 24, sb + 96, fold);
   gelu_stage_ta4<true, false>(g + 12, nullptr, nullptr, 0);
   const unsigned long long khalf = f2_pack(0.5f, 0.5f);
 #pragma unroll
@@ -246,4 +248,24 @@
   }
 }
 
-}
+__device__ __forceinline__ void split3_bf16(float v, uint32_t (&h)[3]) {
+  const bf16 a = __float2bfloat16_rn(v);
+  const float r1 = v - __bfloat162float(a);
+  const bf16 b = __float2bfloat16_rn(r1);
+  const bf16 c = __float2bfloat16_rn(r1 - __bfloat162float(b));
+  h[0] = __bfloat16_as_ushort(a);
+  h[1] = __bfloat16_as_ushort(b);
+  h[2] = __bfloat16_as_ushort(c);
+}
+__device__ __forceinline__ uint4 rank1_a_row(float neg_mean) {
+  uint32_t m[3];
+  split3_bf16(neg_mean, m);
+  return make_uint4(m[0] | m[0] << 16, m[0] | m[1] << 16, m[1] | m[1] << 16, m[2] | m[2] << 16);
+}
+__device__ __forceinline__ uint4 rank1_b_row(float s) {
+  uint32_t t[3];
+  split3_bf16(s, t);
+  return make_uint4(t[0] | t[1] << 16, t[2] | t[0] << 16, t[1] | t[2] << 16, t[0] | t[1] << 16);
+}
+
+}
diff --git a/audioset-convnext-inf_b200/csrc/dwconv_tc.cu b/audioset-convnext-inf_b200/csrc/dwconv_tc.cu
--- a/audioset-convnext-inf_b200/csrc/dwconv_tc.cu
+++ b/audioset-convnext-inf_b200/csrc/dwconv_tc.cu
@@ -771,8 +771,9 @@
 
 namespace acx {
 namespace dwtc {
+template <bool kRank1>
 __global__ void __launch_bounds__(128) gp_row_stats_kernel(const uint4* __restrict__ v, float2* __restrict__ stats,
-                                                           long long M, int G) {
+                                                           uint4* __restrict__ rank1_plane, long long M, int G) {
   pdl_trigger();
   pdl_wait();
   const long long row = (long long)blockIdx.x * blockDim.x + threadIdx.x;
@@ -804,6 +805,7 @@
   const float var = fmaxf((q.x + q.y) * inv_c - md * md, 0.f);
   const float rstd = rsqrtf(var + 1e-6f);
   stats[row] = make_float2(rstd, -(md + shift) * rstd);
+  if (kRank1) rank1_plane[row] = rank1_a_row(-(md + shift));
 }
 }
 }
@@ -811,8 +813,20 @@
 extern "C" int acx_gp_row_stats(const void* v, float* stats, long long M, int C, void* stream) {
   ACX_CHECK(v && stats, ACX_ERR_ARG, "gp_row_stats: null pointer");
   ACX_CHECK(M > 0 && C > 0 && C % 8 == 0, ACX_ERR_ARG, "gp_row_stats: bad shape M=%lld C=%d", M, C);
-  ACX_CUDA(launch_pdl(dwtc::gp_row_stats_kernel, dim3((unsigned)((M + 127) / 128)), dim3(128), 0, reinterpret_cast<cudaStream_t>(stream),
-                      1, PDL_STATS, reinterpret_cast<const uint4*>(v), reinterpret_cast<float2*>(stats), M, C / 8));
+  ACX_CUDA(launch_pdl(dwtc::gp_row_stats_kernel<false>, dim3((unsigned)((M + 127) / 128)), dim3(128), 0,
+                      reinterpret_cast<cudaStream_t>(stream), 1, PDL_STATS, reinterpret_cast<const uint4*>(v),
+                      reinterpret_cast<float2*>(stats), static_cast<uint4*>(nullptr), M, C / 8));
+  return ACX_OK;
+}
+
+extern "C" int acx_gp_row_stats_rank1(void* v, float* stats, long long M, int C, void* stream) {
+  ACX_CHECK(v && stats, ACX_ERR_ARG, "gp_row_stats_rank1: null pointer");
+  ACX_CHECK(M > 0 && C > 0 && C % 8 == 0, ACX_ERR_ARG, "gp_row_stats_rank1: bad shape M=%lld C=%d", M, C);
+  const long long Mp = (M + 127) / 128 * 128;
+  uint4* vv = reinterpret_cast<uint4*>(v);
+  ACX_CUDA(launch_pdl(dwtc::gp_row_stats_kernel<true>, dim3((unsigned)((M + 127) / 128)), dim3(128), 0,
+                      reinterpret_cast<cudaStream_t>(stream), 1, PDL_STATS, static_cast<const uint4*>(vv),
+                      reinterpret_cast<float2*>(stats), vv + (long long)(C / 8) * Mp, M, C / 8));
   return ACX_OK;
 }
 
diff --git a/audioset-convnext-inf_b200/csrc/gemm_umma.cu b/audioset-convnext-inf_b200/csrc/gemm_umma.cu
--- a/audioset-convnext-inf_b200/csrc/gemm_umma.cu
+++ b/audioset-convnext-inf_b200/csrc/gemm_umma.cu
@@ -19,6 +19,7 @@
   int reverse;
 };
 constexpr int ACX_EPI_BIAS_GELU_FOLD = 3;
+constexpr int ACX_EPI_BIAS_GELU_RSTD = 4;
 
 template <int BN_, int NEPI_, int CG_ = 1>
 struct GemmCfg {
@@ -219,7 +220,7 @@
       };
       fetch_resid(0);
       LnFold fold{0ull, 0ull, ptx::smem_u32(sbias), ptx::smem_u32(sbias)};
-      if (EPI == ACX_EPI_BIAS_GELU_FOLD) {
+      if (EPI == ACX_EPI_BIAS_GELU_FOLD || EPI == ACX_EPI_BIAS_GELU_RSTD) {
         const int r = row0 + lane;
         const float2 stt = r < g.M ? __ldg(g.stats + r) : make_float2(0.f, 0.f);
         fold.rstd2 = f2_pack(stt.x, stt.x);
@@ -251,6 +252,14 @@
           if (EPI == ACX_EPI_BIAS_GELU_FOLD) {
             float2 o[16];
             bias_gelu_tile16_sp<false, true>(r, sbias + n, o, fold);
+#pragma unroll
+            for (int j = 0; j < 16; ++j) {
+              v[2 * j] = o[j].x;
+              v[2 * j + 1] = o[j].y;
+            }
+          } else if (EPI == ACX_EPI_BIAS_GELU_RSTD) {
+            float2 o[16];
+            bias_gelu_tile16_sp<false, false, true>(r, sbias + n, o, fold);
 #pragma unroll
             for (int j = 0; j < 16; ++j) {
               v[2 * j] = o[j].x;
@@ -405,8 +414,9 @@
   if (epilogue == ACX_EPI_BIAS_SCALE_RESID)
     ACX_CHECK(gamma && resid, ACX_ERR_ARG, "gemm_bf16: scale+residual epilogue needs gamma and resid");
   ACX_CHECK(!out_gp || epilogue != ACX_EPI_BIAS_GELU, ACX_ERR_UNSUPPORTED, "gemm_bf16: the hidden activation stays row-major");
-  ACX_CHECK(!a_gp || K % 64 == 0, ACX_ERR_UNSUPPORTED, "gemm_bf16: a planar A operand needs K %% 64 == 0 (got %d)", K);
-  ACX_CHECK((stats == nullptr) == (ln_s == nullptr), ACX_ERR_ARG, "gemm_bf16: stats and ln_s go together");
+  const bool rank1 = stats && !ln_s;
+  ACX_CHECK(!a_gp || K % 64 == (rank1 ? 8 : 0), ACX_ERR_UNSUPPORTED, "gemm_bf16: a planar A operand needs K %% 64 == %d (got %d)",
+            rank1 ? 8 : 0, K);
   ACX_CHECK(!stats || epilogue == ACX_EPI_BIAS_GELU, ACX_ERR_UNSUPPORTED, "gemm_bf16: the LayerNorm fold belongs to the GELU epilogue");
   GemmArgs g;
   g.out = reinterpret_cast<bf16*>(out);
@@ -430,6 +440,7 @@
   switch (epilogue) {
     case ACX_EPI_BIAS: return dispatch_bn<ACX_EPI_BIAS>(tmA, W, g, st);
     case ACX_EPI_BIAS_GELU:
+      if (rank1) return dispatch_bn<ACX_EPI_BIAS_GELU_RSTD>(tmA, W, g, st);
       return stats ? dispatch_bn<ACX_EPI_BIAS_GELU_FOLD>(tmA, W, g, st) : dispatch_bn<ACX_EPI_BIAS_GELU>(tmA, W, g, st);
     case ACX_EPI_BIAS_SCALE_RESID: return dispatch_bn<ACX_EPI_BIAS_SCALE_RESID>(tmA, W, g, st);
     default:
@@ -453,6 +464,12 @@
   ACX_CHECK(stats && ln_s, ACX_ERR_ARG, "gemm_bf16_pw1_gp: stats and ln_s are required");
   return gemm_bf16_impl(v_gp, w1f, hid, M, N, K, ACX_EPI_BIAS_GELU, b1f, nullptr, nullptr, 0, 1, stats, ln_s, stream);
 }
+
+extern "C" int acx_gemm_bf16_pw1_gp_rank1(const void* v_gp, const void* w1x, void* hid, int M, int N, int K, const float* b1f,
+                                          const float* stats, void* stream) {
+  ACX_CHECK(stats, ACX_ERR_ARG, "gemm_bf16_pw1_gp_rank1: stats are required");
+  return gemm_bf16_impl(v_gp, w1x, hid, M, N, K, ACX_EPI_BIAS_GELU, b1f, nullptr, nullptr, 0, 1, stats, nullptr, stream);
+}
 extern "C" int acx_gemm_bf16_pw2_gp(const void* hid, const void* w2, void* x_gp, int M, int N, int K, const float* b2,
                                     const float* gamma, void* stream) {
   return gemm_bf16_impl(hid, w2, x_gp, M, N, K, ACX_EPI_BIAS_SCALE_RESID, b2, gamma, x_gp, 1, 0, nullptr, nullptr, stream);
diff --git a/audioset-convnext-inf_b200/csrc/mlp_fused.cu b/audioset-convnext-inf_b200/csrc/mlp_fused.cu
--- a/audioset-convnext-inf_b200/csrc/mlp_fused.cu
+++ b/audioset-convnext-inf_b200/csrc/mlp_fused.cu
@@ -83,8 +83,26 @@
   const float md = (s.x + s.y) * (1.0f / C);
   const float var = fmaxf((q.x + q.y) * (1.0f / C) - md * md, 0.f);
   const float rstd = rsqrtf(var + 1e-6f);
-  return make_float2(rstd, -(md + shift) * rstd);
+  return make_float2(rstd, -(md + shift));
 }
+
+template <int HD, int A_BUFS>
+struct Rank1 {
+  static constexpr int BYTES = (A_BUFS * 128 + HD + 128) * 16;
+  static constexpr int ZERO = (A_BUFS * 128 + HD) * 16;
+  __device__ static __forceinline__ void build(uint8_t* region, const float* __restrict__ ln_s) {
+    uint4* b = reinterpret_cast<uint4*>(region + A_BUFS * 128 * 16);
+    for (int i = threadIdx.x; i < HD + 128; i += blockDim.x) b[i] = i < HD ? rank1_b_row(ln_s[i]) : make_uint4(0u, 0u, 0u, 0u);
+    ptx::fence_proxy_async_smem();
+  }
+  __device__ static __forceinline__ uint64_t desc_a(uint32_t region, int buf) {
+    return ptx::umma_desc_nosw_kmajor(region + buf * 128 * 16, ZERO - buf * 128 * 16, 128);
+  }
+  __device__ static __forceinline__ uint64_t desc_b(uint32_t region, int n0) {
+    const int off = (A_BUFS * 128 + n0) * 16;
+    return ptx::umma_desc_nosw_kmajor(region + off, ZERO - off, 128);
+  }
+};
 
 template <int C_>
 struct MlpCfg {
@@ -105,9 +123,11 @@
   static constexpr int OFF_STG = OFF_H + 2 * KB2 * H_TILE;
   static constexpr int STG_TILE = 32 * 64;
   static constexpr int STG_PER_WARP = STG_TILE;
-  static constexpr int OFF_BAR = OFF_STG + 8 * STG_PER_WARP;
+  using R1 = Rank1<HD, A_BUFS>;
+  static constexpr int OFF_R1 = OFF_STG + 8 * STG_PER_WARP;
+  static constexpr int OFF_BAR = OFF_R1 + R1::BYTES;
   static constexpr int OFF_VEC = OFF_BAR + 512;
-  static constexpr int SMEM_BYTES = OFF_VEC + (3 * HD + 4 * C) * 4 + 2 * BM * 8 + 1024;
+  static constexpr int SMEM_BYTES = OFF_VEC + (HD + 4 * C) * 4 + 2 * BM * 4 + 1024;
   static constexpr int D2_COL = 0, D1_COL = 256, TMEM_COLS = 512;
   static constexpr int OUT_CHUNKS = C / 32;
   static constexpr int OUT_G0 = (OUT_CHUNKS + 1) / 2;
@@ -145,15 +165,10 @@
   float* sgamma = sb2 + C;
   float* slnw = sgamma + C;
   float* slnb = slnw + C;
-  float* ss1 = slnb + C;
-  float2* sstat = reinterpret_cast<float2*>(ss1 + 2 * Cfg::HD);
+  float* sstat = slnb + C;
   const bool ln = a.ln_w != nullptr;
   for (int i = threadIdx.x; i < Cfg::HD; i += blockDim.x) sb1[i] = a.b1[i];
-  if (FOLD)
-    for (int i = threadIdx.x; i < Cfg::HD; i += blockDim.x) {
-      ss1[4 * (i >> 1) + (i & 1)] = a.b1[i];
-      ss1[4 * (i >> 1) + 2 + (i & 1)] = a.ln_s[i];
-    }
+  if (FOLD) Cfg::R1::build(smem + Cfg::OFF_R1, a.ln_s);
   if (ln)
     for (int i = threadIdx.x; i < C; i += blockDim.x) {
       slnw[i] = a.ln_w[i];
@@ -312,6 +327,14 @@
             ptx::umma_commit(&ring_empty[slot]);
             advance();
           }
+          if (FOLD) {
+            if (h == 0) {
+              ptx::mbar_wait(&a_ready[abuf], ause & 1);
+              ptx::tc_fence_after();
+            }
+            const uint32_t r1 = ptx::smem_u32(smem + Cfg::OFF_R1);
+            ptx::umma_bf16(d1, Cfg::R1::desc_a(r1, abuf), Cfg::R1::desc_b(r1, h * Cfg::NH), idesc1, 1u);
+          }
           ptx::umma_commit(&d1_full[db1]);
           if (h == Cfg::NC - 1) ptx::umma_commit(&a_empty[abuf]);
           if (h >= 1) gemm2(h - 1, gc - 1);
@@ -327,7 +350,7 @@
     const int row_in_tile = quad * 32 + lane;
     const uint32_t lane_base = tmem_base + (static_cast<uint32_t>(quad * 32) << 16);
     uint32_t gc = 0;
-    LnFold fold{0ull, 0ull, ptx::smem_u32(sb1), ptx::smem_u32(ss1)};
+    LnFold fold{};
     int it1 = 0;
     for (int tile = blockIdx.x; tile < num_tiles; tile += gridDim.x, ++it1) {
       for (int h = 0; h < Cfg::NC; ++h, ++gc) {
@@ -340,9 +363,8 @@
         if (FOLD && h == 0) {
           const int abuf = it1 % Cfg::A_BUFS;
           ptx::mbar_wait(&a_ready[abuf], (it1 / Cfg::A_BUFS) & 1);
-          const float2 stt = sstat[(it1 & 1) * Cfg::BM + row_in_tile];
-          fold.rstd2 = f2_pack(stt.x, stt.x);
-          fold.nmr2 = f2_pack(stt.y, stt.y);
+          const float rstd = sstat[(it1 & 1) * Cfg::BM + row_in_tile];
+          fold.rstd2 = f2_pack(rstd, rstd);
         }
         uint8_t* hrow = smem + Cfg::OFF_H + (buf * Cfg::KB2 + group) * Cfg::H_TILE + row_in_tile * 128;
         uint32_t ra[32];
@@ -353,7 +375,7 @@
           uint32_t packed[16];
           {
             float2 o[16];
-            bias_gelu_tile16_sp<true, FOLD>(ra, bias + 32 * half, o, fold);
+            bias_gelu_tile16_sp<true, false, FOLD>(ra, bias + 32 * half, o, fold);
 #pragma unroll
             for (int j = 0; j < 16; ++j) packed[j] = Pair<bf16>::pack(o[j].x, o[j].y);
           }
@@ -402,9 +424,12 @@
       ptx::mbar_wait(&a_full[buf], (j / Cfg::A_BUFS) & 1);
       const int r = quad * 32 + lane;
       uint8_t* base = smem + Cfg::OFF_A + buf * Cfg::KB1 * Cfg::A_TILE;
-      sstat[(j & 1) * Cfg::BM + r] =
+      const float2 st =
           GP ? ln_row_stats_smem<C>([&](int ch) { return base + ch * (Cfg::BM * 16) + r * 16; })
              : ln_row_stats_smem<C>([&](int ch) { return base + r * 128 + (ch >> 3) * Cfg::A_TILE + (((ch & 7) ^ (r & 7)) << 4); });
+      sstat[(j & 1) * Cfg::BM + r] = st.x;
+      *reinterpret_cast<uint4*>(smem + Cfg::OFF_R1 + (buf * Cfg::BM + r) * 16) = rank1_a_row(st.y);
+      ptx::fence_proxy_async_smem();
       __syncwarp();
       if (lane == 0) {
         ptx::mbar_arrive(&a_ready[buf]);
@@ -517,12 +542,14 @@
   static constexpr int OFF_W2 = OFF_W1T + 3 * 8192;
   static constexpr int OFF_AM = OFF_W2 + 6 * 12288;
   static constexpr int OFF_AT = OFF_AM + 16384;
-  static constexpr int OFF_H = OFF_AT + 8192;
-  static constexpr int OFF_STG = OFF_H + 32768;
+  using R1 = Rank1<HD, 1>;
+  static constexpr int OFF_R1 = OFF_AT + 8192;
+  static constexpr int OFF_STG = OFF_R1 + R1::BYTES;
   static constexpr int OFF_BAR = OFF_STG + 8 * 2048;
   static constexpr int OFF_VEC = OFF_BAR + 256;
-  static constexpr int SMEM_BYTES = OFF_VEC + (3 * HD + 4 * C) * 4 + 2 * BM * 8 + 1024;
+  static constexpr int SMEM_BYTES = OFF_VEC + (HD + 4 * C) * 4 + 2 * BM * 4 + 1024;
   static constexpr int D2_COL = 0, D2_STRIDE = 128, D1_COL = 256, TMEM_COLS = 512;
+  static constexpr int H_COL = D2_COL + C;
   static constexpr int W_BYTES = 3 * 16384 + 3 * 8192 + 6 * 12288;
   static_assert(SMEM_BYTES <= 227 * 1024, "smem budget");
 };
@@ -556,15 +583,10 @@
   float* sgamma = sb2 + C;
   float* slnw = sgamma + C;
   float* slnb = slnw + C;
-  float* ss1 = slnb + C;
-  float2* sstat = reinterpret_cast<float2*>(ss1 + 2 * Cfg::HD);
+  float* sstat = slnb + C;
   const bool ln = a.ln_w != nullptr;
   for (int i = threadIdx.x; i < Cfg::HD; i += blockDim.x) sb1[i] = a.b1[i];
-  if (FOLD)
-    for (int i = threadIdx.x; i < Cfg::HD; i += blockDim.x) {
-      ss1[4 * (i >> 1) + (i & 1)] = a.b1[i];
-      ss1[4 * (i >> 1) + 2 + (i & 1)] = a.ln_s[i];
-    }
+  if (FOLD) Cfg::R1::build(smem + Cfg::OFF_R1, a.ln_s);
   if (ln)
     for (int i = threadIdx.x; i < C; i += blockDim.x) {
       slnw[i] = a.ln_w[i];
@@ -650,6 +672,20 @@
       ptx::tc_fence_after();
       const int my_tiles = (int)blockIdx.x < num_tiles ? (num_tiles - 1 - (int)blockIdx.x) / (int)gridDim.x + 1 : 0;
       const uint32_t total = (uint32_t)Cfg::NC * my_tiles;
+      const uint32_t r1 = sbase + Cfg::OFF_R1;
+      auto gemm1_finish = [&](uint32_t g, int h, int it) {
+        const int db1 = g & 3;
+        if (FOLD) {
+          if (h == 0) {
+            ptx::mbar_wait(a_ready, it & 1);
+            ptx::tc_fence_after();
+          }
+          ptx::umma_bf16(tmem_base + Cfg::D1_COL + db1 * Cfg::NH, Cfg::R1::desc_a(r1, 0), Cfg::R1::desc_b(r1, h * Cfg::NH),
+                         idesc1, 1u);
+        }
+        ptx::umma_commit(&d1_full[db1]);
+        if (h == Cfg::NC - 1) ptx::umma_commit(a_empty);
+      };
       auto gemm1 = [&](uint32_t g, int h, int it) {
         if (h == 0) {
           ptx::mbar_wait((ln && !FOLD) ? a_ready : a_full, it & 1);
@@ -672,8 +708,7 @@
 #pragma unroll
           for (int k = 0; k < 2; ++k) ptx::umma_bf16(d1, dAt + 2 * k, dBt + 2 * k, idesc1, 1u);
         }
-        ptx::umma_commit(&d1_full[db1]);
-        if (h == Cfg::NC - 1) ptx::umma_commit(a_empty);
+        if (!FOLD) gemm1_finish(g, h, it);
       };
       auto gemm2 = [&](uint32_t g, int h, int it) {
         const int hb = g & 1;
@@ -682,10 +717,10 @@
         if (h == 0) ptx::mbar_wait(&d2_empty[it & 1], ((it >> 1) & 1) ^ 1);
         ptx::tc_fence_after();
         const uint32_t d2 = tmem_base + Cfg::D2_COL + (it & 1) * Cfg::D2_STRIDE;
-        const uint64_t da = ptx::umma_desc_sw128_kmajor(sbase + Cfg::OFF_H + hb * 16384);
+        const uint32_t ha = tmem_base + Cfg::H_COL + hb * Cfg::D2_STRIDE;
         const uint64_t db = ptx::umma_desc_sw128_kmajor(sbase + Cfg::OFF_W2 + h * 12288);
 #pragma unroll
-        for (int k = 0; k < 4; ++k) ptx::umma_bf16(d2, da + 2 * k, db + 2 * k, idesc2, (h | k) != 0 ? 1u : 0u);
+        for (int k = 0; k < 4; ++k) ptx::umma_bf16_tmem_a(d2, ha + 8 * k, db + 2 * k, idesc2, (h | k) != 0 ? 1u : 0u);
         ptx::umma_commit(&h_empty[hb]);
         if (h == Cfg::NC - 1) ptx::umma_commit(&d2_full[it & 1]);
         ACX_TRACE(0, 2 * h + 1);
@@ -693,7 +728,17 @@
       constexpr int LA = 4;
       int h1 = 0, it1 = 0;
       uint32_t g1 = 0;
+      uint32_t gf = 0;
+      int hf = 0, itf = 0;
       auto issue_gemm1 = [&]() {
+        if (FOLD && gf < g1) {
+          gemm1_finish(gf, hf, itf);
+          ++gf;
+          if (++hf == Cfg::NC) {
+            hf = 0;
+            ++itf;
+          }
+        }
         if (g1 < total) {
           gemm1(g1, h1, it1);
           ++g1;
@@ -721,14 +766,14 @@
     const int row_in_tile = quad * 32 + lane;
     const uint32_t lane_base = tmem_base + (static_cast<uint32_t>(quad * 32) << 16);
     const bool tr = (warp == 4 && lane == 0);
-    LnFold fold{0ull, 0ull, ptx::smem_u32(sb1), ptx::smem_u32(ss1)};
+    const uint32_t hcol = lane_base + Cfg::H_COL + group * Cfg::D2_STRIDE;
+    LnFold fold{};
     int it = 0;
     for (int tile = blockIdx.x; tile < num_tiles; tile += gridDim.x, ++it) {
       if (FOLD) {
         ptx::mbar_wait(a_ready, it & 1);
-        const float2 stt = sstat[(it & 1) * Cfg::BM + row_in_tile];
-        fold.rstd2 = f2_pack(stt.x, stt.x);
-        fold.nmr2 = f2_pack(stt.y, stt.y);
+        const float rstd = sstat[(it & 1) * Cfg::BM + row_in_tile];
+        fold.rstd2 = f2_pack(rstd, rstd);
       }
       for (int hc = 0; hc < Cfg::NC / 2; ++hc) {
         const int h = 2 * hc + group;
@@ -740,48 +785,42 @@
         if (tr) ACX_TRACE(1, 4 * hc + 1);
         const uint32_t t0 = lane_base + Cfg::D1_COL + buf * Cfg::NH;
         const uint32_t bias = ptx::smem_u32(sb1 + h * Cfg::NH);
-        const uint32_t hrow = ptx::smem_u32(smem + Cfg::OFF_H + group * 16384 + row_in_tile * 128);
         uint32_t raA[16], raB[16];
         GeluPair gA[8], gB[8];
         uint32_t pk[8] = {};
-        auto store_quarter = [&](int qi) {
-          asm volatile("st.shared.v4.b32 [%0], {%1, %2, %3, %4};" ::"r"(hrow + (((2 * qi) ^ (row_in_tile & 7)) << 4)),
-                       "r"(pk[0]), "r"(pk[1]), "r"(pk[2]), "r"(pk[3])
-                       : "memory");
-          asm volatile("st.shared.v4.b32 [%0], {%1, %2, %3, %4};" ::"r"(hrow + (((2 * qi + 1) ^ (row_in_tile & 7)) << 4)),
-                       "r"(pk[4]), "r"(pk[5]), "r"(pk[6]), "r"(pk[7])
-                       : "memory");
-        };
+        auto store_quarter = [&](int qi) { ptx::tmem_st_32x32b_x8(hcol + 8 * qi, pk); };
         ptx::tmem_ld_32x32b_x16(t0, raA);
         ptx::tmem_ld_32x32b_x16(t0 + 16, raB);
         ptx::tmem_ld_wait_dep(raA, raB);
-        gelu_stage_ta4<false, true, FOLD>(nullptr, gA, raA, bias, fold);
-        gelu_stage_ta4<false, true, FOLD>(nullptr, gA + 4, raA + 8, bias + 32, fold);
+        gelu_stage_ta4<false, true, false, FOLD>(nullptr, gA, raA, bias, fold);
+        gelu_stage_ta4<false, true, false, FOLD>(nullptr, gA + 4, raA + 8, bias + 32, fold);
         ptx::tmem_ld_32x32b_x16(t0 + 32, raA);
-        gelu_stage_ta4<true, true, FOLD>(gA, gB, raB, bias + 64, fold);
-        gelu_stage_ta4<true, true, FOLD>(gA + 4, gB + 4, raB + 8, bias + 96, fold);
+        gelu_stage_ta4<true, true, false, FOLD>(gA, gB, raB, bias + 64, fold);
+        gelu_stage_ta4<true, true, false, FOLD>(gA + 4, gB + 4, raB + 8, bias + 96, fold);
         ptx::tmem_ld_32x32b_x16(t0 + 48, raB);
         gelu_stage_c8_twice_bf16(gA, pk);
         ptx::mbar_wait(&h_empty[group], ((gc >> 1) & 1) ^ 1);
+        ptx::tc_fence_after();
         store_quarter(0);
         ptx::tmem_ld_wait_dep(raA, raB);
         ptx::tc_fence_before();
         __syncwarp();
         if (lane == 0) ptx::mbar_arrive(&d1_empty[buf]);
         if (tr) ACX_TRACE(1, 4 * hc + 2);
-        gelu_stage_ta4<true, true, FOLD>(gB, gA, raA, bias + 128, fold);
-        gelu_stage_ta4<true, true, FOLD>(gB + 4, gA + 4, raA + 8, bias + 160, fold);
+        gelu_stage_ta4<true, true, false, FOLD>(gB, gA, raA, bias + 128, fold);
+        gelu_stage_ta4<true, true, false, FOLD>(gB + 4, gA + 4, raA + 8, bias + 160, fold);
         gelu_stage_c8_twice_bf16(gB, pk);
         store_quarter(1);
-        gelu_stage_ta4<true, true, FOLD>(gA, gB, raB, bias + 192, fold);
-        gelu_stage_ta4<true, true, FOLD>(gA + 4, gB + 4, raB + 8, bias + 224, fold);
+        gelu_stage_ta4<true, true, false, FOLD>(gA, gB, raB, bias + 192, fold);
+        gelu_stage_ta4<true, true, false, FOLD>(gA + 4, gB + 4, raB + 8, bias + 224, fold);
         gelu_stage_c8_twice_bf16(gA, pk);
         store_quarter(2);
         gelu_stage_ta4<true, false>(gB, nullptr, nullptr, 0);
         gelu_stage_ta4<true, false>(gB + 4, nullptr, nullptr, 0);
         gelu_stage_c8_twice_bf16(gB, pk);
         store_quarter(3);
-        ptx::fence_proxy_async_smem();
+        ptx::tmem_st_wait();
+        ptx::tc_fence_before();
         __syncwarp();
         if (lane == 0) ptx::mbar_arrive(&h_full[group]);
         if (tr) ACX_TRACE(1, 4 * hc + 3);
@@ -813,15 +852,12 @@
       const int r = quad * 32 + lane;
       uint8_t* am = smem + Cfg::OFF_AM + r * 128;
       uint8_t* at = smem + Cfg::OFF_AT + r * 64;
-#ifdef ACX_AB_NO_STATS
-      sstat[(j & 1) * Cfg::BM + r] = make_float2(1.f, 0.f);
-      (void)am;
-      (void)at;
-#else
-      sstat[(j & 1) * Cfg::BM + r] =
+      const float2 st =
           GP ? ln_row_stats_smem<C>([&](int ch) { return smem + Cfg::OFF_AM + ch * 2048 + r * 16; })
              : ln_row_stats_smem<C>([&](int ch) { return ch < 8 ? am + ((ch ^ (r & 7)) << 4) : at + (((ch - 8) ^ ((r >> 1) & 3)) << 4); });
-#endif
+      sstat[(j & 1) * Cfg::BM + r] = st.x;
+      *reinterpret_cast<uint4*>(smem + Cfg::OFF_R1 + r * 16) = rank1_a_row(st.y);
+      ptx::fence_proxy_async_smem();
       __syncwarp();
       if (lane == 0) {
         ptx::mbar_arrive(a_ready);
diff --git a/audioset-convnext-inf_b200/csrc/ptx.cuh b/audioset-convnext-inf_b200/csrc/ptx.cuh
--- a/audioset-convnext-inf_b200/csrc/ptx.cuh
+++ b/audioset-convnext-inf_b200/csrc/ptx.cuh
@@ -156,6 +156,15 @@
       ::"r"(tmem_d), "l"(desc_a), "l"(desc_b), "r"(idesc), "r"(accumulate)
       : "memory");
 }
+__device__ __forceinline__ void umma_bf16_tmem_a(uint32_t tmem_d, uint32_t tmem_a, uint64_t desc_b, uint32_t idesc,
+                                                 uint32_t accumulate) {
+  asm volatile(
+      "{\n\t.reg .pred p;\n\t"
+      "setp.ne.b32 p, %4, 0;\n\t"
+      "tcgen05.mma.cta_group::1.kind::f16 [%0], [%1], %2, %3, p;\n\t}\n"
+      ::"r"(tmem_d), "r"(tmem_a), "l"(desc_b), "r"(idesc), "r"(accumulate)
+      : "memory");
+}
 __device__ __forceinline__ void umma_commit(uint64_t* bar) {
   asm volatile("tcgen05.commit.cta_group::1.mbarrier::arrive::one.shared::cluster.b64 [%0];" ::"r"(smem_u32(bar))
                : "memory");
@@ -181,6 +190,14 @@
       : "r"(taddr)
       : "memory");
 }
+__device__ __forceinline__ void tmem_st_32x32b_x8(uint32_t taddr, const uint32_t* r) {
+  asm volatile("tcgen05.st.sync.aligned.32x32b.x8.b32 [%0], {%1, %2, %3, %4, %5, %6, %7, %8};"
+               ::"r"(taddr), "r"(r[0]), "r"(r[1]), "r"(r[2]), "r"(r[3]), "r"(r[4]), "r"(r[5]), "r"(r[6]), "r"(r[7])
+               : "memory");
+}
+__device__ __forceinline__ void tmem_st_wait() {
+  asm volatile("tcgen05.wait::st.sync.aligned;" ::: "memory");
+}
 __device__ __forceinline__ void tmem_ld_wait() {
   asm volatile("tcgen05.wait::ld.sync.aligned;" ::: "memory");
 }
diff --git a/audioset-convnext-inf_b200/engine.py b/audioset-convnext-inf_b200/engine.py
--- a/audioset-convnext-inf_b200/engine.py
+++ b/audioset-convnext-inf_b200/engine.py
@@ -100,6 +100,8 @@
                 if precision == "bf16" and s < 3:
                     stage[-1].update(fold_layernorm_into_pwconv1(g(p + "pwconv1.weight"), g(p + "pwconv1.bias"),
                                                                  g(p + "norm.weight"), g(p + "norm.bias")))
+                    if s == 2:
+                        stage[-1]["w1x"] = rank1_extended_weight(stage[-1]["w1f"], stage[-1]["s1"])
             self.blocks.append(stage)
 
         self.norm_w, self.norm_b = g("norm.weight").contiguous(), g("norm.bias").contiguous()
@@ -110,6 +112,16 @@
     w1f = (w1.double() * ln_w.double()[None, :]).to(torch.float32).to(torch.bfloat16).contiguous()
     return dict(w1f=w1f, s1=w1f.double().sum(1).to(torch.float32).contiguous(),
                 b1f=(b1.double() + w1.double() @ ln_b.double()).to(torch.float32).contiguous())
+
+
+def rank1_extended_weight(w1f, s1):
+    s = s1.float()
+    t0 = s.to(torch.bfloat16)
+    r = s - t0.float()
+    t1 = r.to(torch.bfloat16)
+    t2 = (r - t1.float()).to(torch.bfloat16)
+    tail = torch.stack([t0, t1, t2, t0, t1, t2, t0, t1], 1)
+    return torch.cat([w1f.to(torch.bfloat16), tail.to(w1f.device)], 1).contiguous()
 
 
 def fold_dft_weights(conv_real, conv_imag, n_chunks, tol=1e-6):
@@ -419,9 +431,9 @@
                 stats = ws["stats"].data_ptr()
                 for blk in w.blocks[s]:
                     self._call_v(f"dwconv_tc_c{C}", "acx_dwconv_tc_gp", rh, xg, blk["dw_w"].data_ptr(), blk["dw_b"].data_ptr(), vg, n, H, Wd, C, st)
-                    self._call(f"row_stats_c{C}", "acx_gp_row_stats", vg, stats, M, C, st)
-                    self._call(f"pw1_gelu_k{C}_n{4 * C}", "acx_gemm_bf16_pw1_gp", vg, blk["w1f"].data_ptr(), hid, M, 4 * C, C,
-                               blk["b1f"].data_ptr(), stats, blk["s1"].data_ptr(), st)
+                    self._call(f"row_stats_c{C}", "acx_gp_row_stats_rank1", vg, stats, M, C, st)
+                    self._call(f"pw1_gelu_k{C}_n{4 * C}", "acx_gemm_bf16_pw1_gp_rank1", vg, blk["w1x"].data_ptr(), hid, M, 4 * C,
+                               C + 8, blk["b1f"].data_ptr(), stats, st)
                     self._call(f"pw2_resid_k{4 * C}_n{C}", "acx_gemm_bf16_pw2_gp", hid, blk["w2"].data_ptr(), xg, M, C, 4 * C,
                                blk["b2"].data_ptr(), blk["gamma"].data_ptr(), st)
             elif gp:
diff --git a/include/acx.h b/include/acx.h
--- a/include/acx.h
+++ b/include/acx.h
@@ -65,6 +65,7 @@
                      void* stream);
 ACX_API int acx_gp_transpose(const void* in, void* out, long long M, int C, int to_gp, void* stream);
 ACX_API int acx_gp_row_stats(const void* v, float* stats, long long M, int C, void* stream);
+ACX_API int acx_gp_row_stats_rank1(void* v, float* stats, long long M, int C, void* stream);
 
 ACX_API int acx_ln_patchify(const void* x, const float* ln_w, const float* ln_b, void* a, int B, int H, int W, int C,
                     int act_dtype, void* stream);
@@ -82,6 +83,8 @@
                          const float* stats, const float* ln_s, void* stream);
 ACX_API int acx_gemm_bf16_pw2_gp(const void* hid, const void* w2, void* x_gp, int M, int N, int K, const float* b2,
                          const float* gamma, void* stream);
+ACX_API int acx_gemm_bf16_pw1_gp_rank1(const void* v_gp, const void* w1x, void* hid, int M, int N, int K, const float* b1f,
+                               const float* stats, void* stream);
 ACX_API int acx_gemm_f32(const float* A, long long batch_stride, int rows_per_batch, int row_stride, const float* W,
                  float* out, int ldo, int M, int N, int K, int epilogue, const float* bias,
                  const float* gamma, const float* resid, void* stream);
```

Result: no change. 13850 (median of 6 runs) (+0.7%).
